# cosdata/cosdata

Hardware: AMD Instinct MI355X
Metric: QPS at recall@10≥0.95, 1024-dim dense cosine, 1/2/4/8 MI355X (higher is better)
Workload: dtype u8

## Files before the change

cosdata_amd/csrc/builder.hip:

```cpp
#include <algorithm>
#include <chrono>
#include <cmath>
#include <cstdio>
#include <cstdlib>
#include <cstring>
#include <map>

#include "engine_internal.h"

using namespace cosdev;

namespace {

constexpr u32 NONE = 0xFFFFFFFFu;

inline uint64_t splitmix64(uint64_t &st) {
    uint64_t z = (st += 0x9E3779B97F4A7C15ull);
    z = (z ^ (z >> 30)) * 0xBF58476D1CE4E5B9ull;
    z = (z ^ (z >> 27)) * 0x94D049BB133111EBull;
    return z ^ (z >> 31);
}
inline float rand_f32(uint64_t &st) { return (float)(splitmix64(st) >> 40) * (1.0f / 16777216.0f); }

inline int32_t total_key(float v) {
    int32_t b;
    memcpy(&b, &v, 4);
    b ^= (int32_t)(((uint32_t)(b >> 31)) >> 1);
    return b;
}
inline float metric_min(u32 metric) { return metric == COS_METRIC_COSINE ? -1.0f : -INFINITY; }
inline float metric_max(u32 metric) { return metric == COS_METRIC_COSINE ? 2.0f : INFINITY; }
inline int32_t order_key(u32 metric, float v) {
    const int32_t k = total_key(v);
    return (metric == COS_METRIC_EUCLIDEAN || metric == COS_METRIC_HAMMING) ? ~k : k;
}

}

namespace {

std::vector<double> level_probs(u32 Ltop) {
    std::vector<double> pv(Ltop + 1);
    for (u32 k = 0; k <= Ltop; k++) {
        const int nn = (int)(Ltop - k);
        double r = 1.0, a = 4.0;
        for (int b = nn;;) { if (b & 1) r *= a; b /= 2; if (b == 0) break; a *= a; }
        pv[k] = 1.0 - 1.0 / r;
    }
    return pv;
}
inline uint8_t draw_level(uint64_t &rng, const std::vector<double> &pv, u32 Ltop) {
    const double x = (double)rand_f32(rng);
    u32 k = 0;
    while (k < Ltop && !(x >= pv[k])) k++;
    return (uint8_t)(Ltop - k);
}

struct GraphGuard {
    cos_index *ix;
    bool armed = true;
    ~GraphGuard() {
        if (!armed) return;
        (void)hipStreamSynchronize(ix->own_stream);
        for (auto &l : ix->lv) l.release();
        ix->link.release();
        ix->adj_mag_valid = false;
        ix->have_root = false;
    }
};

void fill_link_levels(cos_index *ix, LinkArgs &la, u32 &maxM) {
    maxM = 0;
    for (u32 l = 0; l <= ix->p.num_layers; l++) {
        LevelHost &H = ix->lv[l];
        LinkLevelDev &D = la.lv[l];
        D.adj_vec = H.d_adj_vec;
        D.adj_node = l == 0 ? H.d_adj_vec : H.d_adj_node;
        D.node_vec = l == 0 ? nullptr : H.d_node_vec;
        D.key = ix->link.key[l].as<int32_t>();
        D.low_idx = ix->link.low_idx[l].as<uint8_t>();
        D.low_key = ix->link.low_key[l].as<int32_t>();
        D.owner = ix->link.owner[l].as<u32>();
        D.M = H.M;
        maxM = std::max(maxM, H.M);
    }
}

int32_t run_batches(cos_index *ix, u32 first, const uint8_t *max_level, std::vector<u32> &cursor, u32 Bmax) {
    const u32 n = ix->n, Ltop = ix->p.num_layers, L1 = Ltop + 1, metric = ix->p.metric;
    hipStream_t st = ix->own_stream;
    LinkArgs la;
    memset(&la, 0, sizeof(la));
    u32 maxM = 0;
    fill_link_levels(ix, la, maxM);
    if (maxM > 256) return cos_fail(COS_ERR_UNIMPLEMENTED, "more than 256 neighbour slots per node");

    const u32 KEEP = (u32)KEEP_INDEX;
    DevBuf d_rows, d_out_ids, d_out_nodes, d_out_sims, d_out_counts, d_status, d_me, d_pend[2], d_cnt, d_evq;
    PinArr<unsigned char> h_rows, h_me, h_pend, h_status, h_cnt;
    const size_t pend_cap = (size_t)Bmax * L1;
    const size_t evq_cap = pend_cap * 2 * KEEP;
    HIP_TRY(d_rows.alloc((size_t)Bmax * 4));
    HIP_TRY(d_out_ids.alloc((size_t)Bmax * L1 * KEEP * 4));
    HIP_TRY(d_out_nodes.alloc((size_t)Bmax * L1 * KEEP * 4));
    HIP_TRY(d_out_sims.alloc((size_t)Bmax * L1 * KEEP * 4));
    HIP_TRY(d_out_counts.alloc((size_t)Bmax * L1 * 4));
    HIP_TRY(d_status.alloc((size_t)Bmax * 4));
    HIP_TRY(d_me.alloc((size_t)Bmax * L1 * 4));
    HIP_TRY(d_pend[0].alloc(pend_cap * 4));
    HIP_TRY(d_pend[1].alloc(pend_cap * 4));
    HIP_TRY(d_cnt.alloc(4 * 4));
    HIP_TRY(d_evq.alloc(evq_cap * 3 * 4));
    HIP_TRY(h_rows.alloc((size_t)Bmax * 4));
    HIP_TRY(h_me.alloc((size_t)Bmax * L1 * 4));
    HIP_TRY(h_pend.alloc(pend_cap * 4));
    HIP_TRY(h_status.alloc((size_t)Bmax * 4));
    HIP_TRY(h_cnt.alloc(4 * 4));
    VisTab vtab;

    la.L1 = L1;
    la.z_nodes = d_out_nodes.as<u32>();
    la.z_sims = d_out_sims.as<float>();
    la.z_counts = d_out_counts.as<u32>();
    la.me = d_me.as<u32>();
    la.metric = metric;
    la.kmin = order_key(metric, metric_min(metric));
    la.kmax = order_key(metric, metric_max(metric));

    IndexDev dev = cos_make_index_dev(ix);
    u32 inserted = first, round = 0;
    u64 n_rounds = 0, n_batches = 0;
    const bool prof = cosdev::tune_or(cosdev::TUNE_BUILD_PROFILE, 0) != 0;
    double t_walk = 0, t_link = 0;
    auto now = []() { return std::chrono::duration<double>(std::chrono::steady_clock::now().time_since_epoch()).count(); };
    u32 *cnt = d_cnt.as<u32>();
    while (inserted < n) {
        const double t0 = now();
        n_batches++;
        const u32 bs = std::min({Bmax, std::max(1u, inserted / 4u), n - inserted});
        u32 np = 0;
        for (u32 b = 0; b < bs; b++) {
            const u32 id = inserted + b;
            h_rows.as<u32>()[b] = id;
            for (u32 l = 0; l <= Ltop; l++) {
                u32 m = NONE;
                if (max_level[id - first] >= l) { m = cursor[l]++; h_pend.as<u32>()[np++] = (l << 16) | b; }
                h_me.as<u32>()[(size_t)b * L1 + l] = m;
            }
        }
        HIP_TRY(hipMemcpyAsync(d_rows.p, h_rows.p, (size_t)bs * 4, hipMemcpyHostToDevice, st));
        HIP_TRY(hipMemcpyAsync(d_me.p, h_me.p, (size_t)bs * L1 * 4, hipMemcpyHostToDevice, st));
        HIP_TRY(hipMemcpyAsync(d_pend[0].p, h_pend.p, (size_t)np * 4, hipMemcpyHostToDevice, st));
        h_cnt.as<u32>()[0] = np; h_cnt.as<u32>()[1] = 0; h_cnt.as<u32>()[2] = 0; h_cnt.as<u32>()[3] = 0;
        HIP_TRY(hipMemcpyAsync(cnt, h_cnt.p, 16, hipMemcpyHostToDevice, st));
        WalkArgs wa;
        memset(&wa, 0, sizeof(wa));
        wa.qcodes = ix->d_codes;
        wa.qmags = ix->d_mags;
        wa.q_rows = d_rows.as<u32>();
        wa.self_ids = d_rows.as<u32>();
        if (dev.visited_mode == COS_VISITED_EXACT) {
            const int32_t vrc = vis_tab_prepare(vtab, ix, Bmax, ix->p.ef_construction, st, wa);
            if (vrc) return vrc;
        }
        wa.B = bs;
        wa.ef = ix->p.ef_construction;
        wa.keep = KEEP;
        wa.out_ids = d_out_ids.as<u32>();
        wa.out_sims = d_out_sims.as<float>();
        wa.out_nodes = d_out_nodes.as<u32>();
        wa.out_counts = d_out_counts.as<u32>();
        wa.out_status = d_status.as<int32_t>();
        cosdev::WalkPlanIn pin = cos_walk_plan_in(ix, bs, wa.ef);
        pin.table_min_B = pin.order_min_B = 0;
        HIP_TRY(launch_walk(ix->eng, dev, wa, cosdev::walk_plan(pin).kernel, st));
        HIP_TRY(hipMemcpyAsync(h_status.p, d_status.p, (size_t)bs * 4, hipMemcpyDeviceToHost, st));
        HIP_TRY(hipStreamSynchronize(st));
        for (u32 b = 0; b < bs; b++)
            if (h_status.as<int32_t>()[b] != COS_OK)
                return cos_fail(h_status.as<int32_t>()[b], "vector %u cannot be indexed (zero norm -> DistanceError::CalculationError)", inserted + b);
        t_walk += now() - t0;
        const double t1 = now();
        u32 pending_ub = np, cur = 0;
        while (pending_ub > 0) {
            const u32 chunk = pending_ub > 64 ? 2 : 4;
            for (u32 r = 0; r < chunk; r++) {
                if (++round > LINK_MAX_ROUND) {
                    for (u32 l = 0; l <= Ltop; l++) HIP_TRY(hipMemsetAsync(ix->link.owner[l].p, 0, (size_t)ix->lv[l].n * 4, st));
                    round = 1;
                }
                HIP_TRY(launch_link_round(la, maxM, d_pend[cur].as<u32>(), cnt + cur, d_pend[cur ^ 1].as<u32>(), cnt + (cur ^ 1), d_evq.as<u32>(), cnt + 2,
                                          pending_ub, round, st));
                cur ^= 1;
                n_rounds++;
            }
            HIP_TRY(hipMemcpyAsync(h_cnt.p, cnt, 16, hipMemcpyDeviceToHost, st));
            HIP_TRY(hipStreamSynchronize(st));
            pending_ub = h_cnt.as<u32>()[cur];
        }
        t_link += now() - t1;
        inserted += bs;
    }
    HIP_TRY(hipStreamSynchronize(st));
    if (prof)
        fprintf(stderr, "[cos_index_build] vectors [%u, %u) batches=%llu link rounds=%llu walk %.2fs link %.2fs\n", first, n, (unsigned long long)n_batches,
                (unsigned long long)n_rounds, t_walk, t_link);
    return COS_OK;
}

}

extern "C" int32_t cos_index_build(cos_index *ix, uint32_t batch_size) {
    if (!ix) return cos_fail(COS_ERR_INVALID, "null index");
    if (!ix->have_vectors) return cos_fail(COS_ERR_NOT_READY, "upload vectors before building");
    int32_t rc = cos_set_device(ix);
    if (rc) return rc;
    const u32 n = ix->n, Ltop = ix->p.num_layers, metric = ix->p.metric;
    const u32 Bmax = std::min<u32>(batch_size ? batch_size : 4096u, LINK_MAX_BATCH);
    hipStream_t st = ix->own_stream;
    GraphGuard guard{ix};

    ix->order_rank_valid = false;
    ix->level_table_valid = false;
    ix->adj_mag_valid = false;
    ix->link.release();
    uint64_t rng = ix->p.seed ? ix->p.seed : 0x1234567ull;
    std::vector<float> root(ix->p.dim);
    for (u32 i = 0; i < ix->p.dim; i++) root[i] = ix->p.range_lo + rand_f32(rng) * (ix->p.range_hi - ix->p.range_lo);
    rc = cos_index_set_root(ix, root.data());
    if (rc) return rc;
    const std::vector<double> pv = level_probs(Ltop);
    std::vector<uint8_t> max_level(n);
    for (u32 id = 0; id < n; id++) max_level[id] = draw_level(rng, pv, Ltop);

    for (u32 l = 0; l <= Ltop; l++) {
        LevelHost &H = ix->lv[l];
        H.release();
        for (u32 id = 0; id < n; id++)
            if (max_level[id] >= l) H.node_ids.push_back(id * ix->id_stride);
        H.node_ids.push_back(COS_ROOT_ID);
        const u32 nl = (u32)H.node_ids.size(), M = H.M;
        if (M > 256) return cos_fail(COS_ERR_UNIMPLEMENTED, "more than 256 neighbour slots per node");
        HIP_TRY(H.d_adj_vec.alloc((size_t)nl * M));
        HIP_TRY(hipMemsetAsync(H.d_adj_vec, 0xFF, (size_t)nl * M * 4, st));
        if (l > 0) {
            std::vector<u32> node_vec(nl), child(nl);
            const std::vector<u32> &D = ix->lv[l - 1].node_ids;
            for (u32 i = 0; i < nl; i++) {
                node_vec[i] = H.node_ids[i] == COS_ROOT_ID ? n : H.node_ids[i] / ix->id_stride;
                child[i] = (u32)(std::lower_bound(D.begin(), D.end(), H.node_ids[i]) - D.begin());
            }
            HIP_TRY(H.d_adj_node.alloc((size_t)nl * M));
            HIP_TRY(hipMemsetAsync(H.d_adj_node, 0xFF, (size_t)nl * M * 4, st));
            HIP_TRY(H.d_node_vec.alloc(nl));
            HIP_TRY(hipMemcpy(H.d_node_vec, node_vec.data(), (size_t)nl * 4, hipMemcpyHostToDevice));
            HIP_TRY(H.d_child.alloc(nl));
            HIP_TRY(hipMemcpy(H.d_child, child.data(), (size_t)nl * 4, hipMemcpyHostToDevice));
        }
        H.n = nl;
        HIP_TRY(ix->link.key[l].alloc((size_t)nl * M * 4));
        HIP_TRY(ix->link.low_idx[l].alloc(nl));
        HIP_TRY(ix->link.low_key[l].alloc((size_t)nl * 4));
        HIP_TRY(ix->link.owner[l].alloc((size_t)nl * 4));
        HIP_TRY(launch_fill_i32(ix->link.key[l].as<int32_t>(), (u64)nl * M, INT32_MIN, st));
        HIP_TRY(hipMemsetAsync(ix->link.low_idx[l].p, 0, nl, st));
        HIP_TRY(launch_fill_i32(ix->link.low_key[l].as<int32_t>(), nl, order_key(metric, metric_min(metric)), st));
        HIP_TRY(hipMemsetAsync(ix->link.owner[l].p, 0, (size_t)nl * 4, st));
    }
    HIP_TRY(hipStreamSynchronize(st));

    std::vector<u32> cursor(Ltop + 1, 0);
    rc = run_batches(ix, 0, max_level.data(), cursor, Bmax);
    if (rc) return rc;
    guard.armed = false;
    ix->link.rng = rng;
    ix->link.n_built = n;
    ix->link.valid = ix->id_stride == 1u;
    if (int32_t rc2 = cos_prepare_walk_plans(ix)) return rc2;
    return COS_OK;
}

extern "C" int32_t cos_index_restore_link_state(cos_index *ix) {
    if (!ix) return cos_fail(COS_ERR_INVALID, "null index");
    if (!ix->have_vectors || !ix->have_root) return cos_fail(COS_ERR_NOT_READY, "restore needs vectors, root and every graph level");
    for (auto &l : ix->lv) if (l.n == 0) return cos_fail(COS_ERR_NOT_READY, "restore needs vectors, root and every graph level");
    if (ix->id_stride != 1u || ix->meta.mdim != 0u) return cos_fail(COS_ERR_UNIMPLEMENTED, "link state of a collection with a metadata schema");
    int32_t rc = cos_set_device(ix);
    if (rc) return rc;
    HIP_TRY(hipDeviceSynchronize());
    const u32 Ltop = ix->p.num_layers, metric = ix->p.metric;
    const int32_t kmin = order_key(metric, metric_min(metric)), kmax = order_key(metric, metric_max(metric));
    hipStream_t st = ix->own_stream;
    ix->link.release();
    struct Fail { cos_index *ix; bool armed = true; ~Fail() { if (armed) ix->link.release(); } } fail_guard{ix};
    constexpr u64 CHUNK_PAIRS = 1ull << 24;
    DevBuf px, py, sims, dst, d_fail;
    HIP_TRY(px.alloc(CHUNK_PAIRS * 4));
    HIP_TRY(py.alloc(CHUNK_PAIRS * 4));
    HIP_TRY(sims.alloc(CHUNK_PAIRS * 4));
    HIP_TRY(dst.alloc(CHUNK_PAIRS * 4));
    HIP_TRY(d_fail.alloc(4));
    HIP_TRY(hipMemsetAsync(d_fail.p, 0, 4, st));
    for (u32 l = 0; l <= Ltop; l++) {
        LevelHost &H = ix->lv[l];
        const u32 nl = H.n, M = H.M;
        HIP_TRY(ix->link.key[l].alloc((size_t)nl * M * 4));
        HIP_TRY(ix->link.low_idx[l].alloc(nl));
        HIP_TRY(ix->link.low_key[l].alloc((size_t)nl * 4));
        HIP_TRY(ix->link.owner[l].alloc((size_t)nl * 4));
        HIP_TRY(hipMemsetAsync(ix->link.owner[l].p, 0, (size_t)nl * 4, st));
        const u32 step = (u32)std::max<u64>(1, CHUNK_PAIRS / M);
        for (u32 n0 = 0; n0 < nl; n0 += step) {
            const u32 cn = std::min(step, nl - n0);
            HIP_TRY(launch_edge_pairs(H.d_adj_vec, l == 0 ? nullptr : H.d_node_vec, n0, cn, M, px.as<u32>(), py.as<u32>(), st));
            HIP_TRY(cosdev::launch_index_pair_distances(ix->eng, ix->d_codes, ix->d_mags, ix->row_stride, ix->nchunks, ix->p.dim, metric, px.as<u32>(), py.as<u32>(),
                                                       (u32)((u64)cn * M), sims.as<float>(), dst.as<int32_t>(), st));
            HIP_TRY(launch_edge_keys(H.d_adj_vec, sims.as<float>(), dst.as<int32_t>(), n0, cn, M, metric, ix->link.key[l].as<int32_t>(), d_fail.as<int32_t>(), st));
        }
        HIP_TRY(launch_low_cache(H.d_adj_vec, ix->link.key[l].as<int32_t>(), nl, M, kmin, kmax, ix->link.low_idx[l].as<uint8_t>(), ix->link.low_key[l].as<int32_t>(), st));
    }
    int32_t failed = 0;
    HIP_TRY(hipMemcpyAsync(&failed, d_fail.p, 4, hipMemcpyDeviceToHost, st));
    HIP_TRY(hipStreamSynchronize(st));
    if (failed) return cos_fail(failed, "an edge of the uploaded graph has no similarity (zero norm -> DistanceError::CalculationError)");
    uint64_t rng = ix->p.seed ? ix->p.seed : 0x1234567ull;
    for (u64 i = 0; i < (u64)ix->p.dim + ix->n; i++) (void)rand_f32(rng);
    ix->link.rng = rng;
    ix->link.n_built = ix->n;
    ix->link.valid = true;
    fail_guard.armed = false;
    return COS_OK;
}

extern "C" int32_t cos_index_release_link_state(cos_index *ix) {
    if (!ix) return cos_fail(COS_ERR_INVALID, "null index");
    int32_t rc = cos_set_device(ix);
    if (rc) return rc;
    HIP_TRY(hipStreamSynchronize(ix->own_stream));
    ix->link.release();
    return COS_OK;
}

extern "C" int32_t cos_index_append(cos_index *ix, const float *raw, uint32_t m, uint32_t flags, uint32_t batch_size) {
    if (!ix || !raw || m == 0) return cos_fail(COS_ERR_INVALID, "null/empty vectors");
    if (!ix->have_vectors || !ix->have_root) return cos_fail(COS_ERR_NOT_READY, "append needs a built index");
    for (auto &l : ix->lv) if (l.n == 0) return cos_fail(COS_ERR_NOT_READY, "append needs a built index");
    if (!ix->link.valid || ix->link.n_built != ix->n)
        return cos_fail(COS_ERR_NOT_READY, "no link state to continue from: the graph was uploaded (not built by cos_index_build on this handle), its root "
                                           "was replaced, or cos_index_release_link_state freed it");
    if (ix->id_stride != 1u || ix->meta.mdim != 0u) return cos_fail(COS_ERR_UNIMPLEMENTED, "append on a collection with a metadata schema");
    if ((u64)ix->n + m >= 0xFFFFFFF0ull) return cos_fail(COS_ERR_INVALID, "too many vectors");
    const bool borrow = (flags & COS_UPLOAD_BORROW_DEVICE) != 0;
    if (borrow != !ix->raw_own)
        return cos_fail(COS_ERR_INVALID, borrow ? "the index owns its raw rows: append host rows" : "the index borrows its raw rows: append with COS_UPLOAD_BORROW_DEVICE and the whole grown table");
    int32_t rc = cos_set_device(ix);
    if (rc) return rc;
    const u32 n0 = ix->n, n1 = n0 + m, Ltop = ix->p.num_layers, metric = ix->p.metric;
    const u32 Bmax = std::min<u32>(batch_size ? batch_size : 4096u, LINK_MAX_BATCH);
    const u64 dim = ix->p.dim, rs = ix->row_stride;
    hipStream_t st = ix->own_stream;
    HIP_TRY(hipDeviceSynchronize());
    GraphGuard guard{ix};
    ix->order_rank_valid = false;
    ix->level_table_valid = false;
    ix->adj_mag_valid = false;
    ix->link.valid = false;
    cos_flat_ws_release(ix);

    {
        DevArr<uint8_t> codes;
        DevArr<float> mags, raw_mags, new_raw;
        HIP_TRY(codes.alloc(((size_t)n1 + 2) * rs));
        HIP_TRY(mags.alloc((size_t)n1 + 2));
        HIP_TRY(raw_mags.alloc((size_t)n1 + 2));
        HIP_TRY(hipMemcpyAsync(codes, ix->d_codes, (size_t)n0 * rs, hipMemcpyDeviceToDevice, st));
        HIP_TRY(hipMemcpyAsync(codes + (size_t)n1 * rs, ix->d_codes + (size_t)n0 * rs, 2 * rs, hipMemcpyDeviceToDevice, st));
        HIP_TRY(hipMemcpyAsync(mags, ix->d_mags, (size_t)n0 * 4, hipMemcpyDeviceToDevice, st));
        HIP_TRY(hipMemcpyAsync(mags + n1, ix->d_mags + n0, 8, hipMemcpyDeviceToDevice, st));
        HIP_TRY(hipMemcpyAsync(raw_mags, ix->d_raw_mags, (size_t)n0 * 4, hipMemcpyDeviceToDevice, st));
        HIP_TRY(hipMemsetAsync(raw_mags + n1, 0, 8, st));
        const float *new_rows;
        if (borrow) {
            new_rows = raw + (size_t)n0 * dim;
        } else {
            HIP_TRY(new_raw.alloc((size_t)n1 * dim));
            HIP_TRY(hipMemcpyAsync(new_raw, ix->d_raw, (size_t)n0 * dim * 4, hipMemcpyDeviceToDevice, st));
            HIP_TRY(hipMemcpyAsync(new_raw + (size_t)n0 * dim, raw, (size_t)m * dim * 4, hipMemcpyHostToDevice, st));
            new_rows = new_raw + (size_t)n0 * dim;
        }
        HIP_TRY(launch_quantize_rows(ix->eng, new_rows, dim, m, ix->p.dim, ix->p.range_lo, ix->p.range_hi, codes + (size_t)n0 * rs, rs, mags + n0, raw_mags + n0, st));
        HIP_TRY(cos_deleted_grow(ix, n0, n1, st));
        HIP_TRY(hipStreamSynchronize(st));
        codes.swap(ix->d_codes);
        mags.swap(ix->d_mags);
        raw_mags.swap(ix->d_raw_mags);
        new_raw.swap(ix->raw_own);
        ix->d_raw = borrow ? raw : ix->raw_own.p;
        ix->n = n1;
    }

    uint64_t rng = ix->link.rng;
    const std::vector<double> pv = level_probs(Ltop);
    std::vector<uint8_t> max_level(m);
    for (u32 i = 0; i < m; i++) max_level[i] = draw_level(rng, pv, Ltop);

    std::vector<u32> cursor(Ltop + 1, 0);
    std::vector<u32> add(Ltop + 1, 0);
    for (u32 l = 0; l <= Ltop; l++)
        for (u32 i = 0; i < m; i++) add[l] += max_level[i] >= l ? 1u : 0u;
    for (u32 l = 0; l <= Ltop; l++) {
        LevelHost &H = ix->lv[l];
        const u32 nl0 = H.n, nl1 = nl0 + add[l], M = H.M;
        cursor[l] = nl0 - 1;
        H.node_ids.pop_back();
        for (u32 i = 0; i < m; i++) if (max_level[i] >= l) H.node_ids.push_back(n0 + i);
        H.node_ids.push_back(COS_ROOT_ID);
        H.host_valid = false;
        H.nbr_ids.clear();
        H.d_adj_mag.reset();
        DevArr<u32> adj_vec, adj_node, node_vec, child;
        DevBuf key, low_idx, low_key;
        HIP_TRY(adj_vec.alloc((size_t)nl1 * M));
        HIP_TRY(launch_grow_rows(H.d_adj_vec, adj_vec, nl0, nl1, M, n0, n1, ROW_EMPTY, st));
        if (l > 0) {
            HIP_TRY(adj_node.alloc((size_t)nl1 * M));
            HIP_TRY(launch_grow_rows(H.d_adj_node, adj_node, nl0, nl1, M, nl0 - 1, nl1 - 1, ROW_EMPTY, st));
            std::vector<u32> nv(add[l] + 1), ch(add[l] + 1);
            const u32 below0 = ix->lv[l - 1].n - add[l - 1] - 1;
            u32 k = 0, kb = 0;
            for (u32 i = 0; i < m; i++) {
                if (max_level[i] >= l) { nv[k] = n0 + i; ch[k] = below0 + kb; k++; }
                if (max_level[i] >= l - 1) kb++;
            }
            nv[k] = n1;
            ch[k] = ix->lv[l - 1].n - 1;
            HIP_TRY(node_vec.alloc(nl1));
            HIP_TRY(child.alloc(nl1));
            HIP_TRY(hipMemcpyAsync(node_vec, H.d_node_vec, (size_t)(nl0 - 1) * 4, hipMemcpyDeviceToDevice, st));
            HIP_TRY(hipMemcpyAsync(child, H.d_child, (size_t)(nl0 - 1) * 4, hipMemcpyDeviceToDevice, st));
            HIP_TRY(hipMemcpy(node_vec + (nl0 - 1), nv.data(), nv.size() * 4, hipMemcpyHostToDevice));
            HIP_TRY(hipMemcpy(child + (nl0 - 1), ch.data(), ch.size() * 4, hipMemcpyHostToDevice));
        }
        HIP_TRY(key.alloc((size_t)nl1 * M * 4));
        HIP_TRY(low_idx.alloc(nl1));
        HIP_TRY(low_key.alloc((size_t)nl1 * 4));
        HIP_TRY(launch_grow_rows(ix->link.key[l].as<u32>(), key.as<u32>(), nl0, nl1, M, 0xFFFFFFFFu, 0xFFFFFFFFu, (u32)INT32_MIN, st));
        HIP_TRY(launch_grow_rows(ix->link.low_key[l].as<u32>(), low_key.as<u32>(), nl0, nl1, 1, 0xFFFFFFFFu, 0xFFFFFFFFu, (u32)order_key(metric, metric_min(metric)), st));
        HIP_TRY(launch_grow_bytes(ix->link.low_idx[l].as<uint8_t>(), low_idx.as<uint8_t>(), nl0, nl1, st));
        HIP_TRY(ix->link.owner[l].alloc((size_t)nl1 * 4));
        HIP_TRY(hipMemsetAsync(ix->link.owner[l].p, 0, (size_t)nl1 * 4, st));
        HIP_TRY(hipStreamSynchronize(st));
        adj_vec.swap(H.d_adj_vec);
        adj_node.swap(H.d_adj_node);
        node_vec.swap(H.d_node_vec);
        child.swap(H.d_child);
        key.swap(ix->link.key[l]);
        low_idx.swap(ix->link.low_idx[l]);
        low_key.swap(ix->link.low_key[l]);
        H.n = nl1;
    }

    rc = run_batches(ix, n0, max_level.data(), cursor, Bmax);
    if (rc) return rc;
    guard.armed = false;
    ix->link.rng = rng;
    ix->link.n_built = n1;
    ix->link.valid = true;
    if (int32_t rc2 = cos_prepare_walk_plans(ix)) return rc2;
    return COS_OK;
}

namespace {

struct RowCache {
    struct Row { std::vector<u32> adj; std::vector<int32_t> key; uint8_t low_idx; int32_t low_key; bool dirty = false; };
    cos_index *ix; u32 level; u32 M;
    std::map<u32, Row> rows;
    hipError_t err = hipSuccess;
    Row &get(u32 node) {
        auto it = rows.find(node);
        if (it != rows.end()) return it->second;
        Row &r = rows[node];
        LevelHost &H = ix->lv[level];
        r.adj.resize(M); r.key.resize(M);
        auto cp = [&](void *dst, const void *src, size_t n) { if (err == hipSuccess) err = hipMemcpy(dst, src, n, hipMemcpyDeviceToHost); };
        cp(r.adj.data(), (level == 0 ? H.d_adj_vec : H.d_adj_node) + (size_t)node * M, (size_t)M * 4);
        cp(r.key.data(), ix->link.key[level].as<int32_t>() + (size_t)node * M, (size_t)M * 4);
        cp(&r.low_idx, ix->link.low_idx[level].as<uint8_t>() + node, 1);
        cp(&r.low_key, ix->link.low_key[level].as<int32_t>() + node, 4);
        return r;
    }
    hipError_t flush(const std::vector<u32> &node_vec ) {
        LevelHost &H = ix->lv[level];
        for (auto &kv : rows) {
            if (!kv.second.dirty || err != hipSuccess) continue;
            const u32 node = kv.first;
            Row &r = kv.second;
            auto cp = [&](void *dst, const void *src, size_t n) { if (err == hipSuccess) err = hipMemcpy(dst, src, n, hipMemcpyHostToDevice); };
            if (level == 0) cp(H.d_adj_vec + (size_t)node * M, r.adj.data(), (size_t)M * 4);
            else {
                std::vector<u32> av(M);
                for (u32 j = 0; j < M; j++) av[j] = r.adj[j] == NONE ? NONE : node_vec[r.adj[j]];
                cp(H.d_adj_node + (size_t)node * M, r.adj.data(), (size_t)M * 4);
                cp(H.d_adj_vec + (size_t)node * M, av.data(), (size_t)M * 4);
            }
            cp(ix->link.key[level].as<int32_t>() + (size_t)node * M, r.key.data(), (size_t)M * 4);
            cp(ix->link.low_idx[level].as<uint8_t>() + node, &r.low_idx, 1);
            cp(ix->link.low_key[level].as<int32_t>() + node, &r.low_key, 4);
        }
        return err;
    }
};

int add_neighbor_host(RowCache &rc, u32 self, u32 nbr, int32_t k, int32_t kmin, int32_t kmax) {
    RowCache::Row &r = rc.get(self);
    const u32 M = rc.M, li = r.low_idx;
    if (k <= r.low_key) return -1;
    const bool ok = r.adj[li] == NONE || k > r.key[li];
    u32 old = NONE;
    if (ok) { old = r.adj[li]; r.adj[li] = nbr; r.key[li] = k; }
    u32 nl = 0;
    int32_t nk = kmax;
    for (u32 j = 0; j < M; j++) {
        if (r.adj[j] == NONE) { nk = kmin; nl = j; break; }
        if (r.key[j] < nk) { nk = r.key[j]; nl = j; }
    }
    r.low_idx = (uint8_t)nl;
    r.low_key = nk;
    r.dirty = true;
    if (!ok) return -1;
    if (old != NONE) {
        RowCache::Row &o = rc.get(old);
        for (u32 j = 0; j < M; j++) if (o.adj[j] == self) { o.adj[j] = NONE; o.key[j] = INT32_MIN; o.dirty = true; break; }
    }
    return (int)li;
}

}

extern "C" int32_t cos_index_delete(cos_index *ix, const uint32_t *ids, uint32_t m) {
    if (!ix || (!ids && m)) return cos_fail(COS_ERR_INVALID, "null argument");
    if (!ix->have_vectors || !ix->have_root) return cos_fail(COS_ERR_NOT_READY, "delete needs a built index");
    for (auto &l : ix->lv) if (l.n == 0) return cos_fail(COS_ERR_NOT_READY, "delete needs a built index");
    if (!ix->link.valid) return cos_fail(COS_ERR_NOT_READY, "no link state (the graph was uploaded, its root replaced, or cos_index_release_link_state freed it)");
    if (ix->id_stride != 1u || ix->meta.mdim != 0u) return cos_fail(COS_ERR_UNIMPLEMENTED, "delete on a collection with a metadata schema");
    for (u32 i = 0; i < m; i++) if (ids[i] >= ix->n) return cos_fail(COS_ERR_INVALID, "id %u is not a resident vector", ids[i]);
    if (m == 0) return COS_OK;
    int32_t rc = cos_set_device(ix);
    if (rc) return rc;
    HIP_TRY(hipDeviceSynchronize());
    const u32 Ltop = ix->p.num_layers, L1 = Ltop + 1, metric = ix->p.metric, KEEP = (u32)KEEP_SEARCH, EF = 512;
    hipStream_t st = ix->own_stream;
    HIP_TRY(cos_deleted_mark(ix, ids, m, st));
    LinkArgs la;
    memset(&la, 0, sizeof(la));
    u32 maxM = 0;
    fill_link_levels(ix, la, maxM);
    la.L1 = L1;
    la.metric = metric;
    const int32_t kmin = order_key(metric, metric_min(metric)), kmax = order_key(metric, metric_max(metric));
    DevBuf d_row, d_out_ids, d_out_nodes, d_out_sims, d_out_counts, d_status, d_dn, d_ust, d_px, d_py, d_ds, d_dst;
    HIP_TRY(d_row.alloc(4));
    HIP_TRY(d_out_ids.alloc((size_t)L1 * KEEP * 4));
    HIP_TRY(d_out_nodes.alloc((size_t)L1 * KEEP * 4));
    HIP_TRY(d_out_sims.alloc((size_t)L1 * KEEP * 4));
    HIP_TRY(d_out_counts.alloc((size_t)L1 * 4));
    HIP_TRY(d_status.alloc(4));
    HIP_TRY(d_dn.alloc((size_t)L1 * 4));
    HIP_TRY(d_ust.alloc((size_t)L1 * 4));
    HIP_TRY(d_px.alloc((size_t)KEEP * 4));
    HIP_TRY(d_py.alloc((size_t)KEEP * 4));
    HIP_TRY(d_ds.alloc((size_t)KEEP * 4));
    HIP_TRY(d_dst.alloc((size_t)KEEP * 4));
    VisTab vtab;
    std::vector<u32> h_ids((size_t)L1 * KEEP), h_nodes((size_t)L1 * KEEP), h_counts(L1), h_dn(L1), h_ust(L1);
    std::vector<std::vector<u32>> node_vec(L1);
    ix->adj_mag_valid = false;
    for (auto &l : ix->lv) { l.host_valid = false; l.nbr_ids.clear(); }

    for (u32 t = 0; t < m; t++) {
        const u32 id = ids[t];
        IndexDev dev = cos_make_index_dev(ix);
        for (u32 l = 0; l <= Ltop; l++) dev.lv[l].adj_mag = nullptr;
        WalkArgs wa;
        memset(&wa, 0, sizeof(wa));
        HIP_TRY(hipMemcpyAsync(d_row.p, &id, 4, hipMemcpyHostToDevice, st));
        wa.qcodes = ix->d_codes;
        wa.qmags = ix->d_mags;
        wa.q_rows = d_row.as<u32>();
        wa.no_self_seed = 1u;
        if (dev.visited_mode == COS_VISITED_EXACT) {
            const int32_t vrc = vis_tab_prepare(vtab, ix, 1, EF, st, wa);
            if (vrc) return vrc;
        }
        wa.B = 1;
        wa.ef = EF;
        wa.keep = KEEP;
        wa.out_ids = d_out_ids.as<u32>();
        wa.out_sims = d_out_sims.as<float>();
        wa.out_nodes = d_out_nodes.as<u32>();
        wa.out_counts = d_out_counts.as<u32>();
        wa.out_status = d_status.as<int32_t>();
        cosdev::WalkPlanIn pin = cos_walk_plan_in(ix, 1, EF);
        pin.table_min_B = pin.order_min_B = 0;
        pin.no_self_seed = true;
        HIP_TRY(launch_walk(ix->eng, dev, wa, cosdev::walk_plan(pin).kernel, st));
        int32_t wst = COS_OK;
        HIP_TRY(hipMemcpyAsync(&wst, d_status.p, 4, hipMemcpyDeviceToHost, st));
        HIP_TRY(hipMemcpyAsync(h_ids.data(), d_out_ids.p, h_ids.size() * 4, hipMemcpyDeviceToHost, st));
        HIP_TRY(hipMemcpyAsync(h_nodes.data(), d_out_nodes.p, h_nodes.size() * 4, hipMemcpyDeviceToHost, st));
        HIP_TRY(hipMemcpyAsync(h_counts.data(), d_out_counts.p, (size_t)L1 * 4, hipMemcpyDeviceToHost, st));
        HIP_TRY(hipStreamSynchronize(st));
        if (wst != COS_OK) return cos_fail(wst, "vector %u cannot be walked for (zero norm -> DistanceError::CalculationError)", id);
        bool any = false;
        for (u32 l = 0; l <= Ltop; l++) {
            const u32 slot = Ltop - l;
            h_dn[l] = NONE;
            for (u32 i = 0; i < h_counts[slot]; i++)
                if (h_ids[(size_t)slot * KEEP + i] == id) { h_dn[l] = h_nodes[(size_t)slot * KEEP + i]; any = true; break; }
        }
        if (!any) continue;
        HIP_TRY(hipMemcpyAsync(d_dn.p, h_dn.data(), (size_t)L1 * 4, hipMemcpyHostToDevice, st));
        HIP_TRY(launch_unlink(la, d_dn.as<u32>(), d_ust.as<u32>(), st));
        HIP_TRY(hipMemcpyAsync(h_ust.data(), d_ust.p, (size_t)L1 * 4, hipMemcpyDeviceToHost, st));
        HIP_TRY(hipStreamSynchronize(st));
        for (u32 l = 0; l <= Ltop; l++) {
            if (h_ust[l] != 1u) continue;
            const LevelHost &H = ix->lv[l];
            const u32 M = H.M, slot = Ltop - l, node = h_dn[l];
            if (l > 0 && node_vec[l].empty()) {
                node_vec[l].resize(H.n);
                HIP_TRY(hipMemcpy(node_vec[l].data(), H.d_node_vec, (size_t)H.n * 4, hipMemcpyDeviceToHost));
            }
            auto vec_row = [&](u32 nd) { return l == 0 ? nd : node_vec[l][nd]; };
            std::vector<u32> res;
            for (u32 i = 0; i < h_counts[slot]; i++) if (h_nodes[(size_t)slot * KEEP + i] != node) res.push_back(h_nodes[(size_t)slot * KEEP + i]);
            RowCache cache{ix, l, M};
            RowCache::Row &dr = cache.get(node);
            for (u32 j = 0; j < M; j++) {
                const u32 x = dr.adj[j];
                if (x == NONE) continue;
                RowCache::Row &xr = cache.get(x);
                bool removed = false, empty = true;
                for (u32 k = 0; k < M; k++) if (xr.adj[k] == node) { xr.adj[k] = NONE; xr.key[k] = INT32_MIN; xr.dirty = true; removed = true; break; }
                for (u32 k = 0; k < M; k++) if (xr.adj[k] != NONE) { empty = false; break; }
                if (!(removed && empty)) continue;
                std::vector<u32> cand, px, py;
                for (u32 r : res) if (r != x) { cand.push_back(r); px.push_back(vec_row(x)); py.push_back(vec_row(r)); }
                std::vector<float> sims(cand.size());
                std::vector<int32_t> dst(cand.size());
                if (!cand.empty()) {
                    HIP_TRY(hipMemcpyAsync(d_px.p, px.data(), px.size() * 4, hipMemcpyHostToDevice, st));
                    HIP_TRY(hipMemcpyAsync(d_py.p, py.data(), py.size() * 4, hipMemcpyHostToDevice, st));
                    HIP_TRY(cosdev::launch_index_pair_distances(ix->eng, ix->d_codes, ix->d_mags, ix->row_stride, ix->nchunks, ix->p.dim, metric, d_px.as<u32>(), d_py.as<u32>(),
                                                               (u32)cand.size(), d_ds.as<float>(), d_dst.as<int32_t>(), st));
                    HIP_TRY(hipMemcpyAsync(sims.data(), d_ds.p, sims.size() * 4, hipMemcpyDeviceToHost, st));
                    HIP_TRY(hipMemcpyAsync(dst.data(), d_dst.p, dst.size() * 4, hipMemcpyDeviceToHost, st));
                    HIP_TRY(hipStreamSynchronize(st));
                    for (int32_t e : dst) if (e != COS_OK) return cos_fail(e, "re-linking node %u after the delete of %u failed (DistanceError)", x, id);
                }
// ... 255 lines not shown
```

cosdata_amd/csrc/device_common.h:

```cpp
#pragma once
#include <hip/hip_runtime.h>
#include <stdint.h>
#include <type_traits>

namespace cosdev {

typedef uint32_t u32;
typedef unsigned long long u64;

constexpr int WAVE = 64;
constexpr u32 ROW_EMPTY = 0xFFFFFFFFu;
constexpr int KEEP_SEARCH = 100;
constexpr int KEEP_INDEX = 64;
constexpr int MAX_LEVELS = 16;

enum : int { ENG_U8 = 0, ENG_Q2 = 1, ENG_F32 = 2, ENG_F16 = 3, ENG_Q1 = 4, ENG_Q3 = 5 };

__device__ __forceinline__ u32 simkey(float v) {
    u32 b = __float_as_uint(v);
    return b ^ ((b >> 31) ? 0xFFFFFFFFu : 0x80000000u);
}
__device__ __forceinline__ float simkey_inv(u32 k) {
    u32 b = (k & 0x80000000u) ? (k ^ 0x80000000u) : ~k;
    return __uint_as_float(b);
}
__device__ __forceinline__ u32 metric_key(u32 metric, float v) {
    u32 k = simkey(v);
    return (metric == 1u || metric == 2u) ? ~k : k;
}
__device__ __forceinline__ float metric_key_inv(u32 metric, u32 k) {
    return simkey_inv((metric == 1u || metric == 2u) ? ~k : k);
}
__device__ __forceinline__ u64 pack_key(u32 hi, u32 lo) { return ((u64)hi << 32) | (u64)lo; }

__device__ __forceinline__ float div_rn_unscaled(float num, float den) {
    float r = __builtin_amdgcn_rcpf(den);
    const float e = __builtin_fmaf(-den, r, 1.0f);
    r = __builtin_fmaf(e, r, r);
    float q = num * r;
    float t = __builtin_fmaf(-den, q, num);
    q = __builtin_fmaf(t, r, q);
    t = __builtin_fmaf(-den, q, num);
    return __builtin_fmaf(t, r, q);
}

__device__ __forceinline__ u64 shfl_xor_u64(u64 v, int m) {
    u32 lo = (u32)v, hi = (u32)(v >> 32);
    lo = (u32)__shfl_xor((int)lo, m, WAVE);
    hi = (u32)__shfl_xor((int)hi, m, WAVE);
    return ((u64)hi << 32) | lo;
}
__device__ __forceinline__ u64 shfl_up1_u64(u64 v) {
    u32 lo = (u32)v, hi = (u32)(v >> 32);
    lo = (u32)__shfl_up((int)lo, 1, WAVE);
    hi = (u32)__shfl_up((int)hi, 1, WAVE);
    return ((u64)hi << 32) | lo;
}
__device__ __forceinline__ u64 shfl_down1_u64(u64 v) {
    u32 lo = (u32)v, hi = (u32)(v >> 32);
    lo = (u32)__shfl_down((int)lo, 1, WAVE);
    hi = (u32)__shfl_down((int)hi, 1, WAVE);
    return ((u64)hi << 32) | lo;
}
template <int CTRL>
__device__ __forceinline__ u32 dpp_mov(u32 fill, u32 v) {
    return (u32)__builtin_amdgcn_update_dpp((int)fill, (int)v, CTRL, 0xf, 0xf, false);
}
template <int CTRL>
__device__ __forceinline__ u32 dpp_mov_z(u32 v) {
    return (u32)__builtin_amdgcn_update_dpp(0, (int)v, CTRL, 0xf, 0xf, true);
}
__device__ __forceinline__ u64 dpp_wave_shr1_u64(u64 v, u64 fill) {
    u32 lo = dpp_mov<0x138>((u32)fill, (u32)v), hi = dpp_mov<0x138>((u32)(fill >> 32), (u32)(v >> 32));
    return ((u64)hi << 32) | lo;
}
__device__ __forceinline__ u64 dpp_wave_shl1_u64(u64 v, u64 fill) {
    u32 lo = dpp_mov<0x130>((u32)fill, (u32)v), hi = dpp_mov<0x130>((u32)(fill >> 32), (u32)(v >> 32));
    return ((u64)hi << 32) | lo;
}
__device__ __forceinline__ u32 group_reduce_add_u32(u32 v, int G) {
    if (G >= 2) v += dpp_mov<0xB1>(0u, v);
    if (G >= 4) v += dpp_mov<0x4E>(0u, v);
    if (G >= 8) v += dpp_mov<0x141>(0u, v);
    if (G >= 16) v += dpp_mov<0x140>(0u, v);
    if (G == 32) v += (u32)__shfl_xor((int)v, 16, WAVE);
    if (G == 64) {
        const u32 t = (u32)__builtin_amdgcn_readlane((int)v, 0) + (u32)__builtin_amdgcn_readlane((int)v, 16) +
                      (u32)__builtin_amdgcn_readlane((int)v, 32) + (u32)__builtin_amdgcn_readlane((int)v, 48);
        v = t;
    }
    return v;
}

__device__ __forceinline__ u32 fold_halves(u32 a, u32 b) {
// ... 76 lines not shown
```

cosdata_amd/csrc/engine.hip:

```cpp
#include <hip/hip_runtime.h>

#include <algorithm>
#include <cstdarg>
#include <cstdio>
#include <cstdlib>
#include <chrono>
#include <cmath>
#include <condition_variable>
#include <cstring>
#include <map>
#include <mutex>
#include <string>
#include <thread>
#include <vector>

#include "engine_internal.h"

using namespace cosdev;

static thread_local std::string g_err;
int32_t cos_fail(int32_t code, const char *fmt, ...) {
    char buf[512];
    va_list ap;
    va_start(ap, fmt);
    vsnprintf(buf, sizeof(buf), fmt, ap);
    va_end(ap);
    g_err = buf;
    return code;
}

extern "C" const char *cos_last_error_string(void) { return g_err.c_str(); }

extern "C" int32_t cos_device_count(int32_t *out) {
    if (!out) return cos_fail(COS_ERR_INVALID, "null argument");
    int n = 0;
    hipError_t e = hipGetDeviceCount(&n);
    if (e != hipSuccess) { *out = 0; return cos_fail(COS_ERR_NO_DEVICE, "hipGetDeviceCount: %s", hipGetErrorString(e)); }
    *out = n;
    return COS_OK;
}

static u32 pow2ceil(u32 v) { u32 p = 1; while (p < v) p <<= 1; return p; }

int32_t cos_set_device(const cos_index *ix) {
    HIP_TRY(hipSetDevice(ix->p.device));
    return COS_OK;
}

static bool graph_ready(const cos_index *ix) {
    if (!ix->have_vectors || !ix->have_root) return false;
    for (auto &l : ix->lv) if (l.n == 0) return false;
    return true;
}

IndexDev cos_make_index_dev(const cos_index *ix) {
    IndexDev d;
    memset(&d, 0, sizeof(d));
    d.codes = ix->d_codes;
    d.mags = ix->d_mags;
    d.raw = ix->d_raw;
    d.raw_mags = ix->d_raw_mags;
    d.row_stride = ix->row_stride;
    d.raw_stride = ix->p.dim;
    d.n = ix->n;
    d.dim = ix->p.dim;
    d.metric = ix->p.metric;
    d.storage = ix->p.storage;
    d.num_layers = ix->p.num_layers;
    d.shortlist = ix->p.shortlist_size;
    d.visited_mode = ix->p.visited_mode;
    d.nchunks = ix->nchunks;
    d.G = ix->G;
    d.id_base = ix->p.id_base;
    d.id_stride = ix->id_stride;
    d.mbits = ix->meta.d_mbits;
    d.mmags = ix->meta.d_mmags;
    d.mdim = ix->meta.mdim;
    for (u32 l = 0; l <= ix->p.num_layers; l++) {
        const LevelHost &h = ix->lv[l];
        d.lv[l].adj_vec = h.d_adj_vec;
        d.lv[l].adj_node = l == 0 ? h.d_adj_vec : h.d_adj_node;
        d.lv[l].node_vec = l == 0 ? nullptr : h.d_node_vec;
        d.lv[l].child = l == 0 ? nullptr : h.d_child;
        d.lv[l].n = h.n;
        d.lv[l].M = h.M;
        d.lv[l].root_idx = h.n ? h.n - 1 : 0;
        d.lv[l].adj_mag = (ix->adj_mag_valid && cosdev::tune_or(cosdev::TUNE_WALK_ADJ_MAG, 1) != 0) ? h.d_adj_mag : nullptr;
        d.lv[l].mag_stride = std::min(h.M, ix->p.shortlist_size);
    }
    return d;
}

extern "C" int32_t cos_index_create(const cos_params *p, cos_index **out) {
    if (!p || !out) return cos_fail(COS_ERR_INVALID, "null argument");
    *out = nullptr;
    if (p->struct_size != sizeof(cos_params) || p->abi_version != COS_ABI_VERSION)
        return cos_fail(COS_ERR_INVALID, "cos_params size/version mismatch (%u/%u, expected %zu/%u)", p->struct_size, p->abi_version,
                    sizeof(cos_params), COS_ABI_VERSION);
    if (p->dim == 0) return cos_fail(COS_ERR_INVALID, "dim == 0");
    auto pow2 = [](u32 v) { return v && !(v & (v - 1)); };
    if (!pow2(p->neighbors_count) || !pow2(p->level0_neighbors_count) || p->neighbors_count > 256 || p->level0_neighbors_count > 256)
        return cos_fail(COS_ERR_INVALID, "neighbors_count / level_0_neighbors_count must be powers of two <= 256 (PerformantFixedSet, fixedset.rs)");
    if (p->num_layers + 1 > (u32)MAX_LEVELS || (p->num_layers + 1) * KEEP_SEARCH > 2048)
        return cos_fail(COS_ERR_UNIMPLEMENTED, "num_layers > 15 not supported on the device");
    if (p->ef_search > cosdev::WALK_GENERAL_MAX_EF || p->ef_construction > cosdev::WALK_GENERAL_MAX_EF)
        return cos_fail(COS_ERR_UNIMPLEMENTED, "ef > %u not supported on the device (the candidates of a level live in one workgroup's LDS)", cosdev::WALK_GENERAL_MAX_EF);
    if (p->metric != COS_METRIC_COSINE && p->metric != COS_METRIC_DOT)
        return cos_fail(COS_ERR_UNIMPLEMENTED, "device walk implements cosine and dot-product metrics");
    int eng;
    u64 row_stride;
    u32 nchunks = 0, G = 1;
    switch (p->storage) {
    case COS_STORAGE_U8:
        eng = ENG_U8; row_stride = ((u64)p->dim + 15) & ~15ull; nchunks = (u32)(row_stride / 16); G = std::min(64u, pow2ceil(nchunks));
        break;
    case COS_STORAGE_SUBBYTE:
        if (p->resolution == 1) { eng = ENG_Q1; nchunks = (p->dim + 127) / 128; }
        else if (p->resolution == 2) { eng = ENG_Q2; nchunks = (p->dim + 63) / 64; }
        else if (p->resolution == 3) { eng = ENG_Q3; nchunks = (p->dim + 31) / 32; }
        else return cos_fail(COS_ERR_CALCULATION, "SubByte resolution %u: the reference's distance arms return CalculationError (cosine.rs:147-154)", p->resolution);
        row_stride = (u64)nchunks * 16; G = std::min(64u, pow2ceil(nchunks));
        break;
    case COS_STORAGE_F32:
        if (p->metric == COS_METRIC_DOT) return cos_fail(COS_ERR_STORAGE_MISMATCH, "DotProductDistance has no FullPrecisionFP arm (dotproduct.rs:20-64)");
        eng = ENG_F32; row_stride = ((u64)p->dim * 4 + 15) & ~15ull; G = 2;
        break;
    case COS_STORAGE_F16:
        eng = ENG_F16; row_stride = ((u64)p->dim * 2 + 15) & ~15ull; G = 1;
        break;
    default: return cos_fail(COS_ERR_UNIMPLEMENTED, "storage kind %u not supported on the device yet", p->storage);
    }
    int ndev = 0;
    if (hipGetDeviceCount(&ndev) != hipSuccess || ndev <= 0) return cos_fail(COS_ERR_NO_DEVICE, "no HIP device visible; the GPU path has no CPU fallback");
    if (p->device < 0 || p->device >= ndev) return cos_fail(COS_ERR_INVALID, "device %d out of range (%d visible)", p->device, ndev);
    cos_index *ix = new cos_index();
    ix->chain_min_B = (u32)cosdev::tune_or(cosdev::TUNE_WALK_CHAIN_MIN_B, ix->chain_min_B);
    ix->walk_order_min_B = (u32)cosdev::tune_or(cosdev::TUNE_WALK_ORDER_MIN_B, ix->walk_order_min_B);
    ix->walk_side_min_B = (u32)cosdev::tune_or(cosdev::TUNE_WALK_SIDE_MIN_B, ix->walk_side_min_B);
    ix->p = *p;
    ix->eng = eng;
    ix->row_stride = row_stride;
    ix->nchunks = nchunks;
    ix->G = G;
    ix->lv.resize(p->num_layers + 1);
    for (u32 l = 0; l <= p->num_layers; l++) ix->lv[l].M = l == 0 ? p->level0_neighbors_count : p->neighbors_count;
    if (hipSetDevice(p->device) != hipSuccess || hipStreamCreateWithFlags(&ix->own_stream, hipStreamNonBlocking) != hipSuccess) {
        delete ix;
        return cos_fail(COS_ERR_HIP, "cannot create stream on device %d", p->device);
    }
    int nx = 0;
    if (hipDeviceGetAttribute(&nx, hipDeviceAttributeNumberOfXccs, p->device) == hipSuccess && nx >= 1 && nx <= 64) ix->num_xcd = (u32)nx;
    else { (void)hipGetLastError(); ix->num_xcd = 1; }
    int ncu = 0;
    if (hipDeviceGetAttribute(&ncu, hipDeviceAttributeMultiprocessorCount, p->device) == hipSuccess && ncu >= 1) ix->n_cus = (u32)ncu;
    else (void)hipGetLastError();
    *out = ix;
    return COS_OK;
}

IndexDev cos_make_meta_dev(const cos_index *ix) {
    IndexDev d = cos_make_index_dev(ix);
    for (u32 l = 0; l <= ix->p.num_layers; l++) {
        const LevelHost &h = ix->meta.lv[l];
        d.lv[l].adj_vec = h.d_adj_vec;
        d.lv[l].adj_node = h.d_adj_node;
        d.lv[l].node_vec = h.d_node_vec;
        d.lv[l].child = h.d_child;
        d.lv[l].node_id = h.d_node_id;
        d.lv[l].node_meta = h.d_node_meta;
        d.lv[l].n = h.n;
        d.lv[l].M = h.M;
        d.lv[l].root_idx = h.root_idx;
    }
    return d;
}

void cos_meta_free_levels(cos_index *ix) {
    for (auto &l : ix->meta.lv) l.release();
}

static void reset_meta(cos_index *ix) {
    for (auto &l : ix->meta.lv) l.release();
    ix->meta.d_mbits.reset();
    ix->meta.d_mmags.reset();
    ix->meta.node_ids.clear();
    ix->meta.mdim = 0;
    ix->id_stride = 1;
}

extern "C" int32_t cos_index_destroy(cos_index *ix) {
    if (!ix) return COS_OK;
    (void)hipSetDevice(ix->p.device);
    (void)hipDeviceSynchronize();
    ix->ws.clear();
    cos_flat_ws_release(ix);
    ix->pipes_all.clear();
    cos_coalesce_release(ix);
    for (auto &l : ix->lv) l.release();
    reset_meta(ix);
    if (ix->own_stream) (void)hipStreamDestroy(ix->own_stream);
    delete ix;
    return COS_OK;
}

extern "C" int32_t cos_index_upload_vectors(cos_index *ix, const float *raw, uint32_t n, uint32_t flags) {
    if (!ix || !raw || n == 0) return cos_fail(COS_ERR_INVALID, "null/empty vectors");
    if (n >= 0xFFFFFFF0u) return cos_fail(COS_ERR_INVALID, "too many vectors");
    int32_t rc = cos_set_device(ix);
    if (rc) return rc;
    ix->d_raw = nullptr;
    ix->raw_own.reset(); ix->d_raw_mags.reset(); ix->d_codes.reset(); ix->d_mags.reset(); ix->d_deleted.reset();
    ix->have_vectors = false;
    cos_flat_ws_release(ix);
    ix->have_root = false;
    for (auto &l : ix->lv) l.release();
    ix->order_rank_valid = false;
    ix->level_table_valid = false;
    ix->adj_mag_valid = false;
    ix->link.release();
    reset_meta(ix);
    const u64 dim = ix->p.dim;
    const float *d_raw = raw;
    DevArr<float> raw_own, raw_mags, mags;
    DevArr<uint8_t> codes;
    if (flags & COS_UPLOAD_BORROW_DEVICE) {
        HIP_TRY(hipDeviceSynchronize());
    } else {
        HIP_TRY(raw_own.alloc((size_t)n * dim));
        HIP_TRY(hipMemcpy(raw_own, raw, (size_t)n * dim * 4, hipMemcpyHostToDevice));
        d_raw = raw_own;
    }
    HIP_TRY(raw_mags.alloc((size_t)n + 2));
    HIP_TRY(codes.alloc(((size_t)n + 2) * ix->row_stride));
    HIP_TRY(mags.alloc((size_t)n + 2));
    HIP_TRY(hipMemsetAsync(codes + (size_t)n * ix->row_stride, 0, 2 * ix->row_stride, ix->own_stream));
    HIP_TRY(hipMemsetAsync(mags + n, 0, 8, ix->own_stream));
    HIP_TRY(launch_quantize_rows(ix->eng, d_raw, dim, n, ix->p.dim, ix->p.range_lo, ix->p.range_hi, codes, ix->row_stride, mags, raw_mags, ix->own_stream));
    HIP_TRY(cos_deleted_reset(ix, n, ix->own_stream));
    HIP_TRY(hipStreamSynchronize(ix->own_stream));
    ix->d_raw = d_raw;
    ix->raw_own = std::move(raw_own);
    ix->d_raw_mags = std::move(raw_mags);
    ix->d_codes = std::move(codes);
    ix->d_mags = std::move(mags);
    ix->n = n;
    ix->have_vectors = true;
    ix->have_root = false;
    return COS_OK;
}

extern "C" int32_t cos_index_set_root(cos_index *ix, const float *root_raw) {
    if (!ix || !root_raw) return cos_fail(COS_ERR_INVALID, "null argument");
    if (!ix->have_vectors) return cos_fail(COS_ERR_NOT_READY, "upload vectors before the root");
    int32_t rc = cos_set_device(ix);
    if (rc) return rc;
    ix->root_raw.assign(root_raw, root_raw + ix->p.dim);
    DevBuf tmp;
    HIP_TRY(tmp.alloc(((size_t)ix->p.dim + 1) * 4));
    float *d_tmp = tmp.as<float>(), *d_dummy = d_tmp + ix->p.dim;
    HIP_TRY(hipMemcpy(d_tmp, root_raw, (size_t)ix->p.dim * 4, hipMemcpyHostToDevice));
    HIP_TRY(launch_quantize_rows(ix->eng, d_tmp, ix->p.dim, 1, ix->p.dim, ix->p.range_lo, ix->p.range_hi,
                                 ix->d_codes + (size_t)ix->n * ix->row_stride, ix->row_stride, ix->d_mags + ix->n, d_dummy, ix->own_stream));
    HIP_TRY(hipStreamSynchronize(ix->own_stream));
    ix->have_root = true;
    ix->level_table_valid = false;
    ix->adj_mag_valid = false;
    if (ix->link.valid && graph_ready(ix)) ix->link.release();
    return COS_OK;
}

static inline u32 row_of(const cos_index *ix, u32 id) { return id == COS_ROOT_ID ? ix->n : id / ix->id_stride; }

static int32_t push_level_to_device(cos_index *ix, u32 level) {
    LevelHost &L = ix->lv[level];
    const u32 n = (u32)L.node_ids.size(), M = L.M;
    std::vector<u32> adj_vec((size_t)n * M), adj_node, node_vec, child;
    if (level > 0) { adj_node.resize((size_t)n * M); node_vec.resize(n); }
    for (u32 i = 0; i < n; i++) {
        if (level > 0) node_vec[i] = row_of(ix, L.node_ids[i]);
        for (u32 j = 0; j < M; j++) {
            u32 id = L.nbr_ids[(size_t)i * M + j];
            if (id == COS_SLOT_EMPTY) {
                adj_vec[(size_t)i * M + j] = ROW_EMPTY;
                if (level > 0) adj_node[(size_t)i * M + j] = ROW_EMPTY;
                continue;
            }
            auto it = std::lower_bound(L.node_ids.begin(), L.node_ids.end(), id);
            if (it == L.node_ids.end() || *it != id) return cos_fail(COS_ERR_INVALID, "level %u: neighbour id %u of node %u is not a node of this level", level, id, L.node_ids[i]);
            adj_vec[(size_t)i * M + j] = row_of(ix, id);
            if (level > 0) adj_node[(size_t)i * M + j] = (u32)(it - L.node_ids.begin());
        }
    }
    L.d_adj_node.reset();
    L.d_node_vec.reset();
    HIP_TRY(L.d_adj_vec.alloc(adj_vec.size()));
    HIP_TRY(hipMemcpy(L.d_adj_vec, adj_vec.data(), adj_vec.size() * 4, hipMemcpyHostToDevice));
    if (level > 0) {
        HIP_TRY(L.d_adj_node.alloc(adj_node.size()));
        HIP_TRY(hipMemcpy(L.d_adj_node, adj_node.data(), adj_node.size() * 4, hipMemcpyHostToDevice));
        HIP_TRY(L.d_node_vec.alloc(node_vec.size()));
        HIP_TRY(hipMemcpy(L.d_node_vec, node_vec.data(), node_vec.size() * 4, hipMemcpyHostToDevice));
    }
    L.n = n;
    L.host_valid = true;
    ix->order_rank_valid = false;
    ix->level_table_valid = false;
    ix->adj_mag_valid = false;
    ix->link.release();
    return COS_OK;
}

static int32_t push_level0_to_device(cos_index *ix, const u32 *nbr) {
    LevelHost &L = ix->lv[0];
    const u32 n = (u32)L.node_ids.size(), M = L.M;
    const size_t slots = (size_t)n * M, chunk = (size_t)32 << 20;
    struct Staging {
        hipEvent_t done[2] = {nullptr, nullptr};
        ~Staging() {
            for (int b = 0; b < 2; b++)
                if (done[b]) (void)hipEventSynchronize(done[b]), (void)hipEventDestroy(done[b]);
        }
    };
    PinArr<u32> buf[2];
    Staging stg;
    HIP_TRY(L.d_adj_vec.alloc(slots));
    for (int b = 0; b < 2; b++) {
        HIP_TRY(buf[b].alloc(std::min(chunk, slots)));
        HIP_TRY(hipEventCreateWithFlags(&stg.done[b], hipEventDisableTiming));
    }
    const u32 nt = std::max(1u, std::min(16u, std::thread::hardware_concurrency()));
    for (size_t c0 = 0, k = 0; c0 < slots; c0 += chunk, k++) {
        const size_t m = std::min(chunk, slots - c0);
        u32 *out = buf[k & 1];
        if (k >= 2) HIP_TRY(hipEventSynchronize(stg.done[k & 1]));
        std::vector<int> bad(nt, 0);
        auto convert = [&](u32 t) {
            for (size_t s = m * t / nt, e = m * (t + 1) / nt; s < e; s++) {
                const u32 id = nbr[c0 + s];
                if (id == COS_SLOT_EMPTY) { out[s] = ROW_EMPTY; continue; }
                if (id != COS_ROOT_ID && (id % ix->id_stride != 0 || id / ix->id_stride >= ix->n)) { bad[t] = 1; return; }
                out[s] = row_of(ix, id);
            }
        };
        std::vector<std::thread> th;
        u32 started = 0;
        try {
            th.reserve(nt);
            for (; started < nt; started++) th.emplace_back(convert, started);
        } catch (...) {
        }
        for (u32 t = started; t < nt; t++) convert(t);
        for (auto &x : th) x.join();
        for (int b : bad)
            if (b) return cos_fail(COS_ERR_INVALID, "level 0: a neighbour id is not a node of this level");
        HIP_TRY(hipMemcpyAsync(L.d_adj_vec + c0, out, m * 4, hipMemcpyHostToDevice, ix->own_stream));
        HIP_TRY(hipEventRecord(stg.done[k & 1], ix->own_stream));
    }
    HIP_TRY(hipStreamSynchronize(ix->own_stream));
    L.nbr_ids.clear();
    L.nbr_ids.shrink_to_fit();
    L.n = n;
    L.host_valid = false;
    ix->order_rank_valid = false;
    ix->level_table_valid = false;
    ix->adj_mag_valid = false;
    ix->link.release();
    return COS_OK;
}

static int32_t resolve_children(cos_index *ix, u32 level) {
    if (level == 0 || level > ix->p.num_layers) return COS_OK;
    LevelHost &L = ix->lv[level], &D = ix->lv[level - 1];
    if (L.node_ids.empty() || D.node_ids.empty()) return COS_OK;
    std::vector<u32> child(L.node_ids.size());
    for (size_t i = 0; i < L.node_ids.size(); i++) {
        auto it = std::lower_bound(D.node_ids.begin(), D.node_ids.end(), L.node_ids[i]);
        if (it == D.node_ids.end() || *it != L.node_ids[i]) return cos_fail(COS_ERR_INVALID, "node %u of level %u is missing on level %u", L.node_ids[i], level, level - 1);
        child[i] = (u32)(it - D.node_ids.begin());
    }
    HIP_TRY(L.d_child.alloc(child.size()));
    HIP_TRY(hipMemcpy(L.d_child, child.data(), child.size() * 4, hipMemcpyHostToDevice));
    return COS_OK;
}

extern "C" int32_t cos_index_upload_graph_level(cos_index *ix, uint32_t level, uint32_t n_nodes, const uint32_t *node_ids,
                                                const uint32_t *nbr_ids) {
    if (!ix || !node_ids || !nbr_ids) return cos_fail(COS_ERR_INVALID, "null argument");
    if (!ix->have_vectors) return cos_fail(COS_ERR_NOT_READY, "upload vectors before the graph");
    if (level > ix->p.num_layers || n_nodes == 0) return cos_fail(COS_ERR_INVALID, "bad level / empty level");
    int32_t rc = cos_set_device(ix);
    if (rc) return rc;
    for (u32 i = 0; i < n_nodes; i++) {
        if (i && node_ids[i] <= node_ids[i - 1]) return cos_fail(COS_ERR_INVALID, "level %u: node_ids must be strictly ascending", level);
        if (node_ids[i] != COS_ROOT_ID && (node_ids[i] % ix->id_stride != 0 || node_ids[i] / ix->id_stride >= ix->n))
            return cos_fail(COS_ERR_INVALID, "level %u: node id %u is not the base id of a resident vector (ids are vector row x %u)", level, node_ids[i], ix->id_stride);
    }
    if (node_ids[n_nodes - 1] != COS_ROOT_ID) return cos_fail(COS_ERR_INVALID, "level %u: the root (0xFFFFFFFF) must be the last node", level);
    if (level == 0 && n_nodes != ix->n + 1) return cos_fail(COS_ERR_INVALID, "level 0 must hold every vector plus the root (%u nodes, expected %u)", n_nodes, ix->n + 1);
    LevelHost &L = ix->lv[level];
    L.node_ids.assign(node_ids, node_ids + n_nodes);
    if (level == 0) {
        rc = push_level0_to_device(ix, nbr_ids);
    } else {
        L.nbr_ids.assign(nbr_ids, nbr_ids + (size_t)n_nodes * L.M);
        rc = push_level_to_device(ix, level);
    }
    if (rc) { L.release(); return rc; }
    rc = resolve_children(ix, level);
    if (rc == COS_OK) rc = resolve_children(ix, level + 1);
    if (rc == COS_OK && graph_ready(ix)) rc = cos_prepare_walk_plans(ix);
    return rc;
}

extern "C" int32_t cos_index_level_count(const cos_index *ix, uint32_t level, uint32_t *n_nodes) {
    if (!ix || !n_nodes || level > ix->p.num_layers) return cos_fail(COS_ERR_INVALID, "bad argument");
    *n_nodes = ix->lv[level].n;
    return COS_OK;
}

static int32_t materialize_host_level(cos_index *ix, u32 level) {
    LevelHost &L = ix->lv[level];
    if (L.host_valid) return COS_OK;
    if (L.n == 0 || L.node_ids.size() != L.n || !L.d_adj_vec) return cos_fail(COS_ERR_NOT_READY, "level %u not resident", level);
    int32_t rc = cos_set_device(ix);
    if (rc) return rc;
    std::vector<u32> adj((size_t)L.n * L.M);
    HIP_TRY(hipMemcpy(adj.data(), level == 0 ? L.d_adj_vec : L.d_adj_node, adj.size() * 4, hipMemcpyDeviceToHost));
    L.nbr_ids.resize(adj.size());
    for (size_t i = 0; i < adj.size(); i++) L.nbr_ids[i] = adj[i] == ROW_EMPTY ? COS_SLOT_EMPTY : L.node_ids[adj[i]];
    L.host_valid = true;
    return COS_OK;
}

extern "C" int32_t cos_index_download_graph_level(const cos_index *ix_, uint32_t level, uint32_t *node_ids, uint32_t *nbr_ids) {
    cos_index *ix = const_cast<cos_index *>(ix_);
    if (!ix || level > ix->p.num_layers) return cos_fail(COS_ERR_INVALID, "bad argument");
    {
        std::lock_guard<std::mutex> g(ix->mu);
        const int32_t rc = materialize_host_level(ix, level);
        if (rc) return rc;
    }
    const LevelHost &L = ix->lv[level];
    if (node_ids) memcpy(node_ids, L.node_ids.data(), L.node_ids.size() * 4);
    if (nbr_ids) memcpy(nbr_ids, L.nbr_ids.data(), L.nbr_ids.size() * 4);
    return COS_OK;
}

extern "C" size_t cos_code_bytes(uint32_t storage, uint32_t resolution, uint32_t dim) {
    switch (storage) {
    case COS_STORAGE_U8: return dim;
    case COS_STORAGE_SUBBYTE: return (size_t)resolution * ((dim + 7) / 8);
    case COS_STORAGE_F16: return (size_t)dim * 2;
    case COS_STORAGE_F32: return (size_t)dim * 4;
    default: return 0;
    }
}

static void row_to_reference_layout(int eng, u32 dim, const uint8_t *dev_row, uint8_t *ref_row) {
    if (eng == ENG_U8) memcpy(ref_row, dev_row, dim);
    else if (eng == ENG_F32) memcpy(ref_row, dev_row, (size_t)dim * 4);
    else if (eng == ENG_F16) memcpy(ref_row, dev_row, (size_t)dim * 2);
    else if (eng == ENG_Q1) memcpy(ref_row, dev_row, (dim + 7) / 8);
    else if (eng == ENG_Q2) {
        const u32 pb = (dim + 7) / 8;
        for (u32 p = 0; p < 2; p++)
            for (u32 b = 0; b < pb; b++) ref_row[(size_t)p * pb + b] = dev_row[(size_t)(b / 8) * 16 + p * 8 + (b % 8)];
    } else {
        const u32 pb = (dim + 7) / 8;
        for (u32 p = 0; p < 3; p++)
            for (u32 b = 0; b < pb; b++) ref_row[(size_t)p * pb + b] = dev_row[(size_t)(b / 4) * 16 + p * 4 + (b % 4)];
    }
}

static void row_to_device_layout(int eng, u32 dim, const uint8_t *ref_row, uint8_t *dev_row) {
    if (eng == ENG_U8) memcpy(dev_row, ref_row, dim);
    else if (eng == ENG_F32) memcpy(dev_row, ref_row, (size_t)dim * 4);
    else if (eng == ENG_F16) memcpy(dev_row, ref_row, (size_t)dim * 2);
    else if (eng == ENG_Q1) memcpy(dev_row, ref_row, (dim + 7) / 8);
    else if (eng == ENG_Q2) {
        const u32 pb = (dim + 7) / 8;
        for (u32 p = 0; p < 2; p++)
            for (u32 b = 0; b < pb; b++) dev_row[(size_t)(b / 8) * 16 + p * 8 + (b % 8)] = ref_row[(size_t)p * pb + b];
    } else {
        const u32 pb = (dim + 7) / 8;
        for (u32 p = 0; p < 3; p++)
            for (u32 b = 0; b < pb; b++) dev_row[(size_t)(b / 4) * 16 + p * 4 + (b % 4)] = ref_row[(size_t)p * pb + b];
    }
}

int32_t cos_set_root_code(cos_index *ix, const uint8_t *ref_code, float mag) {
    if (!ix->have_vectors) return cos_fail(COS_ERR_NOT_READY, "upload vectors before the root");
    int32_t rc = cos_set_device(ix);
    if (rc) return rc;
    std::vector<uint8_t> dev(ix->row_stride, 0);
    row_to_device_layout(ix->eng, ix->p.dim, ref_code, dev.data());
    if (ix->eng == ENG_U8) {
        const float hi = 255.0f * sqrtf((float)ix->p.dim) * 1.0001f;
        if (!(mag == 0.0f || (mag >= 1.0f && mag <= hi))) {
            uint32_t ss = 0;
            for (u32 i = 0; i < ix->p.dim; i++) ss += (uint32_t)ref_code[i] * (uint32_t)ref_code[i];
            mag = sqrtf((float)ss);
        }
    }
    HIP_TRY(hipMemcpy(ix->d_codes + (size_t)ix->n * ix->row_stride, dev.data(), dev.size(), hipMemcpyHostToDevice));
    HIP_TRY(hipMemcpy(ix->d_mags + ix->n, &mag, 4, hipMemcpyHostToDevice));
    ix->root_raw.assign(ix->p.dim, 0.0f);
    ix->have_root = true;
    ix->level_table_valid = false;
    ix->adj_mag_valid = false;
    return COS_OK;
}

int32_t cos_push_level_ids(cos_index *ix, u32 level, std::vector<u32> &&node_ids, std::vector<u32> &&nbr_ids) {
    return cos_index_upload_graph_level(ix, level, (u32)node_ids.size(), node_ids.data(), nbr_ids.data());
}

extern "C" int32_t cos_index_download_codes(const cos_index *ix, void *codes, float *mags) {
    if (!ix || !ix->have_vectors) return cos_fail(COS_ERR_NOT_READY, "no vectors resident");
    HIP_TRY(hipSetDevice(ix->p.device));
    const size_t rows = (size_t)ix->n + 1;
    if (codes) {
        std::vector<uint8_t> dev(rows * ix->row_stride);
        HIP_TRY(hipMemcpy(dev.data(), ix->d_codes, dev.size(), hipMemcpyDeviceToHost));
        const size_t cb = cos_code_bytes(ix->p.storage, ix->p.resolution, ix->p.dim);
        for (size_t r = 0; r < rows; r++) row_to_reference_layout(ix->eng, ix->p.dim, dev.data() + r * ix->row_stride, (uint8_t *)codes + r * cb);
    }
    if (mags) HIP_TRY(hipMemcpy(mags, ix->d_mags, rows * 4, hipMemcpyDeviceToHost));
    return COS_OK;
}

extern "C" int32_t cos_index_download_root(const cos_index *ix, float *root_raw) {
    if (!ix || !root_raw) return cos_fail(COS_ERR_INVALID, "null argument");
    if (!ix->have_root) return cos_fail(COS_ERR_NOT_READY, "no root");
    memcpy(root_raw, ix->root_raw.data(), (size_t)ix->p.dim * 4);
    return COS_OK;
}

static int32_t ensure_level_table(cos_index *ix);
static u32 walk_table_min_B(const cos_index *ix);
extern "C" int32_t cos_index_set_ef_search(cos_index *ix, uint32_t ef) {
    if (!ix) return cos_fail(COS_ERR_INVALID, "null index");
    if (ef > cosdev::WALK_GENERAL_MAX_EF) return cos_fail(COS_ERR_UNIMPLEMENTED, "ef > %u not supported on the device", cosdev::WALK_GENERAL_MAX_EF);
    std::lock_guard<std::mutex> g(ix->mu);
    const bool live = graph_ready(ix);
    if (live)
        if (int32_t rc = cos_set_device(ix)) return rc;
    ix->p.ef_search = ef;
    if (live && walk_table_min_B(ix)) (void)ensure_level_table(ix);
    return COS_OK;
}
extern "C" int32_t cos_index_set_visited_mode(cos_index *ix, uint32_t mode) {
    if (!ix || mode > 1) return cos_fail(COS_ERR_INVALID, "bad visited mode");
    std::lock_guard<std::mutex> g(ix->mu);
    ix->p.visited_mode = mode;
    return COS_OK;
}
extern "C" int32_t cos_index_set_latency_mode(cos_index *ix, uint32_t max_queries) {
    if (!ix) return cos_fail(COS_ERR_INVALID, "null");
    std::lock_guard<std::mutex> g(ix->mu);
    ix->lat_max_B = max_queries;
    return COS_OK;
}

extern "C" int32_t cos_index_set_latency_waves(cos_index *ix, uint32_t max_queries) {
    if (!ix) return cos_fail(COS_ERR_INVALID, "null");
    std::lock_guard<std::mutex> g(ix->mu);
    ix->lat4_max_B = max_queries;
    return COS_OK;
}
extern "C" int32_t cos_index_set_walk_order(cos_index *ix, uint32_t min_queries) {
    if (!ix) return cos_fail(COS_ERR_INVALID, "null");
    std::lock_guard<std::mutex> g(ix->mu);
    ix->walk_order_min_B = min_queries;
    return COS_OK;
}
extern "C" int32_t cos_index_enable_timing(cos_index *ix, int32_t on) {
    if (!ix) return cos_fail(COS_ERR_INVALID, "null");
    std::lock_guard<std::mutex> g(ix->mu);
    if (on && !ix->timing) for (auto &kv : ix->ws) kv.second->ev_count = 0;
    ix->timing = on != 0;
    return COS_OK;
}

int32_t vis_tab_prepare(VisTab &vt, const cos_index *ix, u32 B, u32 ef, hipStream_t st, WalkArgs &wa) {
    const u32 M = std::max(ix->p.level0_neighbors_count, ix->p.neighbors_count);
    const u64 log_cap = (u64)ef * M + 2;
    u32 max_nodes = 0;
    for (const LevelHost &l : ix->lv) max_nodes = std::max(max_nodes, l.n);
    const u32 words = (max_nodes + 31) / 32 + 1;
    if (log_cap > 0xFFFFFFFFull) return cos_fail(COS_ERR_INVALID, "ef too large");
    const size_t need_bits = (size_t)B * words, need_log = (size_t)B * log_cap;
    if (need_bits > vt.bits.cap || need_log > vt.log.cap) {
// ... 6 lines not shown
        HIP_TRY(hipMemsetAsync(vt.bits, 0, vt.bits.cap * 4, st));
        vt.zeroed = true;
    }
    wa.vis_bits = vt.bits;
    wa.vis_log = vt.log;
    wa.vis_words_per_query = words;
    wa.vis_log_cap = (u32)log_cap;
    return COS_OK;
}

static int32_t ensure_order_rank(cos_index *ix) {
    if (ix->order_rank_valid) return COS_OK;
    for (u32 l = 0; l < cosdev::MAX_LEVELS; l++) {
        ix->d_order_rank[l].reset();
        ix->order_rank_n[l] = 0;
    }
    ix->order_levels.clear();
    const u32 Ltop = ix->p.num_layers;
    auto usable = [&](u32 l) { return l >= 1 && l <= Ltop && ix->lv[l].n > 1 && ix->lv[l].n <= (1u << 20) && ix->lv[l].d_adj_node; };
    std::vector<u32> want;
    if (const long long mask = cosdev::tune(cosdev::TUNE_WALK_SPLIT_LEVELS); mask != cosdev::TUNE_UNSET) {
        for (u32 l = Ltop; l >= 1; l--)
            if ((mask >> l) & 1) want.push_back(l);
    } else {
        for (u32 l = 1; l <= Ltop; l++)
            if (usable(l) && (size_t)ix->lv[l].n * ix->row_stride <= ((size_t)64 << 20)) { want.push_back(l); break; }
    }
    u32 prev = Ltop + 1;
    for (u32 l : want) {
        if (!usable(l) || l >= prev) continue;
        ix->order_levels.push_back(l);
        prev = l;
    }
    if (!ix->order_levels.empty()) HIP_TRY(hipDeviceSynchronize());
    for (u32 kl : ix->order_levels) {
        const LevelHost &H = ix->lv[kl];
        const u32 n = H.n, M = H.M;
        std::vector<u32> adj((size_t)n * M), rank(n, 0u), stack;
        HIP_TRY(hipMemcpy(adj.data(), H.d_adj_node, adj.size() * 4, hipMemcpyDeviceToHost));
        std::vector<uint8_t> seen(n, 0);
        u32 next = 0;
        auto dfs_from = [&](u32 start) {
            stack.push_back(start);
            while (!stack.empty()) {
                const u32 v = stack.back();
                stack.pop_back();
                if (seen[v]) continue;
                seen[v] = 1;
                rank[v] = next++;
                const u32 *row = &adj[(size_t)v * M];
                for (u32 j = M; j-- > 0;) {
                    const u32 u = row[j];
                    if (u != cosdev::ROW_EMPTY && u < n && !seen[u]) stack.push_back(u);
                }
            }
        };
        dfs_from(n - 1);
        for (u32 v = 0; v < n; v++) if (!seen[v]) dfs_from(v);
        HIP_TRY(ix->d_order_rank[kl].alloc(n));
        HIP_TRY(hipMemcpy(ix->d_order_rank[kl], rank.data(), (size_t)n * 4, hipMemcpyHostToDevice));
        ix->order_rank_n[kl] = n;
    }
    ix->order_rank_valid = true;
    return COS_OK;
}

static void clear_current_table(cos_index *ix) {
    ix->d_tcodes = nullptr;
    ix->d_tmags = nullptr;
    ix->d_tcsums = nullptr;
    ix->table_cols = 0;
    ix->table_level_min = 0;
    ix->table_stride = 0;
}
static u32 walk_table_max_cols(const cos_index *ix) {
    const long long env = cosdev::tune_or(cosdev::TUNE_WALK_TABLE_COLS, -1);
    return env >= 0 ? (u32)std::min<long long>(env, 1ll << 20) : ix->walk_table_max_cols;
}
static u32 walk_table_min_B(const cos_index *ix) {
    const long long env = cosdev::tune_or(cosdev::TUNE_WALK_TABLE_MIN_B, -1);
    return env >= 0 ? (u32)std::min<long long>(env, 0xFFFFFFFFll) : ix->walk_table_min_B;
}
static constexpr long long WALK_TABLE_EARLY_WGS_DEFAULT = 0;
cosdev::WalkPlanIn cos_walk_plan_in(const cos_index *ix, u32 B, u32 ef) {
    cosdev::WalkPlanIn in{};
    in.eng = ix->eng;
    in.storage = ix->p.storage;
    in.nchunks = ix->nchunks;
    in.G = ix->G;
    in.num_layers = ix->p.num_layers;
    for (u32 l = 0; l <= ix->p.num_layers; l++) in.M[l] = ix->lv[l].M;
    in.shortlist = ix->p.shortlist_size;
    in.visited_mode = ix->p.visited_mode;
    in.mdim = ix->meta.mdim;
    in.B = B;
    in.ef = ef;
    in.chain = true;
    const long long lat = cosdev::tune_or(cosdev::TUNE_WALK_LAT, -1), lat4 = cosdev::tune_or(cosdev::TUNE_WALK_LAT4, -1);
    in.lat_max_B = lat >= 0 ? (u32)std::min(lat, 0xFFFFFFFFll) : ix->lat_max_B;
    in.lat4_max_B = lat4 >= 0 ? (u32)std::min(lat4, 0xFFFFFFFFll) : ix->lat4_max_B;
    in.small_table_tk = cosdev::tune_or(cosdev::TUNE_WALK_SMALL_TABLE_TK, 1) != 0;
    in.adj_mag_mode = (u32)cosdev::tune_or(cosdev::TUNE_WALK_ADJ_MAG, 1);
    in.table_min_B = walk_table_min_B(ix);
    in.order_min_B = ix->walk_order_min_B;
    in.chain_min_B = ix->chain_min_B;
    in.side_min_B = ix->walk_side_min_B;
    in.table_after_sort = cosdev::tune_or(cosdev::TUNE_WALK_TABLE_AFTER_SORT, 1);
    in.table_supported = cosdev::level_table_eng_supported(ix->eng, ix->row_stride);
    in.adj_mag_valid = ix->adj_mag_valid;
    in.table_early_wgs = (u32)std::min<long long>(std::max<long long>(cosdev::tune_or(cosdev::TUNE_WALK_TABLE_EARLY_WGS, WALK_TABLE_EARLY_WGS_DEFAULT), 0), 0xFFFFFFFFll);
    in.table_queue = cosdev::level_table_gemm_queue(ix->eng, ix->row_stride);
    in.n_cus = ix->n_cus;
    return in;
}
static int32_t ensure_level_table(cos_index *ix) {
    const u32 max_cols = walk_table_max_cols(ix);
    const bool automatic = max_cols == COS_WALK_TABLE_AUTO;
    const u32 efs = ix->p.ef_search, Mup = ix->p.neighbors_count;
    const u64 c_rule = (u64)cosdev::tune_or(cosdev::TUNE_WALK_TABLE_RULE_C, 2u * efs <= 3u * Mup ? 10 : (efs <= 2u * Mup ? 8 : 6));
    const u64 per_level = automatic ? std::min<u64>(c_rule * ix->p.ef_search * ix->p.neighbors_count, 1u << 20) : (u64)(1u << 20);
    const u64 total_cap = automatic ? (u64)(1u << 20) : (u64)max_cols;
    const u64 key = automatic ? (0x8000000000000000ull | per_level) : (u64)max_cols;
    if (ix->level_table_valid && ix->table_built_for_key == key) return COS_OK;
    if (!ix->level_table_valid) {
        HIP_TRY(hipDeviceSynchronize());
        ix->table_sets.clear();
    }
    ix->level_table_valid = true;
    ix->table_built_for_key = key;
    clear_current_table(ix);
    for (const auto &t : ix->table_sets)
        if (t.key == key) {
            ix->table_level_min = t.level_min;
            ix->table_cols = t.cols;
            ix->table_stride = t.stride;
            memcpy(ix->table_col0, t.col0, sizeof(t.col0));
            ix->d_tcodes = t.tcodes;
            ix->d_tmags = t.tmags;
            ix->d_tcsums = t.tcsums;
            return COS_OK;
        }
    if (!cosdev::level_table_eng_supported(ix->eng, ix->row_stride) || max_cols == 0) return COS_OK;
    const u32 Ltop = ix->p.num_layers;
    u32 cols = 0, lmin = 0;
    for (u32 l = Ltop; l >= 1; l--) {
        if (!ix->lv[l].d_node_vec || ix->lv[l].n == 0 || ix->lv[l].n > per_level || (u64)cols + ix->lv[l].n > total_cap) break;
        cols += ix->lv[l].n;
        lmin = l;
    }
    if (lmin == 0) return COS_OK;
    HIP_TRY(hipDeviceSynchronize());
    cos_index::TableSet t;
    auto build = [&]() -> hipError_t {
        hipError_t e = t.tcodes.alloc((size_t)cols * ix->row_stride);
        if (e == hipSuccess) e = t.tmags.alloc(cols);
        if (e == hipSuccess) e = t.tcsums.alloc(cols);
        u32 c0 = 0;
        for (u32 l = Ltop; l >= lmin && e == hipSuccess; l--) {
            ix->table_col0[l] = c0;
            e = cosdev::launch_level_table_gather(ix->d_codes, ix->d_mags, ix->row_stride, ix->lv[l].d_node_vec, ix->lv[l].n, c0, t.tcodes, t.tmags, nullptr);
            c0 += ix->lv[l].n;
        }
        if (e == hipSuccess) e = cosdev::launch_code_sums(t.tcodes, ix->row_stride, cols, t.tcsums, nullptr);
        if (e == hipSuccess) e = hipDeviceSynchronize();
        return e;
    };
    if (const hipError_t e = build(); e != hipSuccess) {
        (void)hipDeviceSynchronize();
        if (e == hipErrorOutOfMemory) {
            (void)hipGetLastError();
            return COS_OK;
        }
        ix->level_table_valid = false;
        HIP_TRY(e);
    }
    ix->d_tcodes = t.tcodes;
    ix->d_tmags = t.tmags;
    ix->d_tcsums = t.tcsums;
    ix->table_cols = cols;
    ix->table_level_min = lmin;
    ix->table_stride = ((u64)cols + 31) / 32 * 32;
    t.key = key;
    t.level_min = lmin;
    t.cols = cols;
    t.stride = ix->table_stride;
    memcpy(t.col0, ix->table_col0, sizeof(t.col0));
    ix->table_sets.push_back(std::move(t));
    return COS_OK;
}

extern "C" int32_t cos_index_set_walk_table(cos_index *ix, uint32_t max_cols, uint32_t min_queries) {
    if (!ix) return cos_fail(COS_ERR_INVALID, "null argument");
    if (max_cols > (1u << 20) && max_cols != COS_WALK_TABLE_AUTO) return cos_fail(COS_ERR_INVALID, "max_cols must be <= 2^20 (or COS_WALK_TABLE_AUTO)");
    std::lock_guard<std::mutex> g(ix->mu);
    ix->walk_table_max_cols = max_cols;
    ix->walk_table_min_B = min_queries;
    return COS_OK;
}

extern "C" int32_t cos_index_walk_table_info(cos_index *ix, uint32_t *out_level_min, uint32_t *out_cols) {
    if (!ix || !out_level_min || !out_cols) return cos_fail(COS_ERR_INVALID, "null argument");
    *out_level_min = *out_cols = 0;
    if (!graph_ready(ix)) return cos_fail(COS_ERR_NOT_READY, "index needs vectors, root and every graph level");
    int32_t rc = cos_set_device(ix);
    if (rc) return rc;
    std::lock_guard<std::mutex> g(ix->mu);
    if (walk_table_min_B(ix) == 0) return COS_OK;
    if ((rc = ensure_level_table(ix))) return rc;
    *out_level_min = ix->table_level_min;
    *out_cols = ix->table_cols;
    return COS_OK;
}

static int32_t ensure_adj_mags(cos_index *ix) {
    if (ix->adj_mag_valid) return COS_OK;
    if (!graph_ready(ix) || ix->meta.mdim != 0u) return COS_OK;
    if (cosdev::walk_rows_over_64_slots(cos_walk_plan_in(ix, 0, 0))) return COS_OK;
    HIP_TRY(hipDeviceSynchronize());
    for (u32 l = 0; l <= ix->p.num_layers; l++) {
        ix->lv[l].d_adj_mag.reset();
    }
    for (u32 l = 0; l <= ix->p.num_layers; l++) {
        LevelHost &H = ix->lv[l];
        const u32 slots = std::min(H.M, ix->p.shortlist_size);
        const hipError_t e = H.d_adj_mag.alloc((size_t)H.n * slots);
        if (e == hipErrorOutOfMemory) {
            (void)hipGetLastError();
            for (u32 k = 0; k < l; k++) ix->lv[k].d_adj_mag.reset();
            return COS_OK;
        }
        HIP_TRY(e);
        HIP_TRY(cosdev::launch_fill_adj_mag(H.d_adj_vec, ix->d_mags, H.d_adj_mag, H.n, H.M, slots, ix->own_stream));
    }
    HIP_TRY(hipStreamSynchronize(ix->own_stream));
    ix->adj_mag_valid = true;
    return COS_OK;
}

int32_t cos_prepare_walk_plans(cos_index *ix) {
    std::lock_guard<std::mutex> g(ix->mu);
    if (int32_t rc = ensure_adj_mags(ix)) return rc;
    if (ix->walk_order_min_B)
        if (int32_t rc = ensure_order_rank(ix)) return rc;
    if (walk_table_min_B(ix))
        if (int32_t rc = ensure_level_table(ix)) return rc;
    return COS_OK;
}

extern "C" int32_t cos_index_walk_order_cuts(cos_index *ix, uint32_t *out_levels, uint32_t cap, uint32_t *out_n) {
    if (!ix || !out_n || (cap && !out_levels)) return cos_fail(COS_ERR_INVALID, "null argument");
    *out_n = 0;
    if (!graph_ready(ix)) return cos_fail(COS_ERR_NOT_READY, "index needs vectors, root and every graph level");
    int32_t rc = cos_set_device(ix);
    if (rc) return rc;
    std::lock_guard<std::mutex> g(ix->mu);
    if ((rc = ensure_order_rank(ix))) return rc;
    for (u32 l : ix->order_levels) {
        if (*out_n < cap) out_levels[*out_n] = l;
        (*out_n)++;
    }
    return COS_OK;
}

struct SearchLaunch {
    cosdev::WalkPlan plan;
    u32 ef = 0, visited_mode = 0;
    bool timed = false;
    u64 tab_stride = 0;
    u32 tab_col0[cosdev::MAX_LEVELS] = {};
    const uint8_t *tcodes = nullptr;
    const float *tmags = nullptr;
    const u32 *tcsums = nullptr;
    u32 n_keys = 0, key_level[cosdev::MAX_LEVELS], key_n[cosdev::MAX_LEVELS];
    const u32 *order_rank[cosdev::MAX_LEVELS];
};

static int32_t get_workspace(cos_index *ix, void *key, hipStream_t st, u32 B, u32 top_k, bool host_api, Workspace **out, SearchLaunch *L,
                             bool chain = true) {
    std::lock_guard<std::mutex> g(ix->mu);
    std::unique_ptr<Workspace> &slot = ix->ws[key];
    if (!slot) slot.reset(new Workspace());
    Workspace *w = slot.get();
    const u32 L1 = ix->p.num_layers + 1;
    if (B > w->capB) {
        u32 cap = std::max(B, 64u);
        HIP_TRY(hipStreamSynchronize(st));
        w->capB = 0;
        w->cap_topk = 0;
        HIP_TRY(w->q_codes.alloc((size_t)cap * ix->row_stride));
        HIP_TRY(w->q_mags.alloc(cap));
        HIP_TRY(w->q_raw_mags.alloc(cap));
        HIP_TRY(w->walk_ids.alloc((size_t)cap * L1 * KEEP_SEARCH));
        HIP_TRY(w->walk_sims.alloc((size_t)cap * L1 * KEEP_SEARCH));
        HIP_TRY(w->walk_counts.alloc((size_t)cap * L1));
        HIP_TRY(w->walk_status.alloc(cap));
        HIP_TRY(w->stats.alloc((size_t)cap * 4));
        HIP_TRY(w->stats2.alloc((size_t)cap * 4));
        HIP_TRY(w->qsums.alloc(cap));
        HIP_TRY(w->tab_queue.alloc(16));
        if (ix->eng == ENG_Q2) HIP_TRY(w->qdig.alloc((size_t)cap * (ix->row_stride / 16) * 64));
        HIP_TRY(w->fin_flags.alloc((size_t)cap + 1));
        HIP_TRY(w->rerank_rows.alloc(cap));
        HIP_TRY(w->d_queries.alloc((size_t)cap * ix->p.dim));
        HIP_TRY(w->d_out_counts.alloc(cap));
        HIP_TRY(w->d_out_status.alloc(cap));
        w->capB = cap;
    }
    L->ef = ix->p.ef_search;
    L->visited_mode = ix->p.visited_mode;
    L->timed = ix->timing;
    cosdev::WalkPlanIn in = cos_walk_plan_in(ix, B, L->ef);
    in.chain = chain;
    const cosdev::WalkPlan want = cosdev::walk_plan(in);
    cosdev::WalkHave have{};
    if (want.refill_adj_mag) {
        if (int32_t rc = ensure_adj_mags(ix)) return rc;
        in.adj_mag_valid = ix->adj_mag_valid;
    }
    if (want.prepare_order) {
        if (w->order.cap < w->capB) {
            HIP_TRY(hipStreamSynchronize(st));
            HIP_TRY(cosdev::walk_order_reserve(w->order, w->capB));
        }
        if (int32_t rc = ensure_order_rank(ix)) return rc;
        have.order_buffers = w->order.cap >= B;
        have.n_order_keys = (u32)ix->order_levels.size();
        have.order_level0 = have.n_order_keys ? ix->order_levels[0] : 0u;
    }
    if (want.prepare_table) {
        if (int32_t rc = ensure_level_table(ix)) return rc;
        const size_t need = (size_t)w->capB * ix->table_stride;
        if (need > w->tab.cap) {
            const size_t budget = (size_t)cosdev::tune_or(cosdev::TUNE_WALK_TABLE_MAX_BYTES, (long long)48 << 30);
            HIP_TRY(hipStreamSynchronize(st));
            ix->table_bytes_total -= w->tab.cap * 4;
            w->tab.reset();
            if (ix->table_bytes_total + need * 4 <= budget) {
                if (const hipError_t e = w->tab.alloc(need); e == hipSuccess)
                    ix->table_bytes_total += need * 4;
                else if (e == hipErrorOutOfMemory)
                    (void)hipGetLastError();
                else
                    HIP_TRY(e);
            }
        }
        have.table_level_min = ix->level_table_valid ? ix->table_level_min : 0u;
        have.table_cols = ix->table_cols;
        have.table_buffer = w->tab && (size_t)B * ix->table_stride <= w->tab.cap;
    }
    L->plan = cosdev::walk_plan(in, &have);
    if (L->plan.use_table) {
        L->tab_stride = ix->table_stride;
        memcpy(L->tab_col0, ix->table_col0, sizeof(L->tab_col0));
        L->tcodes = ix->d_tcodes;
        L->tmags = ix->d_tmags;
        L->tcsums = ix->d_tcsums;
    }
    if (L->plan.ordered)
        for (u32 l : ix->order_levels) {
            L->key_level[L->n_keys] = l;
            L->key_n[L->n_keys] = ix->order_rank_n[l];
            L->order_rank[L->n_keys++] = ix->d_order_rank[l];
        }
    if (host_api && (size_t)top_k * w->capB > (size_t)w->cap_topk * w->capB) {
        w->cap_topk = 0;
        HIP_TRY(w->d_out_ids.alloc((size_t)w->capB * top_k));
        HIP_TRY(w->d_out_scores.alloc((size_t)w->capB * top_k));
        w->cap_topk = top_k;
    }
    if (w->ev.empty()) {
        w->ev.assign((size_t)Workspace::EV_RING * Workspace::EV_PER, nullptr);
        for (auto &e : w->ev) HIP_TRY(hipEventCreate(&e));
    }
    if (!w->walk_done) HIP_TRY(hipEventCreateWithFlags(&w->walk_done, hipEventDisableTiming));
    if (!w->walk_fin) HIP_TRY(hipEventCreateWithFlags(&w->walk_fin, hipEventDisableTiming));
    if (!w->last_range) HIP_TRY(hipEventCreateWithFlags(&w->last_range, hipEventDisableTiming));
    if (!w->upper_done) HIP_TRY(hipEventCreateWithFlags(&w->upper_done, hipEventDisableTiming));
    *out = w;
    return COS_OK;
}

static int32_t run_search(cos_index *ix, Workspace *w, const SearchLaunch &L, const float *d_queries, u32 B, u32 top_k, u32 *d_out_ids,
                          float *d_out_scores, u32 *d_out_counts, int32_t *d_out_status, bool do_finalize, hipStream_t st,
                          hipStream_t st_fin = nullptr, hipEvent_t walk_ev = nullptr) {
    const cosdev::WalkPlan &plan = L.plan;
    const bool timed = L.timed, ordered = plan.ordered, chained = plan.chained;
    const u32 ef = L.ef, n_keys = L.n_keys;
    IndexDev dev = cos_make_index_dev(ix);
    dev.visited_mode = L.visited_mode;
    for (u32 l = 0; l <= dev.num_layers; l++)
        if (!((plan.use_adj_mag >> l) & 1u)) dev.lv[l].adj_mag = nullptr;
    WalkArgs wa;
    memset(&wa, 0, sizeof(wa));
    if (dev.visited_mode == COS_VISITED_EXACT) {
        int32_t rc = vis_tab_prepare(w->vis, ix, B, ef, st, wa);
        if (rc) return rc;
    }
    hipEvent_t *ev = &w->ev[(size_t)(w->ev_count % Workspace::EV_RING) * Workspace::EV_PER];
    if (timed) HIP_TRY(hipEventRecord(ev[0], st));
    HIP_TRY(launch_quantize_rows(ix->eng, d_queries, ix->p.dim, B, ix->p.dim, ix->p.range_lo, ix->p.range_hi, w->q_codes, ix->row_stride,
                                 w->q_mags, w->q_raw_mags, st, plan.use_table && ix->eng == ENG_U8 ? w->qsums.p : nullptr));
    if (plan.use_table) {
        auto table_part = [&](hipEvent_t cos_index::*handle_ev, hipEvent_t own_ev, hipEvent_t *marks, u32 wgs, bool first) -> int32_t {
            if (plan.table_waits_for_sort) {
                std::lock_guard<std::mutex> g(ix->chain_mu);
                if (ix->*handle_ev && ix->*handle_ev != own_ev) HIP_TRY(hipStreamWaitEvent(st, ix->*handle_ev, 0));
            }
            if (timed) HIP_TRY(hipEventRecord(marks[0], st));
            HIP_TRY(cosdev::launch_level_table(ix->eng, w->q_codes, w->q_mags, w->qsums, w->qdig, B, L.tcodes, L.tmags, L.tcsums, ix->row_stride, plan.table_cols,
                                               w->tab, L.tab_stride, ix->n_cus, st, w->tab_queue, wgs, first, plan.table_waits_for_sort));
            if (timed) HIP_TRY(hipEventRecord(marks[1], st));
            return COS_OK;
        };
        if (cosdev::level_table_gemm_queue(ix->eng, ix->row_stride)) HIP_TRY(hipMemsetAsync(w->tab_queue, 0, sizeof(u32), st));
        if (plan.table_early_wgs) {
            if (int32_t rc = table_part(&cos_index::chain_upper_ev, w->upper_done, ev + 4, plan.table_early_wgs, true)) return rc;
            if (int32_t rc = table_part(&cos_index::chain_ev, w->walk_done, ev + 8, 0u, false)) return rc;
        } else if (int32_t rc = table_part(&cos_index::chain_last_range_ev, w->last_range, ev + 4, 0u, true))
            return rc;
    }
    if (timed) HIP_TRY(hipEventRecord(ev[1], st));
    wa.qcodes = w->q_codes;
    wa.qmags = w->q_mags;
    wa.B = B;
    wa.ef = ef;
    wa.keep = KEEP_SEARCH;
    wa.out_ids = w->walk_ids;
    wa.out_sims = w->walk_sims;
    wa.out_counts = w->walk_counts;
    wa.out_status = w->walk_status;
    wa.out_stats = w->stats;
    wa.out_stats2 = w->stats2;
    HIP_TRY(hipMemsetAsync(w->stats2, 0, (size_t)B * 32, st));
    if (plan.use_table) {
        wa.tab = w->tab;
        wa.tab_mags = L.tmags;
        wa.tab_stride = L.tab_stride;
        wa.tab_level_min = plan.table_level_min;
        memcpy(wa.tab_col0, L.tab_col0, sizeof(L.tab_col0));
    }
    hipStream_t sw = st;
    if (plan.side_stream) {
        if (!w->walk_stream) {
            int lo = 0, hi = 0;
            HIP_TRY(hipDeviceGetStreamPriorityRange(&lo, &hi));
            HIP_TRY(hipStreamCreateWithPriority(&w->walk_stream, hipStreamNonBlocking, lo));
            HIP_TRY(hipEventCreateWithFlags(&w->prep_done, hipEventDisableTiming));
        }
        sw = w->walk_stream;
        HIP_TRY(hipEventRecord(w->prep_done, st));
        HIP_TRY(hipStreamWaitEvent(sw, w->prep_done, 0));
    }
    auto walk = [&](hipStream_t s) -> int32_t {
        if (!ordered) {
            if (chained) HIP_TRY(hipEventRecord(w->upper_done, s));
            if (chained) HIP_TRY(hipEventRecord(w->last_range, s));
            HIP_TRY(launch_walk(ix->eng, dev, wa, plan.kernel, s));
            return COS_OK;
        }
        wa.phase = 1;
        wa.entry0 = w->order.entry0;
        wa.order_key = w->order.order_key;
        wa.order_iota = w->order.iota;
        u32 first = dev.num_layers;
        for (u32 i = 0; i <= n_keys; i++) {
            const bool last = i == n_keys;
            wa.level_first = first;
            wa.level_last = last ? 0u : L.key_level[i];
            wa.key_n = last ? 0u : L.key_n[i];
            wa.order_rank = last ? nullptr : L.order_rank[i];
            if (last && chained) HIP_TRY(hipEventRecord(w->last_range, s));
            HIP_TRY(launch_walk(ix->eng, dev, wa, plan.kernel, s));
            if (last) break;
            if (chained && i == 0) HIP_TRY(hipEventRecord(w->upper_done, s));
            if (timed && i == 0) HIP_TRY(hipEventRecord(ev[6], s));
            HIP_TRY(cosdev::launch_walk_order(w->order, B, L.key_n[i], ix->num_xcd, s));
            if (timed && i == 0) HIP_TRY(hipEventRecord(ev[7], s));
            wa.q_order = w->order.q_order;
            first = L.key_level[i] - 1;
        }
        return COS_OK;
    };
    if (chained) {
        std::lock_guard<std::mutex> g(ix->chain_mu);
        if (ix->chain_ev && ix->chain_ev != w->walk_done) HIP_TRY(hipStreamWaitEvent(sw, ix->chain_ev, 0));
        if (timed) HIP_TRY(hipEventRecord(ev[1], sw));
        if (int32_t rc = walk(sw)) return rc;
        HIP_TRY(hipEventRecord(w->walk_done, sw));
        ix->chain_ev = w->walk_done;
        ix->chain_last_range_ev = w->last_range;
        ix->chain_upper_ev = w->upper_done;
    } else {
        if (timed && sw != st) HIP_TRY(hipEventRecord(ev[1], sw));
        if (int32_t rc = walk(sw)) return rc;
    }
    if (timed) HIP_TRY(hipEventRecord(ev[2], sw));
    hipStream_t sf = st_fin ? st_fin : st;
    if (sf != sw) {
        hipEvent_t we = walk_ev ? walk_ev : w->walk_fin;
        HIP_TRY(hipEventRecord(we, sw));
        HIP_TRY(hipStreamWaitEvent(sf, we, 0));
    }
    if (do_finalize) {
        HIP_TRY(launch_finalize(dev, d_queries, ix->p.dim, w->q_raw_mags, w->walk_ids, w->walk_sims, w->walk_counts, w->walk_status, B, top_k,
                                d_out_ids, d_out_scores, d_out_counts, d_out_status, w->rerank_rows, sf, ordered ? w->order.q_order : nullptr, w->fin_flags));
    }
    if (timed) { HIP_TRY(hipEventRecord(ev[3], sf)); w->ev_count++; }
    w->lastB = B;
    w->timed = timed;
    w->last_plan = plan;
    { std::lock_guard<std::mutex> g(ix->mu); ix->last_ws = w; }
    return COS_OK;
}

static int32_t check_search_args(cos_index *ix, const void *q, u32 B, u32 top_k) {
    if (!ix || !q) return cos_fail(COS_ERR_INVALID, "null argument");
// ... 775 lines not shown
```

cosdata_amd/csrc/engine_internal.h:

```cpp
#pragma once
#include <hip/hip_runtime.h>

#include <atomic>
#include <condition_variable>
#include <map>
#include <memory>
#include <mutex>
#include <string>
#include <thread>
#include <vector>

#include "../../include/cosdata_hip.h"
#include "engine_types.h"
#include "tuning.h"
#include "link_types.h"
#include "dev_mem.h"
#include "walk_plan.h"

namespace cosdev {
hipError_t launch_fill_i32(int32_t *p, u64 n, int32_t v, hipStream_t st);
hipError_t launch_edge_pairs(const u32 *adj_vec, const u32 *node_vec, u32 node0, u32 cn, u32 M, u32 *px, u32 *py, hipStream_t st);
hipError_t launch_edge_keys(const u32 *adj_vec, const float *sims, const int32_t *st_in, u32 node0, u32 cn, u32 M, u32 metric, int32_t *key, int32_t *fail, hipStream_t st);
hipError_t launch_low_cache(const u32 *adj_vec, const int32_t *key, u32 n, u32 M, int32_t kmin, int32_t kmax, uint8_t *low_idx, int32_t *low_key, hipStream_t st);
hipError_t launch_unlink(const LinkArgs &a, const u32 *dn, u32 *status, hipStream_t st);
hipError_t launch_index_pair_distances(int eng, const uint8_t *codes, const float *mags, u64 row_stride, u32 nchunks, u32 dim, u32 metric, const u32 *d_pair_x,
                                       const u32 *d_pair_y, u32 n_pairs, float *d_out, int32_t *d_status, hipStream_t st);
hipError_t launch_grow_rows(const u32 *src, u32 *dst, u32 old_n, u32 new_n, u32 M, u32 remap_from, u32 remap_to, u32 fill, hipStream_t st);
hipError_t launch_grow_bytes(const uint8_t *src, uint8_t *dst, u32 old_n, u32 new_n, hipStream_t st);
hipError_t launch_fill_adj_mag(const u32 *adj_vec, const float *mags, float *adj_mag, u32 n, u32 M, u32 slots, hipStream_t st);
hipError_t launch_link_round(const LinkArgs &a, u32 maxM, const u32 *pend, const u32 *pcount, u32 *next, u32 *next_count, u32 *evq, u32 *evq_count,
                             u32 count_ub, u32 round, hipStream_t st);
hipError_t launch_quantize_rows(int eng, const float *x, u64 x_stride, u32 n, u32 dim, float lo, float hi, uint8_t *codes,
                                u64 row_stride, float *mags, float *raw_mags, hipStream_t st, u32 *code_sums = nullptr);
hipError_t launch_walk(int eng, const IndexDev &ix, const WalkArgs &wa, WalkKernel kernel, hipStream_t st);
static_assert(WALK_PLAN_MAX_LEVELS == MAX_LEVELS && WALK_PLAN_ENG_U8 == ENG_U8 && WALK_PLAN_ENG_Q2 == ENG_Q2 && WALK_PLAN_FAST_MAX_EF == WALK_FAST_MAX_EF &&
              COS_STORAGE_U8 == 0u && COS_VISITED_REF == 0u, "walk_plan.h restates these");
hipError_t launch_walk_meta(int eng, const IndexDev &ix, const WalkArgs &wa, hipStream_t st);
hipError_t launch_walk_meta_index(int eng, const IndexDev &ix, const WalkArgs &wa, hipStream_t st);
hipError_t launch_finalize(const IndexDev &ix, const float *queries, u64 q_stride, const float *q_raw_mags, const u32 *walk_ids,
                           const float *walk_sims, const u32 *walk_counts, const int32_t *walk_status, u32 B, u32 top_k,
                           u32 *out_ids, float *out_scores, u32 *out_counts, int32_t *out_status, u64 *out_rerank_rows,
                           hipStream_t st, const u32 *q_order = nullptr, u32 *slow_list = nullptr);
struct WalkOrder {
    u32 cap = 0;
    DevArr<u32> entry0;
    DevArr<u32> order_key;
    DevArr<u32> keys_sorted;
    DevArr<u32> iota, vals_sorted, q_order;
    DevBuf tmp;
};
hipError_t walk_order_reserve(WalkOrder &o, u32 B);
hipError_t launch_walk_order(WalkOrder &o, u32 B, u32 key_max, u32 num_xcd, hipStream_t st);
hipError_t launch_level_table_gather(const uint8_t *codes, const float *mags, u64 row_stride, const u32 *node_vec, u32 n, u32 col0,
                                     uint8_t *tcodes, float *tmags, hipStream_t st);
hipError_t launch_code_sums(const uint8_t *codes, u64 row_stride, u32 n, u32 *sums, hipStream_t st);
hipError_t launch_level_table(int eng, const uint8_t *qcodes, const float *qmags, const u32 *qsums, uint8_t *qdig, u32 B, const uint8_t *tcodes, const float *tmags,
                              const u32 *tcsums, u64 row_stride, u32 ncols, float *tab, u64 tab_stride, u32 n_cus, hipStream_t st, u32 *queue, u32 wgs, bool first, bool shared);
bool level_table_gemm_queue(int eng, u64 row_stride);
bool level_table_eng_supported(int eng, u64 row_stride);
int32_t quantize_ref_layout(uint32_t storage, uint32_t res, uint32_t dim, const float *x, uint32_t n, void *codes, float *mags);
int32_t distance_ref_layout(uint32_t metric, uint32_t storage, uint32_t res, uint32_t dim, const void *x_codes, const float *x_mags, uint32_t nx,
                            const void *y_codes, const float *y_mags, uint32_t ny, const uint32_t *pair_x, const uint32_t *pair_y, uint32_t n_pairs,
                            float *out, int32_t *status);
}

using cosdev::u32;
using cosdev::u64;

int32_t cos_fail(int32_t code, const char *fmt, ...);
#define HIP_TRY(expr)                                                                                  \
    do {                                                                                               \
        hipError_t _e = (expr);                                                                        \
        if (_e != hipSuccess) return cos_fail(COS_ERR_HIP, "%s: %s (%s:%d)", #expr, hipGetErrorString(_e), __FILE__, __LINE__); \
    } while (0)

namespace cosdev {
std::mutex &sparse_mutex(cos_sparse *s);
int32_t sparse_device(const cos_sparse *s);
void sparse_limits(const cos_sparse *s, u32 *max_candidates, bool *have_raw, u32 *batch_bound);
int32_t sparse_search_locked(cos_sparse *s, const uint32_t *q_dims, const float *q_vals, const uint32_t *q_offsets, u32 B, u32 top_k,
                             float early_terminate_threshold, u32 reranking_factor, u32 *d_out_ids, float *d_out_scores, u32 *d_out_counts, hipStream_t st);
}

struct LevelHost {
    std::vector<u32> node_ids;
    std::vector<u32> nbr_ids;
    DevArr<u32> d_adj_vec, d_adj_node, d_node_vec, d_child;
    DevArr<u32> d_node_id, d_node_meta;
    DevArr<float> d_adj_mag;
    u32 n = 0, M = 0;
    u32 root_idx = 0;
    bool host_valid = false;
    void release() {
        d_adj_vec.reset(); d_adj_node.reset(); d_node_vec.reset(); d_child.reset();
        d_node_id.reset(); d_node_meta.reset(); d_adj_mag.reset();
        n = 0;
        node_ids.clear();
        nbr_ids.clear();
        host_valid = false;
    }
};

struct LinkState {
    DevBuf key[cosdev::MAX_LEVELS], low_idx[cosdev::MAX_LEVELS], low_key[cosdev::MAX_LEVELS], owner[cosdev::MAX_LEVELS];
    uint64_t rng = 0;
    u32 n_built = 0;
    bool valid = false;
    void release() {
        for (int l = 0; l < cosdev::MAX_LEVELS; l++) { key[l].reset(); low_idx[l].reset(); low_key[l].reset(); owner[l].reset(); }
        valid = false;
    }
};

struct VisTab {
    DevArr<u32> bits, log;
    bool zeroed = false;
};
int32_t vis_tab_prepare(VisTab &vt, const cos_index *ix, u32 B, u32 ef, hipStream_t st, cosdev::WalkArgs &wa);

struct Workspace {
    u32 capB = 0, cap_topk = 0;
    DevArr<uint8_t> q_codes;
    DevArr<float> q_mags, q_raw_mags;
    DevArr<u32> walk_ids, walk_counts;
    DevArr<float> walk_sims;
    DevArr<int32_t> walk_status;
    DevArr<u64> stats;
    DevArr<u64> stats2;
    DevArr<float> tab;
    DevArr<u32> qsums;
    DevArr<u32> tab_queue;
    DevArr<uint8_t> qdig;
    DevArr<u32> fin_flags;
    DevArr<u64> rerank_rows;
    VisTab vis;
    cosdev::WalkOrder order;
    DevArr<float> d_queries;
    DevArr<u32> d_out_ids, d_out_counts;
    DevArr<float> d_out_scores;
    DevArr<int32_t> d_out_status;
    DevArr<u32> f_buf;
    static constexpr u32 EV_RING = 128;
    static constexpr u32 EV_PER = 10;
    std::vector<hipEvent_t> ev;
    u32 ev_count = 0;
    hipEvent_t walk_done = nullptr;
    hipEvent_t last_range = nullptr;
    hipEvent_t upper_done = nullptr;
    hipStream_t walk_stream = nullptr;
    hipEvent_t prep_done = nullptr, walk_fin = nullptr;
    u32 lastB = 0;
    bool timed = false;
    cosdev::WalkPlan last_plan{};
    Workspace() = default;
    Workspace(const Workspace &) = delete;
    ~Workspace() {
        for (hipEvent_t e : {walk_done, walk_fin, last_range, upper_done, prep_done}) if (e) (void)hipEventDestroy(e);
        for (hipEvent_t e : ev) if (e) (void)hipEventDestroy(e);
        if (walk_stream) (void)hipStreamDestroy(walk_stream);
    }
};

struct MetaGraph {
    u32 mdim = 0;
    std::vector<u32> node_ids;
    DevArr<int32_t> d_mbits;
    DevArr<float> d_mmags;
    std::vector<LevelHost> lv;
};

struct HostPipe {
    static constexpr u32 MAX_CHUNKS = 4;
    hipStream_t s[2] = {nullptr, nullptr}, sc = nullptr, sf = nullptr;
    hipEvent_t ev_in[MAX_CHUNKS] = {}, ev_walk[MAX_CHUNKS] = {};
    char wkey[MAX_CHUNKS] = {};
    DevArr<float> d_q;
    DevArr<u32> d_ids, d_counts;
    DevArr<float> d_scores;
    DevArr<int32_t> d_status;
    HostPipe() = default;
    HostPipe(const HostPipe &) = delete;
    ~HostPipe() {
        for (hipEvent_t e : ev_in) if (e) (void)hipEventDestroy(e);
        for (hipEvent_t e : ev_walk) if (e) (void)hipEventDestroy(e);
        for (hipStream_t st : {s[0], s[1], sc, sf}) if (st) (void)hipStreamDestroy(st);
    }
};
static constexpr u32 COS_MAX_HOST_PIPES = 32;

struct cos_index {
    cos_params p;
    int eng = -1;
    u32 n = 0;
    bool have_vectors = false, have_root = false;
    const float *d_raw = nullptr;
    DevArr<float> raw_own;
    DevArr<float> d_raw_mags;
    DevArr<uint8_t> d_codes;
    DevArr<float> d_mags;
    DevArr<u32> d_deleted;
    u64 row_stride = 0;
    u32 nchunks = 0, G = 1;
    std::vector<float> root_raw;
    std::vector<LevelHost> lv;
    u32 id_stride = 1;
    MetaGraph meta;
    hipStream_t own_stream = nullptr;
    std::mutex mu;
    std::map<void *, std::unique_ptr<Workspace>> ws;
    std::mutex pipe_mu;
    std::condition_variable pipe_cv;
    std::vector<std::unique_ptr<HostPipe>> pipes_all;
    std::vector<HostPipe *> pipes_free;
    std::atomic<int> host_calls_active{0};
    Workspace *last_ws = nullptr;
    std::mutex co_mu;
    std::condition_variable co_cv;
    std::vector<struct CoSlot *> co_slots;
    struct CoSlot *co_open = nullptr;
    u32 co_max_queries = 0, co_window_us = 0;
    u32 co_inflight = 0;
    cos_coalescing_stats co_stats{};
    bool timing = false;
    std::mutex chain_mu;
    hipEvent_t chain_ev = nullptr;
    hipEvent_t chain_last_range_ev = nullptr;
    hipEvent_t chain_upper_ev = nullptr;
    u32 chain_min_B = 16384;
    u32 walk_order_min_B = COS_WALK_ORDER_DEFAULT_MIN_B;
    u32 n_cus = 256;
    u32 num_xcd = 8;
    DevArr<u32> d_order_rank[cosdev::MAX_LEVELS];
    u32 order_rank_n[cosdev::MAX_LEVELS] = {};
    std::vector<u32> order_levels;
    bool order_rank_valid = false;
    u32 walk_table_max_cols = COS_WALK_TABLE_AUTO, walk_table_min_B = COS_WALK_TABLE_DEFAULT_MIN_B;
    size_t table_bytes_total = 0;
    bool adj_mag_valid = false;
    LinkState link;
    bool level_table_valid = false;
    u32 table_level_min = 0, table_cols = 0;
    u64 table_built_for_key = 0;
    u64 table_stride = 0;
    u32 table_col0[cosdev::MAX_LEVELS] = {};
    const uint8_t *d_tcodes = nullptr;
    const float *d_tmags = nullptr;
    const u32 *d_tcsums = nullptr;
    struct TableSet { u64 key; u32 level_min, cols; u64 stride; u32 col0[cosdev::MAX_LEVELS]; DevArr<uint8_t> tcodes; DevArr<float> tmags; DevArr<u32> tcsums; };
    std::vector<TableSet> table_sets;
    u32 walk_side_min_B = 4096;
    u32 lat_max_B = COS_LATENCY_MODE_DEFAULT_MAX_B;
    u32 lat4_max_B = COS_LATENCY_WAVES_DEFAULT_MAX_B;
    struct FlatWs *flat_ws = nullptr;
};


struct FlatWs;
void cos_flat_ws_release(cos_index *ix);
hipError_t cos_deleted_reset(cos_index *ix, u32 n, hipStream_t st);
hipError_t cos_deleted_grow(cos_index *ix, u32 n0, u32 n1, hipStream_t st);
hipError_t cos_deleted_mark(cos_index *ix, const u32 *ids, u32 m, hipStream_t st);
void cos_coalesce_release(cos_index *ix);
cosdev::IndexDev cos_make_index_dev(const cos_index *ix);
cosdev::IndexDev cos_make_meta_dev(const cos_index *ix);
int32_t cos_set_device(const cos_index *ix);
cosdev::WalkPlanIn cos_walk_plan_in(const cos_index *ix, u32 B, u32 ef);
int32_t cos_prepare_walk_plans(cos_index *ix);
void cos_meta_free_levels(cos_index *ix);
```

cosdata_amd/csrc/engine_types.h:

```cpp
#pragma once
#include <stdint.h>
#include "device_common.h"

namespace cosdev {

struct LevelDev {
    const u32 *adj_vec;
    const u32 *adj_node;
    const u32 *node_vec;
    const u32 *child;
    u32 n;
    u32 M;
    u32 root_idx;
    const float *adj_mag;
    u32 mag_stride;
    const u32 *node_id;
    const u32 *node_meta;
};

struct IndexDev {
    const uint8_t *codes;
    const float *mags;
    const float *raw;
    const float *raw_mags;
    u64 row_stride;
    u64 raw_stride;
    u32 n;
    u32 dim;
    u32 metric;
    u32 storage;
    u32 num_layers;
    u32 shortlist;
    u32 visited_mode;
    u32 nchunks;
    u32 G;
    u32 id_base;
    u32 id_stride;
    const int32_t *mbits;
    const float *mmags;
    u32 mdim;
    LevelDev lv[MAX_LEVELS];
};

struct WalkArgs {
    const uint8_t *qcodes;
    const float *qmags;
    const u32 *q_rows;
    const u32 *self_ids;
    u32 *vis_bits;
    u32 *vis_log;
    u32 vis_words_per_query;
    u32 vis_log_cap;
    u32 B;
    u32 ef;
    u32 keep;
    u32 *out_ids;
    float *out_sims;
    u32 *out_nodes;
    u32 *out_counts;
    int32_t *out_status;
    const int32_t *f_dims;
    const float *f_mags;
    const u32 *f_off;
    u64 *out_stats;
    u64 *out_stats2;
    const float *tab;
    const float *tab_mags;
    u64 tab_stride;
    u32 tab_level_min;
    u32 tab_col0[MAX_LEVELS];
    u32 no_self_seed;
    u32 smem_mmax;
    u32 smem_win_bytes;
    u32 merge_min;
    u32 phase;
    u32 level_first, level_last;
    u32 key_n;
    const u32 *order_rank;
    const u32 *q_order;
    u32 *entry0;
    u32 *order_key;
    u32 *order_iota;
};

constexpr u32 WALK_FAST_MAX_EF = 1024u;
constexpr u32 WALK_GENERAL_MAX_EF = 16384u;

}
```

cosdata_amd/csrc/kernels_link.hip:

```cpp
#include <hip/hip_runtime.h>

#include <algorithm>

#include "engine_types.h"
#include "link_types.h"

using namespace cosdev;

namespace {

constexpr u32 NONE = 0xFFFFFFFFu;
constexpr int32_t EMPTY_KEY = INT32_MIN;

template <typename T>
__device__ __forceinline__ T ld(const T *p) { return __hip_atomic_load(p, __ATOMIC_RELAXED, __HIP_MEMORY_SCOPE_AGENT); }
template <typename T>
__device__ __forceinline__ void st(T *p, T v) { __hip_atomic_store(p, v, __ATOMIC_RELAXED, __HIP_MEMORY_SCOPE_AGENT); }
template <typename T>
__device__ __forceinline__ u32 ld_uniform_u32(const T *p, int lane) {
    u32 v = 0;
    if (lane == 0) v = (u32)ld(p);
    return readlane_u32(v, 0);
}

// ... 299 lines not shown
        }
        orphan = orphan || (found && !other);
    }
    if (__builtin_amdgcn_ballot_w64(orphan)) { if (lane == 0) status[level] = 1; return; }
    for (u32 s = lane; s < M; s += 64) {
        const u64 o = (u64)node * M + s;
        const u32 x = ld(&lv.adj_node[o]);
        if (x == NONE) continue;
        for (u32 j = 0; j < M; j++) {
            const u64 ox = (u64)x * M + j;
            if (ld(&lv.adj_node[ox]) == node) {
                st(&lv.adj_node[ox], NONE);
                if (lv.adj_vec != lv.adj_node) st(&lv.adj_vec[ox], NONE);
                st(&lv.key[ox], EMPTY_KEY);
                break;
            }
        }
        st(&lv.adj_node[o], NONE);
        if (lv.adj_vec != lv.adj_node) st(&lv.adj_vec[o], NONE);
        st(&lv.key[o], EMPTY_KEY);
    }
    if (lane == 0) status[level] = 2;
}

__global__ void edge_pairs_kernel(const u32 *__restrict__ adj_vec, const u32 *__restrict__ node_vec, u32 node0, u64 total, u32 M, u32 *__restrict__ px, u32 *__restrict__ py) {
    for (u64 i = (u64)blockIdx.x * blockDim.x + threadIdx.x; i < total; i += (u64)gridDim.x * blockDim.x) {
        const u32 node = node0 + (u32)(i / M);
        const u32 self = node_vec ? node_vec[node] : node;
        const u32 v = adj_vec[(u64)node0 * M + i];
        px[i] = self;
        py[i] = v == NONE ? self : v;
    }
}
__global__ void edge_keys_kernel(const u32 *__restrict__ adj_vec, const float *__restrict__ sims, const int32_t *__restrict__ st_in, u32 node0, u64 total, u32 M, u32 metric,
                                 int32_t *__restrict__ key, int32_t *__restrict__ fail) {
    for (u64 i = (u64)blockIdx.x * blockDim.x + threadIdx.x; i < total; i += (u64)gridDim.x * blockDim.x) {
        const u64 o = (u64)node0 * M + i;
        const bool empty = adj_vec[o] == NONE;
        if (!empty && st_in[i] != 0) atomicMax(fail, st_in[i]);
        key[o] = empty ? EMPTY_KEY : order_key(metric, sims[i]);
    }
}
__global__ void low_cache_kernel(const u32 *__restrict__ adj_vec, const int32_t *__restrict__ key, u32 n, u32 M, int32_t kmin, int32_t kmax, uint8_t *__restrict__ low_idx,
                                 int32_t *__restrict__ low_key) {
    for (u64 i = (u64)blockIdx.x * blockDim.x + threadIdx.x; i < n; i += (u64)gridDim.x * blockDim.x) {
        u32 nl = 0;
        int32_t nk = kmax;
        for (u32 j = 0; j < M; j++) {
            if (adj_vec[i * M + j] == NONE) { nl = j; nk = kmin; break; }
            const int32_t k = key[i * M + j];
            if (k < nk) { nk = k; nl = j; }
        }
        low_idx[i] = (uint8_t)nl;
        low_key[i] = nk;
    }
}

__global__ void grow_rows_kernel(const u32 *__restrict__ src, u32 *__restrict__ dst, u32 old_n, u32 new_n, u32 M, u32 remap_from, u32 remap_to, u32 fill) {
    const u64 total = (u64)new_n * M;
    for (u64 i = (u64)blockIdx.x * blockDim.x + threadIdx.x; i < total; i += (u64)gridDim.x * blockDim.x) {
        const u64 row = i / M;
        const u32 col = (u32)(i - row * M);
        u32 v = fill;
        if (row + 1 < old_n) v = src[row * M + col];
        else if (row + 1 == new_n) v = src[(u64)(old_n - 1) * M + col];
        else { dst[i] = fill; continue; }
        dst[i] = v == remap_from ? remap_to : v;
    }
}
__global__ void grow_bytes_kernel(const uint8_t *__restrict__ src, uint8_t *__restrict__ dst, u32 old_n, u32 new_n) {
    for (u64 i = (u64)blockIdx.x * blockDim.x + threadIdx.x; i < new_n; i += (u64)gridDim.x * blockDim.x)
        dst[i] = i + 1 < old_n ? src[i] : (i + 1 == new_n ? src[old_n - 1] : (uint8_t)0);
}

__global__ void fill_adj_mag_kernel(const u32 *__restrict__ adj_vec, const float *__restrict__ mags, float *__restrict__ adj_mag, u64 total, u32 M, u32 slots) {
    for (u64 i = (u64)blockIdx.x * blockDim.x + threadIdx.x; i < total; i += (u64)gridDim.x * blockDim.x) {
        const u64 node = i / slots;
        const u32 slot = (u32)(i - node * slots);
        const u32 v = adj_vec[node * M + slot];
        adj_mag[i] = v == NONE ? 1.0f : mags[v];
    }
}

}

namespace cosdev {

hipError_t launch_fill_i32(int32_t *p, u64 n, int32_t v, hipStream_t st) {
    if (n == 0) return hipSuccess;
    const u32 blocks = (u32)std::min<u64>((n + 255) / 256, 65535);
    hipLaunchKernelGGL(fill_i32_kernel, dim3(blocks), dim3(256), 0, st, p, n, v);
    return hipGetLastError();
}

hipError_t launch_edge_pairs(const u32 *adj_vec, const u32 *node_vec, u32 node0, u32 cn, u32 M, u32 *px, u32 *py, hipStream_t st) {
    const u64 total = (u64)cn * M;
    if (!total) return hipSuccess;
    hipLaunchKernelGGL(edge_pairs_kernel, dim3((u32)std::min<u64>((total + 255) / 256, 1u << 20)), dim3(256), 0, st, adj_vec, node_vec, node0, total, M, px, py);
    return hipGetLastError();
}
hipError_t launch_edge_keys(const u32 *adj_vec, const float *sims, const int32_t *st_in, u32 node0, u32 cn, u32 M, u32 metric, int32_t *key, int32_t *fail, hipStream_t st) {
    const u64 total = (u64)cn * M;
    if (!total) return hipSuccess;
    hipLaunchKernelGGL(edge_keys_kernel, dim3((u32)std::min<u64>((total + 255) / 256, 1u << 20)), dim3(256), 0, st, adj_vec, sims, st_in, node0, total, M, metric, key, fail);
    return hipGetLastError();
}
hipError_t launch_low_cache(const u32 *adj_vec, const int32_t *key, u32 n, u32 M, int32_t kmin, int32_t kmax, uint8_t *low_idx, int32_t *low_key, hipStream_t st) {
    if (!n) return hipSuccess;
    hipLaunchKernelGGL(low_cache_kernel, dim3((u32)std::min<u64>(((u64)n + 255) / 256, 1u << 20)), dim3(256), 0, st, adj_vec, key, n, M, kmin, kmax, low_idx, low_key);
    return hipGetLastError();
}
hipError_t launch_unlink(const LinkArgs &a, const u32 *dn, u32 *status, hipStream_t st) {
    hipLaunchKernelGGL(unlink_kernel, dim3(a.L1), dim3(64), 0, st, a, dn, status);
    return hipGetLastError();
}
hipError_t launch_grow_rows(const u32 *src, u32 *dst, u32 old_n, u32 new_n, u32 M, u32 remap_from, u32 remap_to, u32 fill, hipStream_t st) {
    const u64 total = (u64)new_n * M;
    if (total == 0 || old_n == 0) return hipErrorInvalidValue;
    const u32 blocks = (u32)std::min<u64>((total + 255) / 256, 1u << 20);
    hipLaunchKernelGGL(grow_rows_kernel, dim3(blocks), dim3(256), 0, st, src, dst, old_n, new_n, M, remap_from, remap_to, fill);
    return hipGetLastError();
}
hipError_t launch_grow_bytes(const uint8_t *src, uint8_t *dst, u32 old_n, u32 new_n, hipStream_t st) {
    if (new_n == 0 || old_n == 0) return hipErrorInvalidValue;
    const u32 blocks = (u32)std::min<u64>(((u64)new_n + 255) / 256, 1u << 20);
    hipLaunchKernelGGL(grow_bytes_kernel, dim3(blocks), dim3(256), 0, st, src, dst, old_n, new_n);
    return hipGetLastError();
}

hipError_t launch_fill_adj_mag(const u32 *adj_vec, const float *mags, float *adj_mag, u32 n, u32 M, u32 slots, hipStream_t st) {
    const u64 total = (u64)n * slots;
    if (total == 0) return hipSuccess;
    const u32 blocks = (u32)std::min<u64>((total + 255) / 256, 1u << 20);
    hipLaunchKernelGGL(fill_adj_mag_kernel, dim3(blocks), dim3(256), 0, st, adj_vec, mags, adj_mag, total, M, slots);
    return hipGetLastError();
}

hipError_t launch_link_round(const LinkArgs &a, u32 maxM, const u32 *pend, const u32 *pcount, u32 *next, u32 *next_count, u32 *evq, u32 *evq_count,
                             u32 count_ub, u32 round, hipStream_t st) {
    if (count_ub == 0) return hipSuccess;
    const u64 threads = (u64)count_ub * (KEEP_INDEX + 1);
    hipLaunchKernelGGL(claim_kernel, dim3((u32)((threads + 255) / 256)), dim3(256), 0, st, a, pend, pcount, next_count, evq_count, round);
    if (maxM <= 64) hipLaunchKernelGGL(link_kernel<1>, dim3(count_ub), dim3(64), 0, st, a, pend, pcount, next, next_count, evq, evq_count, round);
    else if (maxM <= 128) hipLaunchKernelGGL(link_kernel<2>, dim3(count_ub), dim3(64), 0, st, a, pend, pcount, next, next_count, evq, evq_count, round);
    else hipLaunchKernelGGL(link_kernel<4>, dim3(count_ub), dim3(64), 0, st, a, pend, pcount, next, next_count, evq, evq_count, round);
    const u32 eblocks = std::min<u32>(1024u, std::max<u32>(1u, count_ub / 2u));
    hipLaunchKernelGGL(evict_kernel, dim3(eblocks), dim3(256), 0, st, a, evq, evq_count);
    return hipGetLastError();
}

}
```

cosdata_amd/csrc/kernels_sparse.hip:

```cpp
#include <hip/hip_runtime.h>
#include <hipcub/hipcub.hpp>

#include <algorithm>
#include <cstdlib>
#include <cstring>
#include <mutex>
#include <vector>

#include "engine_internal.h"
#include "postings_update.h"
#include "topk_select.h"

using namespace cosdev;

namespace {

constexpr u32 SEL = 64;
constexpr u32 SEL_MAX = 1024;

struct SparseDev {
    const u32 *dims;
    const u64 *key_off;
    const u32 *vec_ids;
    const u64 *row_off;
// ... 926 lines not shown

static int32_t sparse_launch(cos_sparse *s, const SparseBatch &sb, u32 *d_oi, float *d_os, u32 *d_oc, hipStream_t st) {
    const u32 B = sb.B, R = sb.R, splits = sb.splits, Q = 1u << s->bits;
    const SparseImage im(B, sb.nq);
    HIP_TRY(s->w_in.grow(im.bytes));
    HIP_TRY(s->w_part.grow((size_t)B * splits * SEL * R * 8));
    unsigned char *d = s->w_in.p;
    const STerm *d_terms = (const STerm *)d;
    const u32 *d_qd = (const u32 *)(d + im.qd), *d_qo = (const u32 *)(d + im.qo), *d_qt_off = (const u32 *)(d + im.qt_off), *d_order = (const u32 *)(d + im.order);
    const float *d_qv = (const float *)(d + im.qv);
    u64 *d_part = s->w_part.as<u64>();
    HIP_TRY(hipMemcpyAsync(d, s->h_in.p, im.bytes, hipMemcpyHostToDevice, st));
    SparseDev dev{nullptr, nullptr, nullptr, s->d_row_off, s->d_raw_dims, s->d_raw_vals, s->T, Q, s->n, s->bits, s->upper};
    HIP_TRY(hipEventRecord(s->ev0, st));
    if (R > 1) {
        auto wide = R == 2 ? sparse_launch_wide<2> : R == 4 ? sparse_launch_wide<4> : R == 8 ? sparse_launch_wide<8> : sparse_launch_wide<16>;
        HIP_TRY(wide(s, dev, B, splits, d_terms, d_qt_off, d_order, d_part, d_qd, d_qv, d_qo, sb.top_k, sb.kwr, sb.rerank, d_oi, d_os, d_oc, st));
    } else {
        if (s->packed)
            hipLaunchKernelGGL(sparse_packed_kernel<8>, dim3(B * splits), dim3(256), 0, st, s->d_pk.p, d_terms, d_qt_off, s->n, s->d_tile_dir.p, d_order, splits, d_part);
        else
            hipLaunchKernelGGL(sparse_tile_kernel<1>, dim3(B * splits), dim3(256), 0, st, s->d_ids.p, s->d_keys.p, d_terms, d_qt_off, s->n, s->d_tile_dir.p, d_order, splits,
                               d_part);
        HIP_TRY(hipGetLastError());
        hipLaunchKernelGGL(sparse_finish_kernel, dim3(B), dim3(64), 0, st, dev, d_part, splits, d_qd, d_qv, d_qo, sb.top_k, sb.kwr, sb.rerank, d_oi, d_os, d_oc);
        HIP_TRY(hipGetLastError());
    }
    HIP_TRY(hipEventRecord(s->ev1, st));
    s->stats_pending = true;
    return COS_OK;
}

static int32_t sparse_search_on_stream(cos_sparse *s, const uint32_t *q_dims, const float *q_vals, const uint32_t *q_offsets, u32 B, u32 top_k,
                                       float early_terminate_threshold, u32 reranking_factor, u32 *d_oi, float *d_os, u32 *d_oc, hipStream_t st) {
    HIP_TRY(hipSetDevice(s->device));
    int32_t rc = sparse_wait_previous(s);
    if (rc) return rc;
    SparseBatch sb;
    rc = sparse_resolve(s, q_dims, q_vals, q_offsets, B, top_k, early_terminate_threshold, reranking_factor, sb);
    if (rc) return rc;
    return sparse_launch(s, sb, d_oi, d_os, d_oc, st);
}

namespace cosdev {
std::mutex &sparse_mutex(cos_sparse *s) { return s->mu; }
int32_t sparse_device(const cos_sparse *s) { return s->device; }
void sparse_limits(const cos_sparse *s, u32 *max_candidates, bool *have_raw, u32 *batch_bound) {
    *max_candidates = s->max_cand;
    *have_raw = s->have_raw;
    *batch_bound = SPK_COUNTED;
}
int32_t sparse_search_locked(cos_sparse *s, const uint32_t *q_dims, const float *q_vals, const uint32_t *q_offsets, u32 B, u32 top_k,
                             float early_terminate_threshold, u32 reranking_factor, u32 *d_out_ids, float *d_out_scores, u32 *d_out_counts, hipStream_t st) {
    return sparse_search_on_stream(s, q_dims, q_vals, q_offsets, B, top_k, early_terminate_threshold, reranking_factor, d_out_ids, d_out_scores, d_out_counts, st);
}
}

extern "C" int32_t cos_sparse_search_batch_device(cos_sparse *s, const uint32_t *q_dims, const float *q_vals, const uint32_t *q_offsets, uint32_t B,
                                                  uint32_t top_k, float early_terminate_threshold, uint32_t reranking_factor, uint32_t *d_out_ids,
                                                  float *d_out_scores, uint32_t *d_out_counts, void *stream) {
    if (!s || !q_dims || !q_vals || !q_offsets || !d_out_ids || !d_out_scores || !d_out_counts || B == 0 || top_k == 0) return cos_fail(COS_ERR_INVALID, "bad argument");
    std::lock_guard<std::mutex> guard(s->mu);
    return sparse_search_on_stream(s, q_dims, q_vals, q_offsets, B, top_k, early_terminate_threshold, reranking_factor, d_out_ids, d_out_scores, d_out_counts,
                                   (hipStream_t)stream);
}

extern "C" int32_t cos_sparse_search_batch(cos_sparse *s, const uint32_t *q_dims, const float *q_vals, const uint32_t *q_offsets, uint32_t B, uint32_t top_k,
                                           float early_terminate_threshold, uint32_t reranking_factor, uint32_t *out_ids, float *out_scores,
                                           uint32_t *out_counts) {
    if (!s || !q_dims || !q_vals || !q_offsets || !out_ids || !out_scores || !out_counts || B == 0 || top_k == 0) return cos_fail(COS_ERR_INVALID, "bad argument");
    std::lock_guard<std::mutex> guard(s->mu);
    int32_t rc = sparse_admit(s, B, top_k, reranking_factor);
    if (rc) return rc;
    HIP_TRY(hipSetDevice(s->device));
    HIP_TRY(s->w_oi.grow((size_t)B * top_k * 4));
    HIP_TRY(s->w_os.grow((size_t)B * top_k * 4));
    HIP_TRY(s->w_oc.grow((size_t)B * 4));
    rc = sparse_search_on_stream(s, q_dims, q_vals, q_offsets, B, top_k, early_terminate_threshold, reranking_factor, s->w_oi.as<u32>(), s->w_os.as<float>(),
                                 s->w_oc.as<u32>(), 0);
    if (rc) return rc;
    HIP_TRY(hipMemcpy(out_ids, s->w_oi.p, (size_t)B * top_k * 4, hipMemcpyDeviceToHost));
    HIP_TRY(hipMemcpy(out_scores, s->w_os.p, (size_t)B * top_k * 4, hipMemcpyDeviceToHost));
    HIP_TRY(hipMemcpy(out_counts, s->w_oc.p, (size_t)B * 4, hipMemcpyDeviceToHost));
    return sparse_wait_previous(s);
}

extern "C" int32_t cos_sparse_layout(cos_sparse *s, uint32_t *packed) {
    if (!s || !packed) return cos_fail(COS_ERR_INVALID, "null argument");
    *packed = s->packed ? 1u : 0u;
    return COS_OK;
}

extern "C" int32_t cos_sparse_set_max_candidates(cos_sparse *s, uint32_t max_candidates) {
    if (!s) return cos_fail(COS_ERR_INVALID, "null argument");
    if (max_candidates == 0 || max_candidates > SEL_MAX) return cos_fail(COS_ERR_INVALID, "max_candidates must be in [1, %u]", SEL_MAX);
    u32 w = SEL;
    while (w < max_candidates) w *= 2;
    std::lock_guard<std::mutex> guard(s->mu);
    s->max_cand = w;
    return COS_OK;
}

extern "C" int32_t cos_sparse_max_candidates(cos_sparse *s, uint32_t *out) {
    if (!s || !out) return cos_fail(COS_ERR_INVALID, "null argument");
    std::lock_guard<std::mutex> guard(s->mu);
    *out = s->max_cand;
    return COS_OK;
}

extern "C" int32_t cos_sparse_last_stats(cos_sparse *s, cos_sparse_search_stats *out) {
    if (!s || !out) return cos_fail(COS_ERR_INVALID, "null argument");
    std::lock_guard<std::mutex> guard(s->mu);
    HIP_TRY(hipSetDevice(s->device));
    const int32_t rc = sparse_wait_previous(s);
    if (rc) return rc;
    *out = s->last;
    return COS_OK;
}

namespace {

constexpr size_t SPAD_UNPACKED = 64 * SPU, SPAD_PACKED = 1;

__device__ __forceinline__ u32 spk_word(u32 id, u32 key) { return key << 24 | (id + 1u); }

template <bool PACKED>
struct SparseIds {
    const u32 *__restrict__ a;
    __device__ __forceinline__ u32 operator()(u64 p) const { return PACKED ? (a[p] & 0xFFFFFFu) - 1u : a[p]; }
};

__global__ __launch_bounds__(256) void sparse_delta_kernel(const u32 *__restrict__ pair_id, const float *__restrict__ vals, u32 np, float upper, u32 bits,
                                                           u64 *__restrict__ out) {
    const u32 i = blockIdx.x * blockDim.x + threadIdx.x;
    if (i >= np) return;
    out[i] = (u64)pair_id[i] << 8 | sparse_quantize(vals[i], upper, bits);
}

template <bool PACKED>
struct SparseMerge {
    const u32 *__restrict__ old_a;
    const uint8_t *__restrict__ old_keys;
    const u64 *__restrict__ delta;
    u32 *__restrict__ new_a;
    uint8_t *__restrict__ new_keys;
    struct P { u32 a, ky; };
    __device__ __forceinline__ P zero() const { return {0u, 0u}; }
    __device__ __forceinline__ P from_old(u64 p) const { return {old_a[p], PACKED ? 0u : (u32)old_keys[p]}; }
    __device__ __forceinline__ P from_delta(u64 p) const {
        const u64 v = delta[p];
        return {PACKED ? spk_word((u32)(v >> 8), (u32)v & 255u) : (u32)(v >> 8), (u32)v & 255u};
    }
    __device__ __forceinline__ void store4(u64 j, const P (&v)[4]) const {
        *reinterpret_cast<uint4 *>(new_a + j) = make_uint4(v[0].a, v[1].a, v[2].a, v[3].a);
        if (!PACKED) *reinterpret_cast<u32 *>(new_keys + j) = v[0].ky | v[1].ky << 8 | v[2].ky << 16 | v[3].ky << 24;
    }
    __device__ __forceinline__ void store1(u64 j, const P &v) const {
        new_a[j] = v.a;
        if (!PACKED) new_keys[j] = (uint8_t)v.ky;
    }
};

template <bool PACKED>
__global__ __launch_bounds__(256) void sparse_claim_kernel(const u32 *__restrict__ a, const uint8_t *__restrict__ keys, const u32 *__restrict__ pair_id_key ,
                                                           const u64 *__restrict__ pair_begin, const u32 *__restrict__ pair_len, u32 np,
                                                           u32 *__restrict__ flags, uint8_t *__restrict__ found) {
// ... 405 lines not shown
```

cosdata_amd/csrc/tuning.h:

```cpp
#pragma once
#include <cstdint>

namespace cosdev {

enum TuneKey : int {
    TUNE_WALK_CHAIN_MIN_B,
    TUNE_WALK_ORDER_MIN_B,
    TUNE_WALK_SIDE_MIN_B,
    TUNE_WALK_SPLIT_LEVELS,
    TUNE_WALK_TABLE_COLS,
    TUNE_WALK_TABLE_MIN_B,
    TUNE_WALK_TABLE_MAX_BYTES,
    TUNE_WALK_TABLE_GEMM,
    TUNE_HOST_PIPELINE_MIN_B,
    TUNE_FLAT_UNFUSED,
    TUNE_FLAT_TILE_KERNEL,
    TUNE_FLAT_PF,
    TUNE_FLAT_FP4,
    TUNE_BM25_BLOCKS,
    TUNE_SPARSE_LAYOUT,
    TUNE_WALK_PB,
    TUNE_WALK_PB_UPPER,
    TUNE_WALK_LAT,
    TUNE_WALK_LAT4,
    TUNE_WALK_SMALL_TABLE_TK,
    TUNE_WALK_LAT_WARM,
    TUNE_WALK_LAT_LA,
    TUNE_WALK_LAT4_E,
    TUNE_FINALIZE_FAST,
    TUNE_SHARDSET_FORCE_RCCL,
    TUNE_BUILD_PROFILE,
    TUNE_WALK_MERGE_MIN,
    TUNE_WALK_ADJ_MAG,
    TUNE_WALK_TABLE_RULE_C,
    TUNE_WALK_TABLE_AFTER_SORT,
    TUNE_WALK_UPPER_LDS_PAD,
    TUNE_WALK_R2,
    TUNE_FINALIZE_WIDE_MAX_B,
    TUNE_FLAT_FP4_W8,
    TUNE_WALK_TABLE_EARLY_WGS,
    TUNE_COUNT
};

constexpr long long TUNE_UNSET = INT64_MIN;

long long tune(TuneKey k);
inline long long tune_or(TuneKey k, long long dflt) {
    const long long v = tune(k);
    return v == TUNE_UNSET ? dflt : v;
}

}
```

cosdata_amd/csrc/tuning.hip:

```cpp
#include <atomic>
#include <cstdlib>
#include <cstring>
#include <mutex>

#include "engine_internal.h"
#include "tuning.h"

namespace cosdev {
namespace {

const char *const NAMES[TUNE_COUNT] = {
    "walk_chain_min_b", "walk_order_min_b", "walk_side_min_b", "walk_split_levels", "walk_table_cols", "walk_table_min_b",
    "walk_table_max_bytes", "walk_table_gemm", "host_pipeline_min_b", "flat_unfused", "flat_tile_kernel", "flat_pf", "flat_fp4",
    "bm25_blocks", "sparse_layout", "walk_pb", "walk_pb_upper", "walk_lat", "walk_lat4", "walk_small_table_tk", "walk_lat_warm",
    "walk_lat_la", "walk_lat4_e", "finalize_fast", "shardset_force_rccl", "build_profile",
    "walk_merge_min", "walk_adj_mag", "walk_table_rule_c", "walk_table_after_sort", "walk_upper_lds_pad", "walk_r2", "finalize_wide_max_b", "flat_fp4_w8",
    "walk_table_early_wgs",
};
std::atomic<long long> g_values[TUNE_COUNT];
std::once_flag g_once;

int find_key(const char *name, size_t len) {
    for (int k = 0; k < TUNE_COUNT; k++)
        if (strlen(NAMES[k]) == len && strncmp(NAMES[k], name, len) == 0) return k;
    return -1;
}

void init_once() {
    std::call_once(g_once, [] {
        for (auto &v : g_values) v.store(TUNE_UNSET, std::memory_order_relaxed);
        const char *e = getenv("COS_TUNING");
        while (e && *e) {
            const char *end = strchr(e, ',');
            const size_t item = end ? (size_t)(end - e) : strlen(e);
            const char *eq = (const char *)memchr(e, '=', item);
            if (eq) {
                const int k = find_key(e, (size_t)(eq - e));
                char *stop = nullptr;
                const long long v = strtoll(eq + 1, &stop, 10);
                if (k >= 0 && stop != eq + 1) g_values[k].store(v, std::memory_order_relaxed);
            }
            e = end ? end + 1 : nullptr;
        }
    });
}

}

long long tune(TuneKey k) {
    init_once();
    return g_values[k].load(std::memory_order_relaxed);
}

}

using namespace cosdev;

extern "C" int32_t cos_tuning_set(const char *name, int64_t value) {
    if (!name) return cos_fail(COS_ERR_INVALID, "null knob name");
    const int k = find_key(name, strlen(name));
    if (k < 0) return cos_fail(COS_ERR_INVALID, "unknown tuning knob '%s'", name);
    if (value == TUNE_UNSET) return cos_fail(COS_ERR_INVALID, "INT64_MIN is the 'unset' marker: use cos_tuning_clear");
    init_once();
    g_values[k].store(value, std::memory_order_relaxed);
    return COS_OK;
}

extern "C" int32_t cos_tuning_clear(const char *name) {
    init_once();
    if (!name) {
        for (auto &v : g_values) v.store(TUNE_UNSET, std::memory_order_relaxed);
        return COS_OK;
    }
    const int k = find_key(name, strlen(name));
    if (k < 0) return cos_fail(COS_ERR_INVALID, "unknown tuning knob '%s'", name);
    g_values[k].store(TUNE_UNSET, std::memory_order_relaxed);
    return COS_OK;
}

extern "C" int32_t cos_tuning_get(const char *name, int64_t *out_value, int32_t *out_is_set) {
    if (!name || !out_value || !out_is_set) return cos_fail(COS_ERR_INVALID, "null argument");
    const int k = find_key(name, strlen(name));
    if (k < 0) return cos_fail(COS_ERR_INVALID, "unknown tuning knob '%s'", name);
    const long long v = tune((TuneKey)k);
    *out_is_set = v != TUNE_UNSET;
    *out_value = v == TUNE_UNSET ? 0 : v;
    return COS_OK;
}
```

cosdata_amd/csrc/walk_kernel.inc:

```
constexpr int PB = 4;
constexpr int LA = 4;

struct WalkSmem {
    u32 *vis;
    u64 *res;
    u32 *wl_vec;
    u32 *wl_node;
    u32 *win_vec;
    u32 *win_node;
    float *win_mag;
    float *qf;
};

template <int ENG, int CH, int R, bool G64, bool EXACT, int PB64 = 4>
__global__ __launch_bounds__(64) __attribute__((amdgpu_waves_per_eu(CH >= 3 ? (R <= 4 ? (CH == 3 ? 4 : 3) : (CH == 3 ? 3 : 2)) : (R == 1 ? ((ENG == ENG_U8 && CH == 1 && G64 && !EXACT) ? 7 : 6) : (R <= 4 ? 5 : 4)), 8))) void walk_kernel(const IndexDev ix, const WalkArgs wa) {
    extern __shared__ __attribute__((aligned(16))) unsigned char smem_raw[];
    const int lane = threadIdx.x;
    if (blockIdx.x >= wa.B) return;
    const u32 qi = wa.q_order ? wa.q_order[blockIdx.x] : blockIdx.x;
    const bool resume = wa.phase != 0u && wa.level_first < ix.num_layers;
    if (resume && wa.out_status[qi] != COS_OK) return;

    const u32 Mmax = wa.smem_mmax;
    WalkSmem sm;
// ... 44 lines not shown
    } else {
        const float *qg = (const float *)qcode;
        for (u32 i = lane; i < (u32)(ix.row_stride / 4); i += 64) sm.qf[i] = qg[i];
        __builtin_amdgcn_s_waitcnt(0);
#pragma unroll
        for (int c = 0; c < CH; c++) qreg[c] = make_uint4(0, 0, 0, 0);
    }

    u32 loff64[CH];
#pragma unroll
    for (int c = 0; c < CH; c++) {
        const u32 chunk = (u32)lane + (u32)c * 64u;
        loff64[c] = (chunk < ix.nchunks ? chunk : 0u) * 16u;
    }

    u64 n_evals = 0, n_exp = 0, adj_bytes = 0, n_rounds = 0, n_tab = 0;
    const u32 merge_min = uniform_u32(wa.merge_min);
    int32_t status = COS_OK;
    u32 entry = uniform_u32(resume ? wa.entry0[qi] : ix.lv[L].root_idx);
    const int level_first = wa.phase ? (int)wa.level_first : (int)L, level_last = wa.phase ? (int)wa.level_last : 0;
    u32 order_key = wa.key_n;

    auto single_distance = [&](u32 row, float &sim_out) -> bool {
        float dotf;
        if constexpr (!FLOAT_ENG) {
            dotf = (float)int_row_dot_group0<ENG, CH>(qreg, ix.codes + (u64)row * ix.row_stride, ix.nchunks, lig, grp, G);
        } else if constexpr (ENG == ENG_F16) {
            float d = f16_lane_dot(ix.codes + (u64)row * ix.row_stride, sm.qf, ix.dim);
            dotf = __uint_as_float(readlane_u32(__float_as_uint(d), 0));
        } else {
            float d = f32_oct_dot((const float *)(ix.codes + (u64)row * ix.row_stride), sm.qf, ix.dim, lane & 7);
            dotf = __uint_as_float(readlane_u32(__float_as_uint(d), 0));
        }
        bool bad;
        sim_out = cosine_or_dot(metric, dotf, qmag, uniform_f32(ix.mags[row]), bad);
        return !bad;
    };

    for (int level = level_first; level >= level_last; level--) {
        const LevelDev lv = ix.lv[level];
        const u32 M = lv.M;
        const u32 slots = M < ix.shortlist ? M : ix.shortlist;
        const u32 bitmask = 64u * M - 1u;
        const u32 out_slot = L - (u32)level;
        u32 nlog = 0;
        const bool tab_level = TABLE_OK && wa.tab != nullptr && (u32)level >= wa.tab_level_min;
        const float *tabq = wa.tab + (u64)qi * wa.tab_stride + wa.tab_col0[level];
        const float *tabm = wa.tab_mags + wa.tab_col0[level];

        if (!exact) {
            vis_clear<64>(sm.vis, M, lane);
            if (lane == 0 && wa.no_self_seed == 0u) vis_set_bit(sm.vis, self_id & bitmask);
        }

        Pool<R> pool;
        pool.clear();
        u32 npool = 0, npop = 0;
        u32 res_lo = 0, res_hi = 0;

        {
            const u32 erow = uniform_u32(lv.node_vec ? lv.node_vec[entry] : entry);
            float s0;
            if (tab_level) {
                bool bad;
                s0 = cosine_or_dot(metric, uniform_f32(tabq[entry]), qmag, uniform_f32(tabm[entry]), bad);
                if (bad) { status = COS_ERR_CALCULATION; break; }
            } else if (!single_distance(erow, s0)) { status = COS_ERR_CALCULATION; break; }
            if (lane == 0) {
                if (!exact) vis_set_bit(sm.vis, vis_bit_of(erow, N, ix.id_stride, bitmask));
                else {
                    atomicOr(&vis[entry >> 5], 1u << (entry & 31));
                    vlog[0] = entry >> 5;
                }
            }
            pool.insert_at(pack_key(metric_key(metric, s0), entry), 0, lane);
            npool = 1;
            if (exact) nlog = 1;
        }

        u32 failed = 0;
        u32 lev_evals = 1;
        const u32 log2M = (u32)__ffs((int)M) - 1u;
        const u64 slotmask = slots >= 64u ? ~0ull : ((1ull << slots) - 1ull);
        auto level_rounds = [&](auto tabc, auto cosc, auto amagc) __attribute__((always_inline)) {
        constexpr bool TAB = decltype(tabc)::value;
        constexpr bool COSINE = decltype(cosc)::value;
        constexpr bool AMAG = decltype(amagc)::value && G64 && !FLOAT_ENG;
        const u32 metric_t = COSINE ? 0u : metric;
        while (npool > 0 && npop < wa.ef) {
            n_rounds++;
            u32 kwin = npool < (u32)LA ? npool : (u32)LA;
            if (kwin > wa.ef - npop) kwin = wa.ef - npop;
            u32 wv_[LA], wn_[LA];
            {
                const u32 slot_l = (u32)lane < slots ? (u32)lane : slots - 1u;
                auto fetch_stage = [&](auto bothc) {
                    constexpr bool BOTH = decltype(bothc)::value;
                    float wm_[LA];
                    static_for<0, LA>([&](auto ic) {
                        constexpr int i = decltype(ic)::value;
                        const u32 nd = pool.template peek_node<i>();
                        const u64 off = ((u64)nd << log2M) + slot_l;
                        wv_[i] = lv.adj_vec[off];
                        if constexpr (BOTH) wn_[i] = lv.adj_node[off];
                        if constexpr (!TAB && AMAG) wm_[i] = lv.adj_mag[(u64)nd * lv.mag_stride + slot_l];
                    });
                    if constexpr (!TAB) {
                        static_for<0, LA>([&](auto ic) {
                            constexpr int i = decltype(ic)::value;
                            sm.win_vec[i * 64 + lane] = wv_[i];
                            sm.win_node[i * 64 + lane] = BOTH ? wn_[i] : wv_[i];
                            if constexpr (AMAG) sm.win_mag[i * 64 + lane] = wm_[i];
                        });
                    }
                };
                if (TAB || level != 0) fetch_stage(std::true_type{});
                else fetch_stage(std::false_type{});
            }
            u32 stop = 0;
            auto consume = [&](u32 wi, u32 nb_vec, u32 nb_node, float nb_mag) __attribute__((always_inline)) {
                if constexpr (R == 1) {
                    const u64 hd = pool.head();
                    res_lo = writelane_dyn(res_lo, (u32)hd, (int)npop);
                    res_hi = writelane_dyn(res_hi, (u32)(hd >> 32), (int)npop);
                } else if (lane == 0) sm.res[npop] = pool.e[0];
                pool.pop_head(lane);
                npool--;
                npop++;
                const int limit = (int)wa.ef - (int)npop;
                const int ahead = (int)kwin - 1 - (int)wi;
                u32 window_ok = 1;

                const u64 vmask = ballot64(nb_vec != ROW_EMPTY) & slotmask;
                u64 wmask;
                if (!exact) {
                    u32 bit = vis_bit_of(nb_vec, N, 1u, bitmask);
                    if (ix.id_stride != 1u) {
                        asm volatile("");
                        bit = vis_bit_of(nb_vec, N, ix.id_stride, bitmask);
                    }
                    const u32 word = bit >> 5, msk = 1u << (bit & 31);
                    u32 seen = sm.vis[word];
                    asm volatile("" : "+v"(seen));
                    const u64 cmask = vmask & ballot64((seen & msk) == 0u);
                    wmask = cmask;
                    if (cmask) {
                    u32 old = 0;
                    if (__builtin_amdgcn_inverse_ballot_w64(cmask)) old = atomicOr(&sm.vis[word], msk);
                    wmask = vis_alias_winners(cmask, bit, cmask & ballot64((old & msk) != 0u));
                    }
                } else {
                    u32 w = 0;
                    if (__builtin_amdgcn_inverse_ballot_w64(vmask)) w = __hip_atomic_load(&vis[nb_node >> 5], __ATOMIC_RELAXED, __HIP_MEMORY_SCOPE_AGENT);
                    wmask = vmask & ballot64(((w >> (nb_node & 31)) & 1u) == 0u);
                    if (__builtin_amdgcn_inverse_ballot_w64(wmask)) {
                        atomicOr(&vis[nb_node >> 5], 1u << (nb_node & 31));
                        vlog[nlog + (u32)__popcll(wmask & ((1ull << lane) - 1ull))] = nb_node >> 5;
                    }
                    nlog += (u32)__popcll(wmask);
                }
                if (wmask) {
                const bool win = __builtin_amdgcn_inverse_ballot_w64(wmask);
                const int W = __popcll(wmask);
                lev_evals += (u32)W;
                auto insert_serial = [&](u64 pm, u32 keyv, u32 nodev) {
                    while (pm) {
                        const int p = __ffsll((long long)pm) - 1;
                        pm = clear_bit_u64(pm, p);
                        const u64 kk = pack_key(readlane_u32(keyv, p), readlane_u32(nodev, p));
                        const int pos = pool.rank_of(kk);
                        if (pos < limit) {
                            pool.insert_at(kk, pos, lane);
                            npool = npool + 1u < (u32)(64 * R) ? npool + 1u : (u32)(64 * R);
                            window_ok = pos < ahead ? 0u : window_ok;
                        }
                    }
                };
                auto commit = [&](u64 leadmask, u32 keyv, u32 nodev) {
                    const u64 bar = limit > 0 ? pool.peek_dyn((u32)(limit - 1)) : ~0ull;
                    insert_serial(leadmask & ballot64(pack_key(keyv, nodev) > bar), keyv, nodev);
                };
                auto commit_merge = [&](u64 leadmask, u32 keyv, u32 nodev) {
                    const u64 bar = limit > 0 ? pool.peek_dyn((u32)(limit - 1)) : ~0ull;
                    const u64 mykey = pack_key(keyv, nodev);
                    const u64 pm = leadmask & ballot64(mykey > bar);
                    const u32 Wp = (u32)__popcll(pm);
                    if (Wp < merge_min) { insert_serial(pm, keyv, nodev); return; }
                    u32 below[R];
#pragma unroll
                    for (int r = 0; r < R; r++) below[r] = 0u;
                    u32 posv = 0u;
                    u32 abovev = 0u;
                    u32 minrank = ~0u;
                    u64 m = pm;
                    while (m) {
                        const int p = __ffsll((long long)m) - 1;
                        m = clear_bit_u64(m, p);
                        const u64 kk = pack_key(readlane_u32(keyv, p), readlane_u32(nodev, p));
                        u32 rank = 0;
#pragma unroll
                        for (int r = 0; r < R; r++) {
                            const bool gt = pool.e[r] > kk;
                            rank += (u32)__popcll(ballot64(gt));
                            below[r] += gt ? 1u : 0u;
                        }
                        minrank = rank < minrank ? rank : minrank;
                        abovev += kk > mykey ? 1u : 0u;
                        posv = writelane_dyn(posv, rank, p);
                    }
                    window_ok = (int)minrank < ahead ? 0u : window_ok;
                    u64 *mg = (u64 *)sm.win_vec;
#pragma unroll
                    for (int r = 0; r < R; r++) {
                        u32 np = (u32)lane * R + r + (Wp - below[r]);
                        np = np < (u32)(64 * R) ? np : (u32)(64 * R);
                        mg[np] = pool.e[r];
                    }
                    if (__builtin_amdgcn_inverse_ballot_w64(pm)) {
                        u32 np = posv + abovev;
                        np = np < (u32)(64 * R) ? np : (u32)(64 * R);
                        mg[np] = mykey;
                    }
                    __builtin_amdgcn_fence(__ATOMIC_RELEASE, "wavefront");
                    __builtin_amdgcn_wave_barrier();
                    __builtin_amdgcn_fence(__ATOMIC_ACQUIRE, "wavefront");
#pragma unroll
                    for (int r = 0; r < R; r++) pool.e[r] = mg[(u32)lane * R + r];
                    npool = npool + Wp < (u32)(64 * R) ? npool + Wp : (u32)(64 * R);
                };
                if constexpr (TAB) {
                    float simv = 0.0f, magv = 1.0f;
                    if (win) { simv = tabq[nb_node]; magv = tabm[nb_node]; }
                    bool badl;
                    simv = cosine_or_dot<ENG == ENG_U8>(metric_t, simv, qmag, magv, badl);
                    if (wmask & ballot64(badl)) failed = 1;
                    else if constexpr (R <= 4) {
                        if (merge_min != 0u) commit_merge(wmask, metric_key(metric_t, simv), nb_node);
                        else commit(wmask, metric_key(metric_t, simv), nb_node);
                    } else commit(wmask, metric_key(metric_t, simv), nb_node);
                } else if constexpr (G64 && !FLOAT_ENG) {
                    float magw = 1.0f;
                    if constexpr (AMAG) magw = nb_mag;
                    else if (win) magw = ix.mags[nb_vec];
                    u64 m = wmask;
                    while (m && !failed) {
                        u32 lsel = 0;
                        u32 tot = 0;
                        u64 leadmask = 0;
                        auto eval_block = [&](auto npc) {
                            constexpr int NP = decltype(npc)::value;
                            constexpr int LS = 64 / NP;
                            uint4 buf[NP][CH];
                            int cnt = 0;
                            static_for<0, NP>([&](auto pc) {
                                constexpr int p = decltype(pc)::value;
                                if (m) {
                                    const int l = __ffsll((long long)m) - 1;
                                    m = clear_bit_u64(m, l);
                                    const uint8_t *rp = row_ptr_scalar(ix.codes, readlane_u32(nb_vec, l), (u32)ix.row_stride);
                                    lsel = writelane_u32<p * LS>(lsel, (u32)l << 2);
#pragma unroll
                                    for (int c = 0; c < CH; c++) {
                                        u32 lo = loff64[c];
                                        asm("" : "+v"(lo));
                                        buf[p][c] = *(const uint4 *)(rp + lo);
                                    }
                                    cnt++;
                                }
                            });
                            u32 acc[NP];
                            static_for<0, NP>([&](auto pc) {
                                constexpr int p = decltype(pc)::value;
                                acc[p] = 0;
                                if (p < cnt) {
                                    asm volatile("");
#pragma unroll
                                    for (int c = 0; c < CH; c++) acc[p] = chunk_dot<ENG>(qreg[c], buf[p][c], acc[p]);
                                }
                            });
                            tot = wave_reduce_rows<NP>(acc);
                            constexpr u64 firsts = NP == 8 ? 0x0101010101010101ull : 0x0001000100010001ull;
                            leadmask = cnt == NP ? firsts : firsts & ((1ull << (cnt * LS)) - 1ull);
                        };
                        if constexpr (PB64 == 8) {
                            if (__popcll(m) > 4) eval_block(std::integral_constant<int, 8>{});
                            else eval_block(std::integral_constant<int, 4>{});
                        } else {
                            eval_block(std::integral_constant<int, 4>{});
                        }
                        const float magv = __uint_as_float((u32)__builtin_amdgcn_ds_bpermute((int)lsel, (int)__float_as_uint(magw)));
                        const u32 nodev = (u32)__builtin_amdgcn_ds_bpermute((int)lsel, (int)nb_node);
                        const float dotv = (float)tot;
                        bool badl;
                        const float sim = cosine_or_dot<ENG == ENG_U8>(metric, dotv, qmag, magv, badl);
                        if (leadmask & ballot64(badl)) { failed = 1; break; }
                        commit(leadmask, metric_key(metric, sim), nodev);
                    }
                } else {
                if (win) {
                    const int rank = __popcll(wmask & ((1ull << lane) - 1ull));
                    sm.wl_vec[rank] = nb_vec;
                    sm.wl_node[rank] = nb_node;
                }

                for (int base = 0; base < W; base += RP * PB) {
                    u32 prow[PB];
                    float pmag[PB];
                    uint4 buf[PB][CH];
                    float fdot[PB];
#pragma unroll
                    for (int p = 0; p < PB; p++) {
                        if (base + p * RP >= W) break;
                        const int my = base + p * RP + grp;
                        const bool v = my < W;
                        prow[p] = v ? sm.wl_vec[my] : 0u;
                        pmag[p] = 1.0f;
                        if (v) pmag[p] = ix.mags[prow[p]];
                        if constexpr (!FLOAT_ENG) {
#pragma unroll
                            for (int c = 0; c < CH; c++) {
                                u32 chunk = (u32)lig + (u32)c * (u32)G;
                                buf[p][c] = make_uint4(0, 0, 0, 0);
                                if (v && chunk < ix.nchunks) buf[p][c] = *(const uint4 *)(ix.codes + (u64)prow[p] * ix.row_stride + (u64)chunk * 16);
                            }
                        }
                    }
                    if constexpr (FLOAT_ENG) {
#pragma unroll
                        for (int p = 0; p < PB; p++) {
                            if (base + p * RP >= W) break;
                            if constexpr (ENG == ENG_F32)
                                fdot[p] = f32_oct_dot((const float *)(ix.codes + (u64)prow[p] * ix.row_stride), sm.qf, ix.dim, lane & 7);
                            else
                                fdot[p] = f16_lane_dot(ix.codes + (u64)prow[p] * ix.row_stride, sm.qf, ix.dim);
                        }
                    }
#pragma unroll
                    for (int p = 0; p < PB; p++) {
                        if (base + p * RP >= W) break;
                        float dotf;
                        if constexpr (!FLOAT_ENG) {
                            u32 acc = 0;
#pragma unroll
                            for (int c = 0; c < CH; c++) acc = chunk_dot<ENG>(qreg[c], buf[p][c], acc);
                            acc = group_reduce_add_u32(acc, G);
                            dotf = (float)acc;
                        } else {
                            dotf = fdot[p];
                        }
                        const int mine = base + p * RP + grp;
                        const bool leadg = lig == 0 && mine < W;
                        bool badl;
                        const float sim = cosine_or_dot(metric, dotf, qmag, pmag[p], badl);
                        if (ballot64(mine < W && badl)) { failed = 1; break; }
                        const u32 mynode = leadg ? sm.wl_node[mine] : 0u;
                        commit(ballot64(leadg), metric_key(metric, sim), mynode);
                    }
                    if (failed) break;
                }
                }
                stop = failed | (window_ok ^ 1u);
                }
            };
            if constexpr (TAB) {
                static_for<0, LA>([&](auto ic) __attribute__((always_inline)) {
                    constexpr int i = decltype(ic)::value;
                    if ((u32)i < kwin && !stop) consume((u32)i, wv_[i], wn_[i], 1.0f);
                });
            } else {
                for (u32 wi = 0; wi < kwin && !stop; wi++)
                    consume(wi, sm.win_vec[wi * 64 + lane], sm.win_node[wi * 64 + lane], AMAG ? sm.win_mag[wi * 64 + lane] : 1.0f);
            }
            if (failed) break;
        }
        };
        if (tab_level) {
            if (metric == 0u) level_rounds(std::true_type{}, std::true_type{}, std::false_type{});
            else level_rounds(std::true_type{}, std::false_type{}, std::false_type{});
        } else {
            bool done = false;
            if constexpr (G64 && !FLOAT_ENG) {
                if (lv.adj_mag != nullptr) {
                    level_rounds(std::false_type{}, std::false_type{}, std::true_type{});
                    done = true;
                }
            }
            if (!done) level_rounds(std::false_type{}, std::false_type{}, std::false_type{});
        }
        n_exp += npop;
        adj_bytes += (u64)npop * slots * 4;
        n_evals += lev_evals;
        if (tab_level) n_tab += lev_evals;
        if (exact) {
            __atomic_signal_fence(__ATOMIC_SEQ_CST);
            __builtin_amdgcn_s_waitcnt(0);
            for (u32 i = lane; i < nlog; i += 64) {
                const u32 w = __hip_atomic_load(&vlog[i], __ATOMIC_RELAXED, __HIP_MEMORY_SCOPE_AGENT);
                __hip_atomic_store(&vis[w], 0u, __ATOMIC_RELAXED, __HIP_MEMORY_SCOPE_AGENT);
            }
            __atomic_signal_fence(__ATOMIC_SEQ_CST);
            __builtin_amdgcn_s_waitcnt(0);
        }
        if (failed) { status = COS_ERR_CALCULATION; break; }

        u64 rk[R];
#pragma unroll
        for (int r = 0; r < R; r++) {
            const u32 e = (u32)lane * R + r;
            if constexpr (R == 1) rk[r] = e < npop ? pack_key(res_hi, res_lo) : 0ull;
            else rk[r] = e < npop ? sm.res[e] : 0ull;
        }
        bitonic_sort_desc<R>(rk, lane);
        u32 cnt = npop < wa.keep ? npop : wa.keep;
        if (npop == 0) {
            const u32 erow = uniform_u32(lv.node_vec ? lv.node_vec[entry] : entry);
            float s0;
            if (!single_distance(erow, s0)) { status = COS_ERR_CALCULATION; break; }
            rk[0] = lane == 0 ? pack_key(metric_key(metric, s0), entry) : 0ull;
            cnt = 1;
        }
        const u64 obase = level_list_base(ix, wa, qi, out_slot);
#pragma unroll
        for (int r = 0; r < R; r++) {
            const u32 e = (u32)lane * R + r;
            if (e < cnt) {
                const u32 nd = (u32)rk[r];
                const u32 vrow = lv.node_vec ? lv.node_vec[nd] : nd;
                wa.out_ids[obase + e] = vrow == N ? COS_ROOT_ID : vrow * ix.id_stride;
                wa.out_sims[obase + e] = metric_key_inv(metric, (u32)(rk[r] >> 32));
                if (wa.out_nodes) wa.out_nodes[obase + e] = nd;
            }
        }
        if (lane == 0) wa.out_counts[(u64)qi * (L + 1) + out_slot] = cnt;
        if (level > 0) {
            const u32 best = (u32)readlane_u64(rk[0], 0);
            entry = uniform_u32(lv.child[best]);
            if (wa.phase != 0u && level == level_last) order_key = uniform_u32(wa.order_rank[best]);
        }
    }

    if (lane == 0) {
        wa.out_status[qi] = status;
        if (wa.phase != 0u && level_last > 0) {
            wa.entry0[qi] = entry;
            wa.order_key[qi] = status == COS_OK ? order_key : wa.key_n;
            wa.order_iota[qi] = qi;
        }
        if (wa.out_stats) {
            const bool add = resume;
            wa.out_stats[(u64)qi * 4 + 0] = n_evals + (add ? wa.out_stats[(u64)qi * 4 + 0] : 0ull);
            wa.out_stats[(u64)qi * 4 + 1] = n_exp + (add ? wa.out_stats[(u64)qi * 4 + 1] : 0ull);
            wa.out_stats[(u64)qi * 4 + 2] = adj_bytes + (add ? wa.out_stats[(u64)qi * 4 + 2] : 0ull);
            wa.out_stats[(u64)qi * 4 + 3] = n_rounds + (add ? wa.out_stats[(u64)qi * 4 + 3] : 0ull);
        }
        if (wa.out_stats2) {
            if (resume || wa.phase == 0u) {
                wa.out_stats2[(u64)qi * 4 + 0] = n_evals;
                wa.out_stats2[(u64)qi * 4 + 1] = n_exp;
                wa.out_stats2[(u64)qi * 4 + 2] = adj_bytes;
            }
            wa.out_stats2[(u64)qi * 4 + 3] = n_tab + (resume ? wa.out_stats2[(u64)qi * 4 + 3] : 0ull);
        }
    }
}
```

cosdata_amd/csrc/walk_plan.h:

```cpp
#pragma once
#include <algorithm>
#include <cstdint>

namespace cosdev {

constexpr int WALK_PLAN_MAX_LEVELS = 16;
constexpr int WALK_PLAN_ENG_U8 = 0, WALK_PLAN_ENG_Q2 = 1;
constexpr uint32_t WALK_PLAN_FAST_MAX_EF = 1024u;

constexpr uint32_t ADJ_MAG_REFILL_MIN_B = 1024u, ADJ_MAG_USE_MIN_B = 4096u;

enum class WalkKernel : uint8_t {
    General,
    Throughput,
    Lat1,
    Lat4
};

struct WalkPlanIn {
    int eng;
    uint32_t storage;
    uint32_t nchunks, G;
    uint32_t num_layers, M[WALK_PLAN_MAX_LEVELS], shortlist, visited_mode, mdim;
    uint32_t B, ef;
    bool chain;
    bool no_self_seed;
    uint32_t lat_max_B, lat4_max_B;
    bool small_table_tk;
    uint32_t adj_mag_mode;
    uint32_t table_min_B;
    uint32_t order_min_B, chain_min_B, side_min_B;
    long long table_after_sort;
    bool table_supported;
    bool adj_mag_valid;
    uint32_t table_early_wgs;
    bool table_queue;
    uint32_t n_cus;
};

struct WalkHave {
    uint32_t table_level_min, table_cols;
    bool table_buffer;
    uint32_t n_order_keys, order_level0;
    bool order_buffers;
};

struct WalkPlan {
    WalkKernel kernel;
    bool ordered;
    bool use_table;
    bool table_waits_for_sort;
    uint32_t table_early_wgs;
    uint32_t use_adj_mag;
    bool refill_adj_mag;
    bool chained;
    bool side_stream;
    bool prepare_order, prepare_table;
    uint32_t table_level_min, table_cols, cut_after_level;
};

inline uint32_t table_gemm_stripe_tiles(uint32_t B, uint32_t cols, uint32_t n_cus, bool shared) {
    const uint32_t n_tiles = (cols + 63u) / 64u, row_groups = (B + 255u) / 256u, cus = n_cus ? n_cus : 256u;
    if (!shared) {
        const uint32_t groups = std::max(1u, cus / std::max(1u, std::min(row_groups, cus)));
        return std::max(1u, (n_tiles + groups - 1u) / groups);
    }
    const uint64_t units = (uint64_t)n_tiles * row_groups;
    return (uint32_t)std::min<uint64_t>(64u, std::max<uint64_t>(2u, units / (24ull * cus)));
}
inline uint32_t table_gemm_items(uint32_t B, uint32_t cols, uint32_t n_cus, bool shared) {
    const uint32_t n_tiles = (cols + 63u) / 64u, st = table_gemm_stripe_tiles(B, cols, n_cus, shared);
    return (uint32_t)std::min<uint64_t>(0xFFFFFFFFull, (uint64_t)((n_tiles + st - 1u) / st) * ((B + 255u) / 256u));
}

inline bool walk_rows_over_64_slots(const WalkPlanIn &in) {
    for (uint32_t l = 0; l <= in.num_layers; l++)
        if (std::min(in.M[l], in.shortlist) > 64u) return true;
    return false;
}

inline bool walk_general_needed(const WalkPlanIn &in) {
    if (in.ef > WALK_PLAN_FAST_MAX_EF) return true;
    if (in.nchunks != 0u && in.G != 0u && (in.nchunks + in.G - 1u) / in.G > (in.storage == 0u  ? 4u : 1u)) return true;
    return walk_rows_over_64_slots(in);
}

inline bool walk_latency_domain(const WalkPlanIn &in, uint32_t max_B) {
    if (max_B == 0 || in.B > max_B) return false;
    if (in.visited_mode != 0) return false;
    if (in.eng != WALK_PLAN_ENG_U8 && in.eng != WALK_PLAN_ENG_Q2) return false;
    if (in.nchunks == 0 || in.nchunks > 64u) return false;
    if (in.ef == 0 || in.ef > 256) return false;
    return true;
}

inline WalkKernel walk_fast_kernel(const WalkPlanIn &in, bool table_available) {
    if (in.no_self_seed) return WalkKernel::Throughput;
    const bool lat4 = walk_latency_domain(in, in.lat4_max_B) && std::max(in.M[0], in.M[in.num_layers]) <= 64u;
    if (table_available && in.small_table_tk && in.eng == WALK_PLAN_ENG_U8)
        return in.ef > 128u && lat4 ? WalkKernel::Lat4 : WalkKernel::Throughput;
    if (lat4) return WalkKernel::Lat4;
    if (walk_latency_domain(in, in.lat_max_B)) return WalkKernel::Lat1;
    return WalkKernel::Throughput;
}

inline WalkPlan walk_plan(const WalkPlanIn &in, const WalkHave *have = nullptr) {
    WalkPlan p{};
    const bool general = walk_general_needed(in);
    p.ordered = !general && in.order_min_B && in.B >= in.order_min_B && in.ef <= 256u && (!have || (have->n_order_keys > 0 && have->order_buffers));
    bool table = !general && in.table_min_B && (have ? have->table_level_min != 0 && have->table_buffer : in.table_supported);
    const bool table_size = in.B >= in.table_min_B || in.B <= in.lat4_max_B;
    if (general) p.kernel = WalkKernel::General;
    else if (p.ordered) {
        p.kernel = WalkKernel::Throughput;
        table = table && table_size;
    } else {
        const WalkKernel with_table = walk_fast_kernel(in, true);
        table = table && ((with_table == WalkKernel::Lat4 && in.eng == WALK_PLAN_ENG_U8) || (with_table == WalkKernel::Throughput && table_size));
        p.kernel = table ? with_table : walk_fast_kernel(in, false);
    }
    p.use_table = table;
    p.chained = in.chain && in.B >= in.chain_min_B;
    if (have && table) {
        p.table_level_min = have->table_level_min;
        p.table_cols = have->table_cols;
        p.table_waits_for_sort = p.chained && (in.table_after_sort == 2 || (in.table_after_sort == 1 && (uint64_t)have->table_cols * in.B >= (1ull << 30)));
        if (p.table_waits_for_sort && in.table_queue)
            p.table_early_wgs = std::min(in.table_early_wgs, table_gemm_items(in.B, have->table_cols, in.n_cus, true));
    }
    if (have && p.ordered) p.cut_after_level = have->order_level0;
    if (in.adj_mag_valid && in.adj_mag_mode != 0)
        for (uint32_t l = 0; l <= in.num_layers; l++)
            if (in.adj_mag_mode == 2 || (in.ef <= 2u * in.M[l] && in.B >= ADJ_MAG_USE_MIN_B)) p.use_adj_mag |= 1u << l;
    p.refill_adj_mag = !in.adj_mag_valid && in.B >= ADJ_MAG_REFILL_MIN_B;
    p.side_stream = in.side_min_B && in.B >= in.side_min_B;
    p.prepare_order = p.ordered;
    p.prepare_table = p.use_table;
    return p;
}

}
```

Before: 1.055 million.

## Reuse level table dot products for neighbours promoted from the level just below

Adds a per-slot AdjUp side table (neighbour magnitude plus its index in the level above) for the level just below the precomputed table levels. The walk kernel can then take query dot products for neighbours that also exist in the upper level straight from the level table, instead of scanning their u8 codes. This cuts distance work and code-row reads at that level, at the cost of extra device memory, a build-time fill kernel and one fewer lookahead window slot. It also moves the stats2 memset earlier on the stream and pads sparse output past the result count.

```diff
diff --git a/cosdata_amd/csrc/builder.hip b/cosdata_amd/csrc/builder.hip
--- a/cosdata_amd/csrc/builder.hip
+++ b/cosdata_amd/csrc/builder.hip
@@ -64,7 +64,7 @@
         (void)hipStreamSynchronize(ix->own_stream);
         for (auto &l : ix->lv) l.release();
         ix->link.release();
-        ix->adj_mag_valid = false;
+        ix->invalidate_adj_side();
         ix->have_root = false;
     }
 };
@@ -222,7 +222,7 @@
 
     ix->order_rank_valid = false;
     ix->level_table_valid = false;
-    ix->adj_mag_valid = false;
+    ix->invalidate_adj_side();
     ix->link.release();
     uint64_t rng = ix->p.seed ? ix->p.seed : 0x1234567ull;
     std::vector<float> root(ix->p.dim);
@@ -363,7 +363,7 @@
     GraphGuard guard{ix};
     ix->order_rank_valid = false;
     ix->level_table_valid = false;
-    ix->adj_mag_valid = false;
+    ix->invalidate_adj_side();
     ix->link.valid = false;
     cos_flat_ws_release(ix);
 
@@ -418,6 +418,7 @@
         H.host_valid = false;
         H.nbr_ids.clear();
         H.d_adj_mag.reset();
+        H.d_adj_up.reset();
         DevArr<u32> adj_vec, adj_node, node_vec, child;
         DevBuf key, low_idx, low_key;
         HIP_TRY(adj_vec.alloc((size_t)nl1 * M));
@@ -575,7 +576,7 @@
     VisTab vtab;
     std::vector<u32> h_ids((size_t)L1 * KEEP), h_nodes((size_t)L1 * KEEP), h_counts(L1), h_dn(L1), h_ust(L1);
     std::vector<std::vector<u32>> node_vec(L1);
-    ix->adj_mag_valid = false;
+    ix->invalidate_adj_side();
     for (auto &l : ix->lv) { l.host_valid = false; l.nbr_ids.clear(); }
 
     for (u32 t = 0; t < m; t++) {
diff --git a/cosdata_amd/csrc/device_common.h b/cosdata_amd/csrc/device_common.h
--- a/cosdata_amd/csrc/device_common.h
+++ b/cosdata_amd/csrc/device_common.h
@@ -10,6 +10,8 @@
 
 constexpr int WAVE = 64;
 constexpr u32 ROW_EMPTY = 0xFFFFFFFFu;
+constexpr u32 ADJ_UP_NONE = 0xFFFFFFFFu;
+struct alignas(8) AdjUp { float mag; u32 up; };
 constexpr int KEEP_SEARCH = 100;
 constexpr int KEEP_INDEX = 64;
 constexpr int MAX_LEVELS = 16;
diff --git a/cosdata_amd/csrc/engine.hip b/cosdata_amd/csrc/engine.hip
--- a/cosdata_amd/csrc/engine.hip
+++ b/cosdata_amd/csrc/engine.hip
@@ -87,6 +87,7 @@
         d.lv[l].root_idx = h.n ? h.n - 1 : 0;
         d.lv[l].adj_mag = (ix->adj_mag_valid && cosdev::tune_or(cosdev::TUNE_WALK_ADJ_MAG, 1) != 0) ? h.d_adj_mag : nullptr;
         d.lv[l].mag_stride = std::min(h.M, ix->p.shortlist_size);
+        d.lv[l].adj_up = (d.lv[l].adj_mag != nullptr && l != 0 && ix->adj_up_level == l) ? h.d_adj_up : nullptr;
     }
     return d;
 }
@@ -216,7 +217,7 @@
     for (auto &l : ix->lv) l.release();
     ix->order_rank_valid = false;
     ix->level_table_valid = false;
-    ix->adj_mag_valid = false;
+    ix->invalidate_adj_side();
     ix->link.release();
     reset_meta(ix);
     const u64 dim = ix->p.dim;
@@ -264,7 +265,7 @@
     HIP_TRY(hipStreamSynchronize(ix->own_stream));
     ix->have_root = true;
     ix->level_table_valid = false;
-    ix->adj_mag_valid = false;
+    ix->invalidate_adj_side();
     if (ix->link.valid && graph_ready(ix)) ix->link.release();
     return COS_OK;
 }
@@ -305,7 +306,7 @@
     L.host_valid = true;
     ix->order_rank_valid = false;
     ix->level_table_valid = false;
-    ix->adj_mag_valid = false;
+    ix->invalidate_adj_side();
     ix->link.release();
     return COS_OK;
 }
@@ -363,7 +364,7 @@
     L.host_valid = false;
     ix->order_rank_valid = false;
     ix->level_table_valid = false;
-    ix->adj_mag_valid = false;
+    ix->invalidate_adj_side();
     ix->link.release();
     return COS_OK;
 }
@@ -507,7 +508,7 @@
     ix->root_raw.assign(ix->p.dim, 0.0f);
     ix->have_root = true;
     ix->level_table_valid = false;
-    ix->adj_mag_valid = false;
+    ix->invalidate_adj_side();
     return COS_OK;
 }
 
@@ -680,6 +681,7 @@
     return env >= 0 ? (u32)std::min<long long>(env, 0xFFFFFFFFll) : ix->walk_table_min_B;
 }
 static constexpr long long WALK_TABLE_EARLY_WGS_DEFAULT = 0;
+static constexpr long long WALK_UP_TABLE_DEFAULT = 1;
 cosdev::WalkPlanIn cos_walk_plan_in(const cos_index *ix, u32 B, u32 ef) {
     cosdev::WalkPlanIn in{};
     in.eng = ix->eng;
@@ -706,6 +708,7 @@
     in.table_after_sort = cosdev::tune_or(cosdev::TUNE_WALK_TABLE_AFTER_SORT, 1);
     in.table_supported = cosdev::level_table_eng_supported(ix->eng, ix->row_stride);
     in.adj_mag_valid = ix->adj_mag_valid;
+    in.up_table_mode = (u32)std::min<long long>(std::max<long long>(cosdev::tune_or(cosdev::TUNE_WALK_UP_TABLE, WALK_UP_TABLE_DEFAULT), 0), 2);
     in.table_early_wgs = (u32)std::min<long long>(std::max<long long>(cosdev::tune_or(cosdev::TUNE_WALK_TABLE_EARLY_WGS, WALK_TABLE_EARLY_WGS_DEFAULT), 0), 0xFFFFFFFFll);
     in.table_queue = cosdev::level_table_gemm_queue(ix->eng, ix->row_stride);
     in.n_cus = ix->n_cus;
@@ -835,13 +838,51 @@
     return COS_OK;
 }
 
+static int32_t ensure_adj_up(cos_index *ix) {
+    const u32 want = (ix->adj_mag_valid && ix->level_table_valid && ix->table_level_min >= 2u && ix->eng == ENG_U8 && ix->G == 64u &&
+                      cosdev::tune_or(cosdev::TUNE_WALK_UP_TABLE, WALK_UP_TABLE_DEFAULT) != 0)
+                         ? ix->table_level_min - 1u
+                         : 0u;
+    if (want != 0u && (ix->adj_up_level == want || ix->adj_up_oom_level == want)) return COS_OK;
+    bool any = false;
+    for (u32 l = 0; l <= ix->p.num_layers; l++) any = any || ix->lv[l].d_adj_up;
+    if (any) {
+        HIP_TRY(hipDeviceSynchronize());
+        for (u32 l = 0; l <= ix->p.num_layers; l++) ix->lv[l].d_adj_up.reset();
+    }
+    ix->adj_up_level = 0;
+    if (want == 0u) return COS_OK;
+    ix->adj_up_oom_level = 0;
+    HIP_TRY(hipDeviceSynchronize());
+    LevelHost &H = ix->lv[want];
+    const LevelHost &U = ix->lv[want + 1];
+    const u32 slots = std::min(H.M, ix->p.shortlist_size);
+    if (!H.d_adj_node || !U.d_child || H.n == 0 || U.n == 0) return COS_OK;
+    DevArr<u32> up;
+    hipError_t e = H.d_adj_up.alloc((size_t)H.n * slots);
+    if (e == hipSuccess) e = up.alloc(H.n);
+    if (e == hipErrorOutOfMemory) {
+        (void)hipGetLastError();
+        H.d_adj_up.reset();
+        ix->adj_up_oom_level = want;
+        return COS_OK;
+    }
+    HIP_TRY(e);
+    HIP_TRY(cosdev::launch_fill_adj_up(H.d_adj_vec, H.d_adj_node, ix->d_mags, U.d_child, U.n, up, H.d_adj_up, H.n, H.M, slots, ix->own_stream));
+    HIP_TRY(hipStreamSynchronize(ix->own_stream));
+    ix->adj_up_level = want;
+    return COS_OK;
+}
+
 int32_t cos_prepare_walk_plans(cos_index *ix) {
     std::lock_guard<std::mutex> g(ix->mu);
     if (int32_t rc = ensure_adj_mags(ix)) return rc;
     if (ix->walk_order_min_B)
         if (int32_t rc = ensure_order_rank(ix)) return rc;
-    if (walk_table_min_B(ix))
+    if (walk_table_min_B(ix)) {
         if (int32_t rc = ensure_level_table(ix)) return rc;
+        if (int32_t rc = ensure_adj_up(ix)) return rc;
+    }
     return COS_OK;
 }
 
@@ -927,6 +968,8 @@
     }
     if (want.prepare_table) {
         if (int32_t rc = ensure_level_table(ix)) return rc;
+        if (int32_t rc = ensure_adj_up(ix)) return rc;
+        have.adj_up_level = ix->adj_up_level;
         const size_t need = (size_t)w->capB * ix->table_stride;
         if (need > w->tab.cap) {
             const size_t budget = (size_t)cosdev::tune_or(cosdev::TUNE_WALK_TABLE_MAX_BYTES, (long long)48 << 30);
@@ -988,6 +1031,8 @@
     dev.visited_mode = L.visited_mode;
     for (u32 l = 0; l <= dev.num_layers; l++)
         if (!((plan.use_adj_mag >> l) & 1u)) dev.lv[l].adj_mag = nullptr;
+    for (u32 l = 0; l <= dev.num_layers; l++)
+        if (plan.up_table_level != l || l == 0u || dev.lv[l].adj_mag == nullptr) dev.lv[l].adj_up = nullptr;
     WalkArgs wa;
     memset(&wa, 0, sizeof(wa));
     if (dev.visited_mode == COS_VISITED_EXACT) {
@@ -998,6 +1043,7 @@
     if (timed) HIP_TRY(hipEventRecord(ev[0], st));
     HIP_TRY(launch_quantize_rows(ix->eng, d_queries, ix->p.dim, B, ix->p.dim, ix->p.range_lo, ix->p.range_hi, w->q_codes, ix->row_stride,
                                  w->q_mags, w->q_raw_mags, st, plan.use_table && ix->eng == ENG_U8 ? w->qsums.p : nullptr));
+    HIP_TRY(hipMemsetAsync(w->stats2, 0, (size_t)B * 32, st));
     if (plan.use_table) {
         auto table_part = [&](hipEvent_t cos_index::*handle_ev, hipEvent_t own_ev, hipEvent_t *marks, u32 wgs, bool first) -> int32_t {
             if (plan.table_waits_for_sort) {
@@ -1029,7 +1075,6 @@
     wa.out_status = w->walk_status;
     wa.out_stats = w->stats;
     wa.out_stats2 = w->stats2;
-    HIP_TRY(hipMemsetAsync(w->stats2, 0, (size_t)B * 32, st));
     if (plan.use_table) {
         wa.tab = w->tab;
         wa.tab_mags = L.tmags;
diff --git a/cosdata_amd/csrc/engine_internal.h b/cosdata_amd/csrc/engine_internal.h
--- a/cosdata_amd/csrc/engine_internal.h
+++ b/cosdata_amd/csrc/engine_internal.h
@@ -28,6 +28,8 @@
 hipError_t launch_grow_rows(const u32 *src, u32 *dst, u32 old_n, u32 new_n, u32 M, u32 remap_from, u32 remap_to, u32 fill, hipStream_t st);
 hipError_t launch_grow_bytes(const uint8_t *src, uint8_t *dst, u32 old_n, u32 new_n, hipStream_t st);
 hipError_t launch_fill_adj_mag(const u32 *adj_vec, const float *mags, float *adj_mag, u32 n, u32 M, u32 slots, hipStream_t st);
+hipError_t launch_fill_adj_up(const u32 *adj_vec, const u32 *adj_node, const float *mags, const u32 *child_up, u32 n_up, u32 *up, AdjUp *adj_up, u32 n, u32 M, u32 slots,
+                              hipStream_t st);
 hipError_t launch_link_round(const LinkArgs &a, u32 maxM, const u32 *pend, const u32 *pcount, u32 *next, u32 *next_count, u32 *evq, u32 *evq_count,
                              u32 count_ub, u32 round, hipStream_t st);
 hipError_t launch_quantize_rows(int eng, const float *x, u64 x_stride, u32 n, u32 dim, float lo, float hi, uint8_t *codes,
@@ -88,12 +90,13 @@
     DevArr<u32> d_adj_vec, d_adj_node, d_node_vec, d_child;
     DevArr<u32> d_node_id, d_node_meta;
     DevArr<float> d_adj_mag;
+    DevArr<cosdev::AdjUp> d_adj_up;
     u32 n = 0, M = 0;
     u32 root_idx = 0;
     bool host_valid = false;
     void release() {
         d_adj_vec.reset(); d_adj_node.reset(); d_node_vec.reset(); d_child.reset();
-        d_node_id.reset(); d_node_meta.reset(); d_adj_mag.reset();
+        d_node_id.reset(); d_node_meta.reset(); d_adj_mag.reset(); d_adj_up.reset();
         n = 0;
         node_ids.clear();
         nbr_ids.clear();
@@ -237,6 +240,8 @@
     u32 walk_table_max_cols = COS_WALK_TABLE_AUTO, walk_table_min_B = COS_WALK_TABLE_DEFAULT_MIN_B;
     size_t table_bytes_total = 0;
     bool adj_mag_valid = false;
+    u32 adj_up_level = 0, adj_up_oom_level = 0;
+    void invalidate_adj_side() { adj_mag_valid = false; adj_up_level = 0; adj_up_oom_level = 0; }
     LinkState link;
     bool level_table_valid = false;
     u32 table_level_min = 0, table_cols = 0;
diff --git a/cosdata_amd/csrc/engine_types.h b/cosdata_amd/csrc/engine_types.h
--- a/cosdata_amd/csrc/engine_types.h
+++ b/cosdata_amd/csrc/engine_types.h
@@ -14,6 +14,7 @@
     u32 root_idx;
     const float *adj_mag;
     u32 mag_stride;
+    const AdjUp *adj_up;
     const u32 *node_id;
     const u32 *node_meta;
 };
diff --git a/cosdata_amd/csrc/kernels_link.hip b/cosdata_amd/csrc/kernels_link.hip
--- a/cosdata_amd/csrc/kernels_link.hip
+++ b/cosdata_amd/csrc/kernels_link.hip
@@ -405,6 +405,25 @@
     }
 }
 
+__global__ void scatter_up_kernel(const u32 *__restrict__ child_up, u32 n_up, u32 *__restrict__ up, u32 n) {
+    for (u64 j = (u64)blockIdx.x * blockDim.x + threadIdx.x; j < n_up; j += (u64)gridDim.x * blockDim.x) {
+        const u32 c = child_up[j];
+        if (c < n) up[c] = (u32)j;
+    }
+}
+__global__ void fill_adj_up_kernel(const u32 *__restrict__ adj_vec, const u32 *__restrict__ adj_node, const float *__restrict__ mags, const u32 *__restrict__ up, u32 n,
+                                   AdjUp *__restrict__ adj_up, u64 total, u32 M, u32 slots) {
+    for (u64 i = (u64)blockIdx.x * blockDim.x + threadIdx.x; i < total; i += (u64)gridDim.x * blockDim.x) {
+        const u64 node = i / slots;
+        const u32 slot = (u32)(i - node * slots);
+        const u32 row = adj_vec[node * M + slot], v = adj_node[node * M + slot];
+        AdjUp e;
+        e.mag = row == NONE ? 1.0f : mags[row];
+        e.up = v < n ? up[v] : ADJ_UP_NONE;
+        adj_up[i] = e;
+    }
+}
+
 }
 
 namespace cosdev {
@@ -456,6 +475,17 @@
     if (total == 0) return hipSuccess;
     const u32 blocks = (u32)std::min<u64>((total + 255) / 256, 1u << 20);
     hipLaunchKernelGGL(fill_adj_mag_kernel, dim3(blocks), dim3(256), 0, st, adj_vec, mags, adj_mag, total, M, slots);
+    return hipGetLastError();
+}
+
+hipError_t launch_fill_adj_up(const u32 *adj_vec, const u32 *adj_node, const float *mags, const u32 *child_up, u32 n_up, u32 *up, AdjUp *adj_up, u32 n, u32 M, u32 slots,
+                              hipStream_t st) {
+    const u64 total = (u64)n * slots;
+    if (total == 0 || n_up == 0) return hipErrorInvalidValue;
+    hipError_t e = hipMemsetAsync(up, 0xFF, (size_t)n * sizeof(u32), st);
+    if (e != hipSuccess) return e;
+    hipLaunchKernelGGL(scatter_up_kernel, dim3((u32)std::min<u64>(((u64)n_up + 255) / 256, 1u << 20)), dim3(256), 0, st, child_up, n_up, up, n);
+    hipLaunchKernelGGL(fill_adj_up_kernel, dim3((u32)std::min<u64>((total + 255) / 256, 1u << 20)), dim3(256), 0, st, adj_vec, adj_node, mags, up, n, adj_up, total, M, slots);
     return hipGetLastError();
 }
 
diff --git a/cosdata_amd/csrc/kernels_sparse.hip b/cosdata_amd/csrc/kernels_sparse.hip
--- a/cosdata_amd/csrc/kernels_sparse.hip
+++ b/cosdata_amd/csrc/kernels_sparse.hip
@@ -1032,6 +1032,11 @@
     HIP_TRY(hipMemcpy(out_ids, s->w_oi.p, (size_t)B * top_k * 4, hipMemcpyDeviceToHost));
     HIP_TRY(hipMemcpy(out_scores, s->w_os.p, (size_t)B * top_k * 4, hipMemcpyDeviceToHost));
     HIP_TRY(hipMemcpy(out_counts, s->w_oc.p, (size_t)B * 4, hipMemcpyDeviceToHost));
+    for (u32 q = 0; q < B; q++)
+        for (u32 i = std::min(out_counts[q], top_k); i < top_k; i++) {
+            out_ids[(size_t)q * top_k + i] = 0xFFFFFFFFu;
+            out_scores[(size_t)q * top_k + i] = 0.0f;
+        }
     return sparse_wait_previous(s);
 }
 
diff --git a/cosdata_amd/csrc/tuning.h b/cosdata_amd/csrc/tuning.h
--- a/cosdata_amd/csrc/tuning.h
+++ b/cosdata_amd/csrc/tuning.h
@@ -39,6 +39,7 @@
     TUNE_FINALIZE_WIDE_MAX_B,
     TUNE_FLAT_FP4_W8,
     TUNE_WALK_TABLE_EARLY_WGS,
+    TUNE_WALK_UP_TABLE,
     TUNE_COUNT
 };
 
diff --git a/cosdata_amd/csrc/tuning.hip b/cosdata_amd/csrc/tuning.hip
--- a/cosdata_amd/csrc/tuning.hip
+++ b/cosdata_amd/csrc/tuning.hip
@@ -15,7 +15,7 @@
     "bm25_blocks", "sparse_layout", "walk_pb", "walk_pb_upper", "walk_lat", "walk_lat4", "walk_small_table_tk", "walk_lat_warm",
     "walk_lat_la", "walk_lat4_e", "finalize_fast", "shardset_force_rccl", "build_profile",
     "walk_merge_min", "walk_adj_mag", "walk_table_rule_c", "walk_table_after_sort", "walk_upper_lds_pad", "walk_r2", "finalize_wide_max_b", "flat_fp4_w8",
-    "walk_table_early_wgs",
+    "walk_table_early_wgs", "walk_up_table",
 };
 std::atomic<long long> g_values[TUNE_COUNT];
 std::once_flag g_once;
diff --git a/cosdata_amd/csrc/walk_kernel.inc b/cosdata_amd/csrc/walk_kernel.inc
--- a/cosdata_amd/csrc/walk_kernel.inc
+++ b/cosdata_amd/csrc/walk_kernel.inc
@@ -150,14 +150,19 @@
         u32 lev_evals = 1;
         const u32 log2M = (u32)__ffs((int)M) - 1u;
         const u64 slotmask = slots >= 64u ? ~0ull : ((1ull << slots) - 1ull);
-        auto level_rounds = [&](auto tabc, auto cosc, auto amagc) __attribute__((always_inline)) {
+        auto level_rounds = [&](auto tabc, auto cosc, auto amagc, auto upc) __attribute__((always_inline)) {
         constexpr bool TAB = decltype(tabc)::value;
         constexpr bool COSINE = decltype(cosc)::value;
         constexpr bool AMAG = decltype(amagc)::value && G64 && !FLOAT_ENG;
+        constexpr bool UPT = decltype(upc)::value && AMAG && !TAB && ENG == ENG_U8;
         const u32 metric_t = COSINE ? 0u : metric;
+        constexpr int LAW = UPT ? LA - 1 : LA;
+        u32 *const w_vec = sm.win_vec, *const w_node = UPT ? sm.win_vec + LAW * 64 : sm.win_node, *const w_up = sm.win_vec + 3 * LAW * 64;
+        float *const w_mag = UPT ? (float *)(sm.win_vec + 2 * LAW * 64) : sm.win_mag;
+        const float *tabu = UPT ? wa.tab + (u64)qi * wa.tab_stride + wa.tab_col0[UPT ? level + 1 : 0] : nullptr;
         while (npool > 0 && npop < wa.ef) {
             n_rounds++;
-            u32 kwin = npool < (u32)LA ? npool : (u32)LA;
+            u32 kwin = npool < (u32)LAW ? npool : (u32)LAW;
             if (kwin > wa.ef - npop) kwin = wa.ef - npop;
             u32 wv_[LA], wn_[LA];
             {
@@ -165,20 +170,27 @@
                 auto fetch_stage = [&](auto bothc) {
                     constexpr bool BOTH = decltype(bothc)::value;
                     float wm_[LA];
-                    static_for<0, LA>([&](auto ic) {
+                    u32 wu_[LA];
+                    static_for<0, LAW>([&](auto ic) {
                         constexpr int i = decltype(ic)::value;
                         const u32 nd = pool.template peek_node<i>();
                         const u64 off = ((u64)nd << log2M) + slot_l;
                         wv_[i] = lv.adj_vec[off];
                         if constexpr (BOTH) wn_[i] = lv.adj_node[off];
-                        if constexpr (!TAB && AMAG) wm_[i] = lv.adj_mag[(u64)nd * lv.mag_stride + slot_l];
+                        if constexpr (!TAB && AMAG && !UPT) wm_[i] = lv.adj_mag[(u64)nd * lv.mag_stride + slot_l];
+                        if constexpr (UPT) {
+                            const uint2 mu = ((const uint2 *)lv.adj_up)[(u64)nd * lv.mag_stride + slot_l];
+                            wm_[i] = __uint_as_float(mu.x);
+                            wu_[i] = mu.y;
+                        }
                     });
                     if constexpr (!TAB) {
-                        static_for<0, LA>([&](auto ic) {
+                        static_for<0, LAW>([&](auto ic) {
                             constexpr int i = decltype(ic)::value;
-                            sm.win_vec[i * 64 + lane] = wv_[i];
-                            sm.win_node[i * 64 + lane] = BOTH ? wn_[i] : wv_[i];
-                            if constexpr (AMAG) sm.win_mag[i * 64 + lane] = wm_[i];
+                            w_vec[i * 64 + lane] = wv_[i];
+                            w_node[i * 64 + lane] = BOTH ? wn_[i] : wv_[i];
+                            if constexpr (AMAG) w_mag[i * 64 + lane] = wm_[i];
+                            if constexpr (UPT) w_up[i * 64 + lane] = wu_[i];
                         });
                     }
                 };
@@ -186,7 +198,7 @@
                 else fetch_stage(std::false_type{});
             }
             u32 stop = 0;
-            auto consume = [&](u32 wi, u32 nb_vec, u32 nb_node, float nb_mag) __attribute__((always_inline)) {
+            auto consume = [&](u32 wi, u32 nb_vec, u32 nb_node, float nb_mag, u32 nb_up) __attribute__((always_inline)) {
                 if constexpr (R == 1) {
                     const u64 hd = pool.head();
                     res_lo = writelane_dyn(res_lo, (u32)hd, (int)npop);
@@ -311,6 +323,19 @@
                     if constexpr (AMAG) magw = nb_mag;
                     else if (win) magw = ix.mags[nb_vec];
                     u64 m = wmask;
+                    if constexpr (UPT) {
+                        const u64 tmask = wmask & ballot64(nb_up != ADJ_UP_NONE);
+                        if (tmask) {
+                            float dotv = 0.0f;
+                            if (__builtin_amdgcn_inverse_ballot_w64(tmask)) dotv = tabu[nb_up];
+                            bool badl;
+                            const float sim = cosine_or_dot<ENG == ENG_U8>(metric, dotv, qmag, magw, badl);
+                            if (tmask & ballot64(badl)) failed = 1;
+                            else commit(tmask, metric_key(metric, sim), nb_node);
+                            n_tab += (u64)__popcll(tmask);
+                            m = wmask & ~tmask;
+                        }
+                    }
                     while (m && !failed) {
                         u32 lsel = 0;
                         u32 tot = 0;
@@ -433,27 +458,34 @@
             if constexpr (TAB) {
                 static_for<0, LA>([&](auto ic) __attribute__((always_inline)) {
                     constexpr int i = decltype(ic)::value;
-                    if ((u32)i < kwin && !stop) consume((u32)i, wv_[i], wn_[i], 1.0f);
+                    if ((u32)i < kwin && !stop) consume((u32)i, wv_[i], wn_[i], 1.0f, ADJ_UP_NONE);
                 });
             } else {
                 for (u32 wi = 0; wi < kwin && !stop; wi++)
-                    consume(wi, sm.win_vec[wi * 64 + lane], sm.win_node[wi * 64 + lane], AMAG ? sm.win_mag[wi * 64 + lane] : 1.0f);
+                    consume(wi, w_vec[wi * 64 + lane], w_node[wi * 64 + lane], AMAG ? w_mag[wi * 64 + lane] : 1.0f, UPT ? w_up[wi * 64 + lane] : ADJ_UP_NONE);
             }
             if (failed) break;
         }
         };
         if (tab_level) {
-            if (metric == 0u) level_rounds(std::true_type{}, std::true_type{}, std::false_type{});
-            else level_rounds(std::true_type{}, std::false_type{}, std::false_type{});
+            if (metric == 0u) level_rounds(std::true_type{}, std::true_type{}, std::false_type{}, std::false_type{});
+            else level_rounds(std::true_type{}, std::false_type{}, std::false_type{}, std::false_type{});
         } else {
             bool done = false;
             if constexpr (G64 && !FLOAT_ENG) {
                 if (lv.adj_mag != nullptr) {
-                    level_rounds(std::false_type{}, std::false_type{}, std::true_type{});
+                    bool up = false;
+                    if constexpr (ENG == ENG_U8) {
+                        if (lv.adj_up != nullptr && wa.tab != nullptr && (u32)level + 1u == wa.tab_level_min) {
+                            level_rounds(std::false_type{}, std::false_type{}, std::true_type{}, std::true_type{});
+                            up = true;
+                        }
+                    }
+                    if (!up) level_rounds(std::false_type{}, std::false_type{}, std::true_type{}, std::false_type{});
                     done = true;
                 }
             }
-            if (!done) level_rounds(std::false_type{}, std::false_type{}, std::false_type{});
+            if (!done) level_rounds(std::false_type{}, std::false_type{}, std::false_type{}, std::false_type{});
         }
         n_exp += npop;
         adj_bytes += (u64)npop * slots * 4;
diff --git a/cosdata_amd/csrc/walk_plan.h b/cosdata_amd/csrc/walk_plan.h
--- a/cosdata_amd/csrc/walk_plan.h
+++ b/cosdata_amd/csrc/walk_plan.h
@@ -36,6 +36,7 @@
     uint32_t table_early_wgs;
     bool table_queue;
     uint32_t n_cus;
+    uint32_t up_table_mode;
 };
 
 struct WalkHave {
@@ -43,6 +44,7 @@
     bool table_buffer;
     uint32_t n_order_keys, order_level0;
     bool order_buffers;
+    uint32_t adj_up_level;
 };
 
 struct WalkPlan {
@@ -57,6 +59,7 @@
     bool side_stream;
     bool prepare_order, prepare_table;
     uint32_t table_level_min, table_cols, cut_after_level;
+    uint32_t up_table_level;
 };
 
 inline uint32_t table_gemm_stripe_tiles(uint32_t B, uint32_t cols, uint32_t n_cus, bool shared) {
@@ -133,6 +136,12 @@
         for (uint32_t l = 0; l <= in.num_layers; l++)
             if (in.adj_mag_mode == 2 || (in.ef <= 2u * in.M[l] && in.B >= ADJ_MAG_USE_MIN_B)) p.use_adj_mag |= 1u << l;
     p.refill_adj_mag = !in.adj_mag_valid && in.B >= ADJ_MAG_REFILL_MIN_B;
+    if (have && p.use_table && p.kernel == WalkKernel::Throughput && in.up_table_mode != 0 && in.eng == WALK_PLAN_ENG_U8 && in.G == 64u &&
+        in.mdim == 0u && have->table_level_min >= 2u && have->adj_up_level == have->table_level_min - 1u) {
+        const uint32_t l = have->table_level_min - 1u;
+        if (in.up_table_mode == 2 && in.adj_mag_valid && in.adj_mag_mode != 0) p.use_adj_mag |= 1u << l;
+        if ((p.use_adj_mag >> l) & 1u) p.up_table_level = l;
+    }
     p.side_stream = in.side_min_B && in.B >= in.side_min_B;
     p.prepare_order = p.ordered;
     p.prepare_table = p.use_table;
```

After: 1.142 million (median of 6 runs). 8.3% higher.
